# proxima-one/kzg

Measured on AMD Instinct MI355X. Metric: commitments/sec + MSM G1-adds/sec at degree 2^20, 1/2/4/8 MI355X, higher is better.
Workload: dtype u32 limbs (Fq 381-bit / Fr 255-bit Montgomery integer arithmetic); 1 GPU; degree-2^20 coeff_form commit (G1 Pippenger MSM) on 1xMI355X, batch of 64 per step; mode=single, polynomial_coefficients=1048576, scalars=uniform full-width Fr (SplitMix64 counter stream), terms_per_rank=1048576, window_bits=17, windows=15, srs=setup(tau, n) generated on the GPU, table=15 window rows 2^(17 w) P per point, inputs_resident_in_hbm=True

## Files before the change

### kzg_amd/csrc/capi.hip

```cpp
#include <algorithm>

#include "common.h"
#include "emit.h"
#include "multiopen_plan.h"

namespace kzg {

static int host_scalar(kzg_ctx *ctx, const void *s, int sfmt, Fr *mont) {
    Fr v;
    memcpy(v.v, s, 32);
    if (sfmt == KZG_FR_CANONICAL_LE_32) {
        if (!is_canonical(v)) return fail(ctx, KZG_ERR_SHAPE, "scalar not canonical (>= r)");
        v = to_mont(v);
    } else if (sfmt != KZG_FR_MONT_LE_32) {
        return fail(ctx, KZG_ERR_SHAPE, "unknown scalar format");
    }
    *mont = v;
    return KZG_OK;
}

static void scalar_out(const Fr &mont, int sfmt, void *dst) {
    Fr v = sfmt == KZG_FR_CANONICAL_LE_32 ? from_mont(mont) : mont;
    memcpy(dst, v.v, 32);
}
// ... 39 lines not shown
            KZG_HIP_CHECK(ctx, hipMemcpyAsync(ctx->lanes[lane].pinned, d_pt, sizeof(MsmPoint), hipMemcpyDeviceToHost, st));
            KZG_TRY(heavy_pickup_enqueue(ctx, lane));
            KZG_HIP_CHECK(ctx, hipStreamSynchronize(st));
            MsmPoint pt;
            memcpy(&pt, ctx->lanes[lane].pinned, sizeof pt);
            alignas(16) uint8_t buf[144];
            emit_one(pt, buf, ofmt);
            memcpy(out, buf, psz);
        } else {
            KZG_TRY(emit_point(ctx, lane, d_pt, ctx->lanes[lane].pinned, ofmt));
            KZG_TRY(heavy_pickup_enqueue(ctx, lane));
            KZG_HIP_CHECK(ctx, hipStreamSynchronize(st));
            memcpy(out, ctx->lanes[lane].pinned, psz);
        }
    }
    heavy_pickup_read(ctx, lane);
    if (ctx->prof) prof_collect(ctx);
    return KZG_OK;
}

static int check_sfmt(kzg_ctx *ctx, int sfmt) {
    if (sfmt != KZG_FR_MONT_LE_32 && sfmt != KZG_FR_CANONICAL_LE_32) return fail(ctx, KZG_ERR_SHAPE, "unknown scalar format");
    return KZG_OK;
}

static bool is_pow2(size_t x) { return x && !(x & (x - 1)); }
static bool count_ok(size_t n) { return n <= ((size_t)1 << 40); }

#ifdef KZG_TEST_HOOKS
__global__ __launch_bounds__(256) void k_test_fr_mul(const Fr *a, const Fr *b, size_t n, Fr *o) {
    size_t i = (size_t)blockIdx.x * blockDim.x + threadIdx.x;
    if (i < n) o[i] = mul(a[i], b[i]);
}
__global__ __launch_bounds__(256) void k_test_fq_mul(const Fq *a, const Fq *b, size_t n, Fq *o) {
    size_t i = (size_t)blockIdx.x * blockDim.x + threadIdx.x;
    if (i < n) o[i] = mul(a[i], b[i]);
}
__global__ __launch_bounds__(256) void k_test_fr_inv(const Fr *a, size_t n, Fr *o) {
    size_t i = (size_t)blockIdx.x * blockDim.x + threadIdx.x;
    if (i < n) o[i] = a[i].is_zero() ? Fr::zero() : inv(a[i]);
}
__global__ __launch_bounds__(256) void k_test_g1_add(const G1Affine *a, const G1Affine *b, size_t n, G1Affine *o) {
    size_t i = (size_t)blockIdx.x * blockDim.x + threadIdx.x;
    if (i >= n) return;
    G1Xyzz p = g1_madd(G1Xyzz::from_affine(a[i]), b[i]);
    G1Xyzz pa = g1_madd(g1_dbl(G1Xyzz::from_affine(a[i])), g1_neg(a[i]));
    G1Xyzz pb = g1_madd(g1_dbl(G1Xyzz::from_affine(b[i])), g1_neg(b[i]));
    G1Xyzz q = g1_add(pa, pb);
    G1Affine r1 = g1_to_affine(p), r2 = g1_to_affine(q);
    bool same = (r1.x == r2.x) && (r1.y == r2.y);
    o[i] = same ? r1 : G1Affine{Fq::one(), Fq::one()};
}
__global__ __launch_bounds__(256) void k_test_g1_mul(const G1Affine *p, const Fr *k, size_t n, G1Affine *o) {
    size_t i = (size_t)blockIdx.x * blockDim.x + threadIdx.x;
    if (i >= n) return;
    Fr kk = k[i];
    o[i] = g1_to_affine(g1_scalar_mul(p[i], kk.v));
}

#endif

}

using namespace kzg;

extern "C" int kzg_msm_g1(kzg_ctx *ctx, const kzg_srs *srs, size_t offset, const void *scalars, size_t n, int sfmt,
                          int flags, void *out, int ofmt) {
    if (!ctx || !srs || !out || (!scalars && n)) return KZG_ERR_SHAPE;
    Lease ls;
    KZG_TRY(lease_lane(ctx, &ls));
    const int lane = ls.lane;
    KZG_HIP_CHECK(ctx, hipSetDevice(ctx->device));
    KZG_TRY(check_sfmt(ctx, sfmt));
    if (!point_format_bytes(ofmt)) return fail(ctx, KZG_ERR_SHAPE, "unknown G1 output format");
    if (n > srs->n || offset > srs->n - n) return fail(ctx, KZG_ERR_SHAPE, "MSM range exceeds the SRS (reference: slice index panic)");
    KZG_TRY(lane_reserve(ctx, lane, msm_workspace_bytes(srs, n) + stage_bytes(n * 32, flags) + 8192));
    const void *d_sc = nullptr;
    KZG_TRY(stage_in(ctx, lane, scalars, n * 32, flags, &d_sc));
    MsmPoint *res = nullptr;
    KZG_TRY(lease_msm(ctx, ls, srs, offset, d_sc, n, sfmt, &res));
    return finish_point(ctx, lane, res, out, ofmt, flags);
}

extern "C" int kzg_commit_coeff(kzg_ctx *ctx, const kzg_srs *srs, const void *coeffs, size_t n, int sfmt, int flags,
                                void *out, int ofmt) {
    return kzg_msm_g1(ctx, srs, 0, coeffs, n, sfmt, flags, out, ofmt);
}

extern "C" int kzg_commit_eval(kzg_ctx *ctx, const kzg_srs *lagrange, const void *evals, size_t d, int sfmt, int flags,
                               void *out, int ofmt) {
    if (!ctx || !lagrange) return KZG_ERR_SHAPE;
    if (d != lagrange->n) return fail(ctx, KZG_ERR_SHAPE, "assert!(self.d == evals.d) (src/eval_form.rs:115)");
    return kzg_msm_g1(ctx, lagrange, 0, evals, d, sfmt, flags, out, ofmt);
}

struct BatchPipe {
    int nl = 1, nas = 0;
    uint8_t *d_out = nullptr;
    bool out_dev = false;
};

static int batch_begin(kzg_ctx *ctx, size_t batch, size_t out_bytes, void *out, int flags, BatchPipe *bp) {
    bp->out_dev = (flags & KZG_OUT_DEVICE) != 0;
    if (bp->out_dev) {
        bp->d_out = (uint8_t *)out;
    } else {
        if (ctx->batch_out_bytes < out_bytes + 256) {
            if (ctx->batch_out) hipFree(ctx->batch_out);
            ctx->batch_out = nullptr;
            ctx->batch_out_bytes = 0;
            KZG_HIP_CHECK(ctx, hipMalloc((void **)&ctx->batch_out, out_bytes + 256));
            ctx->batch_out_bytes = out_bytes + 256;
        }
        bp->d_out = (uint8_t *)ctx->batch_out;
    }
    KZG_TRY(plan_pipeline(ctx, (int)std::min<size_t>(batch, (size_t)ctx->opt_streams), &bp->nl, &bp->nas));
    for (int l = 0; l < bp->nl; l++) set_lane_mode(ctx, l, bp->nl > 1, batch >= 2 * (size_t)bp->nl);
    return KZG_OK;
}

static int batch_msm(kzg_ctx *ctx, const BatchPipe &bp, size_t b, int lane, const kzg_srs *srs, size_t offset, const void *d_sc,
                     size_t n, int sfmt, MsmPoint **res, MsmPending *defer = nullptr) {
    if (bp.nas) {
        const int ev = defer ? lane + (int)((b / (size_t)bp.nl) & 1) * bp.nl : lane;
        return msm_run(ctx, lane, srs, offset, d_sc, n, sfmt, res, ctx->accum_streams[b % (size_t)accum_streams_for(ctx, bp.nas, srs, n)],
                       ctx->sorted_events[ev], ctx->accum_events[ev], defer);
    }
    return msm_run(ctx, lane, srs, offset, d_sc, n, sfmt, res);
}

static int batch_end(kzg_ctx *ctx, const BatchPipe &bp, int rc, void *out, size_t out_bytes) {
    for (int l = 0; l < bp.nl; l++) hipStreamSynchronize(ctx->lanes[l].stream);
    for (int l = 0; l < bp.nl; l++) set_lane_mode(ctx, l, false, false);
    if (rc == KZG_OK && !bp.out_dev) {
        hipError_t e = hipMemcpy(out, bp.d_out, out_bytes, hipMemcpyDeviceToHost);
        if (e != hipSuccess) rc = fail(ctx, KZG_ERR_HIP, hipGetErrorString(e));
    }
#if !defined(KZG_TIMING_NO_PICKUP)
    if (rc == KZG_OK) {
        uint32_t hv[KZG_MAX_LANES];
        if (hipMemcpy(hv, ctx->d_lane_heavy, sizeof hv, hipMemcpyDeviceToHost) == hipSuccess)
            for (int l = 0; l < bp.nl; l++) {
                Lane &ln = ctx->lanes[l];
                if (ln.heavy_seq == ln.heavy_seen) continue;
                ln.heavy_seen = ln.heavy_seq;
                if (hv[l] == ln.heavy_seq) ctx->heavy_last.store(ctx->msm_count.load(std::memory_order_relaxed), std::memory_order_relaxed);
            }
    }
#endif
    if (ctx->prof) prof_collect(ctx);
    return rc;
}

namespace kzg {
int msm_batch_strided(kzg_ctx *ctx, const kzg_srs *srs, size_t offset, const void *scalars, size_t n, size_t batch,
                      size_t stride_bytes, int sfmt, int flags, void *out, int ofmt) {
    Guard g(ctx);
    KZG_HIP_CHECK(ctx, hipSetDevice(ctx->device));
    KZG_TRY(check_sfmt(ctx, sfmt));
    size_t psz = point_format_bytes(ofmt);
    if (!psz) return fail(ctx, KZG_ERR_SHAPE, "unknown G1 output format");
    if (n > srs->n || offset > srs->n - n) return fail(ctx, KZG_ERR_SHAPE, "MSM range exceeds the SRS");
    if (batch == 0) return KZG_OK;
    BatchPipe bp;
    KZG_TRY(batch_begin(ctx, batch, batch * psz, out, flags, &bp));
    size_t per = align_up(msm_workspace_bytes(srs, n) + stage_bytes(n * 32, flags) + 8192, 4096);
    int rc = KZG_OK;
    const bool defer = bp.nas > 0 && batch > (size_t)bp.nl && !ctx->opt_no_defer_tail;
    std::vector<MsmPending> pend(defer ? 2 * (size_t)bp.nl : 0);
    for (int l = 0; l < bp.nl && rc == KZG_OK; l++) rc = lane_reserve(ctx, l, defer ? 2 * per : per);
    auto finish = [&](size_t b) {
        const int l = (int)(b % bp.nl);
        MsmPoint *res = nullptr;
        int r = msm_finish(ctx, pend[(size_t)l + ((b / (size_t)bp.nl) & 1) * (size_t)bp.nl], &res);
        if (r == KZG_OK) r = emit_point(ctx, l, res, bp.d_out + b * psz, ofmt);
        return r;
    };
    for (size_t b = 0; b < batch && rc == KZG_OK; b++) {
        int l = (int)(b % bp.nl);
        const size_t half = defer ? ((b / (size_t)bp.nl) & 1) : 0;
        ctx->lanes[l].arena_used = half * per;
        ctx->lanes[l].arena_limit = defer ? (half + 1) * per : 0;
        const void *d_sc = nullptr;
        rc = stage_in(ctx, l, (const uint8_t *)scalars + b * stride_bytes, n * 32, flags, &d_sc);
        MsmPoint *res = nullptr;
        if (defer) {
            MsmPending &pd = pend[(size_t)l + half * (size_t)bp.nl];
            if (rc == KZG_OK) rc = batch_msm(ctx, bp, b, l, srs, offset, d_sc, n, sfmt, &res, &pd);
            if (rc == KZG_OK && !pd.active) pd.result = res;
            if (rc == KZG_OK && b >= (size_t)bp.nl) rc = finish(b - bp.nl);
            continue;
        }
        if (rc == KZG_OK) rc = batch_msm(ctx, bp, b, l, srs, offset, d_sc, n, sfmt, &res);
        if (rc == KZG_OK) rc = emit_point(ctx, l, res, bp.d_out + b * psz, ofmt);
    }
    if (defer)
        for (size_t b = batch > (size_t)bp.nl ? batch - bp.nl : 0; b < batch && rc == KZG_OK; b++) rc = finish(b);
    for (int l = 0; l < bp.nl; l++) ctx->lanes[l].arena_limit = 0;
    return batch_end(ctx, bp, rc, out, batch * psz);
}
}

extern "C" int kzg_msm_g1_batch(kzg_ctx *ctx, const kzg_srs *srs, size_t offset, const void *scalars, size_t n,
                                size_t batch, int sfmt, int flags, void *out, int ofmt) {
    if (!ctx || !srs || !out || (!scalars && n && batch)) return KZG_ERR_SHAPE;
    if (n > SIZE_MAX / 32) return KZG_ERR_SHAPE;
    return msm_batch_strided(ctx, srs, offset, scalars, n, batch, n * 32, sfmt, flags, out, ofmt);
}

extern "C" int kzg_witness_coeff_many(kzg_ctx *ctx, const kzg_srs *srs, const void *coeffs, size_t n, const void *xs,
                                      const void *ys, size_t count, int sfmt, int flags, void *out, int ofmt, int *status) {
    if (!ctx || !srs || !coeffs || !out || n == 0 || ((!xs || !ys) && count)) return KZG_ERR_SHAPE;
    Guard g(ctx);
    KZG_HIP_CHECK(ctx, hipSetDevice(ctx->device));
    KZG_TRY(check_sfmt(ctx, sfmt));
    size_t psz = point_format_bytes(ofmt);
    if (!psz) return fail(ctx, KZG_ERR_SHAPE, "unknown G1 output format");
    if (n - 1 > srs->n) return fail(ctx, KZG_ERR_SHAPE, "quotient longer than the SRS (reference: slice index panic)");
    if (count == 0) return KZG_OK;
    std::vector<Fr> xm(count);
    for (size_t j = 0; j < count; j++) KZG_TRY(host_scalar(ctx, (const uint8_t *)xs + 32 * j, sfmt, &xm[j]));
    for (size_t j = 0; j < count; j++) {
        Fr ym;
        KZG_TRY(host_scalar(ctx, (const uint8_t *)ys + 32 * j, sfmt, &ym));
    }
    BatchPipe bp;
    KZG_TRY(batch_begin(ctx, count, count * psz, out, flags, &bp));
    int rc = KZG_OK;
    const int sl = bp.nl;
    rc = ensure_lanes(ctx, sl + 1);
    if (rc == KZG_OK) rc = lane_reserve(ctx, sl, stage_bytes(n * 32, flags) + count * 32 + 4096);
    const void *d_coeffs = nullptr;
    Fr *d_px = nullptr;
    if (rc == KZG_OK) rc = stage_in(ctx, sl, coeffs, n * 32, flags, &d_coeffs);
    if (rc == KZG_OK && !(d_px = (Fr *)lane_alloc(ctx, sl, count * 32))) rc = fail(ctx, KZG_ERR_ALLOC, "workspace");
    if (rc == KZG_OK && hipStreamSynchronize(ctx->lanes[sl].stream) != hipSuccess) rc = fail(ctx, KZG_ERR_HIP, "stage-in of the coefficients");
    size_t per = msm_workspace_bytes(srs, n - 1) + n * 32 + (n / 2048 + 4) * 64 + 65536;
    for (int l = 0; l < bp.nl && rc == KZG_OK; l++) rc = lane_reserve(ctx, l, per);
    for (size_t j = 0; j < count && rc == KZG_OK; j++) {
        int l = (int)(j % bp.nl);
        ctx->lanes[l].arena_used = 0;
        Fr *dq = (Fr *)lane_alloc(ctx, l, n * 32);
        if (!dq) rc = fail(ctx, KZG_ERR_ALLOC, "workspace");
        if (rc == KZG_OK) rc = quotient_linear_run(ctx, l, (const Fr *)d_coeffs, n, xm[j], dq, d_px + j);
        MsmPoint *res = nullptr;
        if (rc == KZG_OK) rc = batch_msm(ctx, bp, j, l, srs, 0, dq, n - 1, sfmt, &res);
        if (rc == KZG_OK) rc = emit_point(ctx, l, res, bp.d_out + j * psz, ofmt);
    }
    rc = batch_end(ctx, bp, rc, out, count * psz);
    if (rc != KZG_OK) return rc;
    std::vector<uint8_t> px(count * 32);
    KZG_HIP_CHECK(ctx, hipMemcpy(px.data(), d_px, count * 32, hipMemcpyDeviceToHost));
    int worst = KZG_OK;
    for (size_t j = 0; j < count; j++) {
        int sj = memcmp(px.data() + 32 * j, (const uint8_t *)ys + 32 * j, 32) != 0 ? KZG_ERR_POINT_NOT_ON_POLY : KZG_OK;
        if (status) status[j] = sj;
        if (sj) worst = sj;
    }
    if (worst && !status) return fail(ctx, KZG_ERR_POINT_NOT_ON_POLY, "point not on polynomial!");
    return KZG_OK;
}

extern "C" int kzg_witness_eval_many(kzg_ctx *ctx, const kzg_srs *lagrange, const void *evals, size_t d, const size_t *indices,
                                     size_t count, int sfmt, int flags, void *out, int ofmt) {
    if (!ctx || !lagrange || !evals || !out || (!indices && count)) return KZG_ERR_SHAPE;
    Guard g(ctx);
    KZG_HIP_CHECK(ctx, hipSetDevice(ctx->device));
    KZG_TRY(check_sfmt(ctx, sfmt));
    size_t psz = point_format_bytes(ofmt);
    if (!psz) return fail(ctx, KZG_ERR_SHAPE, "unknown G1 output format");
    if (!is_pow2(d)) return fail(ctx, KZG_ERR_SHAPE, "evaluation domain size must be a power of two");
    for (size_t j = 0; j < count; j++)
        if (indices[j] >= d) return fail(ctx, KZG_ERR_SHAPE, "evaluation index out of range (reference: index panic)");
    if (d > lagrange->n) return fail(ctx, KZG_ERR_SHAPE, "evaluations longer than the Lagrange SRS (reference: slice panic)");
    uint32_t log_d = (uint32_t)ilog2_ceil(d);
    if (log_d >= FR_TWO_ADICITY) return fail(ctx, KZG_ERR_DEGREE_TOO_LARGE, "domain too large");
    if (count == 0) return KZG_OK;
    BatchPipe bp;
    KZG_TRY(batch_begin(ctx, count, count * psz, out, flags, &bp));
    const int sl = bp.nl;
    int rc = ensure_lanes(ctx, sl + 1);
    if (rc == KZG_OK) rc = lane_reserve(ctx, sl, stage_bytes(d * 32, flags) + 4096);
    const void *de = nullptr;
    if (rc == KZG_OK) rc = stage_in(ctx, sl, evals, d * 32, flags, &de);
    if (rc == KZG_OK) rc = eval_tables_ready(ctx, sl, log_d);
    size_t per = msm_workspace_bytes(lagrange, d) + d * 32 + (d / 256 + 4) * 32 + 65536;
    for (int l = 0; l < bp.nl && rc == KZG_OK; l++) rc = lane_reserve(ctx, l, per);
    for (size_t j = 0; j < count && rc == KZG_OK; j++) {
        int l = (int)(j % bp.nl);
        ctx->lanes[l].arena_used = 0;
        Fr *dq = (Fr *)lane_alloc(ctx, l, d * 32);
        if (!dq) rc = fail(ctx, KZG_ERR_ALLOC, "workspace");
        if (rc == KZG_OK) rc = quotient_eval_run(ctx, l, (const Fr *)de, log_d, indices[j], sfmt, dq);
        MsmPoint *res = nullptr;
        if (rc == KZG_OK) rc = batch_msm(ctx, bp, j, l, lagrange, 0, dq, d, sfmt, &res);
        if (rc == KZG_OK) rc = emit_point(ctx, l, res, bp.d_out + j * psz, ofmt);
    }
    return batch_end(ctx, bp, rc, out, count * psz);
}

extern "C" int kzg_g1_sum(kzg_ctx *ctx, const void *points, size_t count, int pfmt, int flags, void *out, int ofmt) {
    if (!ctx || !out || (!points && count)) return KZG_ERR_SHAPE;
    Guard g(ctx);
    KZG_HIP_CHECK(ctx, hipSetDevice(ctx->device));
    size_t psz = point_format_bytes(pfmt);
    if (!psz || !point_format_bytes(ofmt)) return fail(ctx, KZG_ERR_SHAPE, "unknown G1 point format");
    size_t cnt = count ? count : 1;
    size_t need = stage_bytes(cnt * psz, flags) + cnt * sizeof(G1Xyzz) + (cnt + 2 * sum_points_scratch_count(cnt) + 4) * sizeof(MsmPoint) + 8192;
    KZG_TRY(lane_reserve(ctx, 0, need));
    hipStream_t st = ctx->lanes[0].stream;
    G1Xyzz *dec = (G1Xyzz *)lane_alloc(ctx, 0, cnt * sizeof(G1Xyzz));
    MsmPoint *pts = (MsmPoint *)lane_alloc(ctx, 0, cnt * sizeof(MsmPoint));
    MsmPoint *scratch = (MsmPoint *)lane_alloc(ctx, 0, 2 * sum_points_scratch_count(cnt) * sizeof(MsmPoint));
    int *bad = (int *)lane_alloc(ctx, 0, 256);
    if (!dec || !pts || !scratch || !bad) return fail(ctx, KZG_ERR_ALLOC, "sum workspace not reserved");
    KZG_HIP_CHECK(ctx, hipMemsetAsync(bad, 0, sizeof(int), st));
    MsmPoint *res = pts;
    if (count == 0) {
        KZG_TRY(point_set_infinity(ctx, st, pts));
    } else {
        const void *d_raw = nullptr;
        KZG_TRY(stage_in(ctx, 0, points, count * psz, flags, &d_raw));
        KZG_TRY(decode_points(ctx, st, d_raw, count, pfmt, dec, bad, POINTS_ON_CURVE));
        KZG_TRY(points_to30(ctx, st, dec, pts, count));
        KZG_TRY(sum_points_run(ctx, 0, pts, count, scratch, &res));
    }
    int hbad = 0;
    KZG_HIP_CHECK(ctx, hipMemcpyAsync(&hbad, bad, sizeof(int), hipMemcpyDeviceToHost, st));
    KZG_TRY(finish_point(ctx, 0, res, out, ofmt, flags));
    if (hbad) return fail(ctx, KZG_ERR_BAD_POINT, "a G1 point failed to decode or is not on the curve");
    return KZG_OK;
}

namespace kzg {
int g1_sum_batch_strided(kzg_ctx *ctx, const void *points, size_t count, size_t groups, size_t gstride, size_t istride, int pfmt,
                         int flags, void *out, int ofmt, int level) {
    Guard g(ctx);
    KZG_HIP_CHECK(ctx, hipSetDevice(ctx->device));
    size_t psz = point_format_bytes(pfmt), osz = point_format_bytes(ofmt);
    if (!psz || !osz) return fail(ctx, KZG_ERR_SHAPE, "unknown G1 point format");
    if (count > (1u << 20) || groups > (1u << 24)) return fail(ctx, KZG_ERR_SHAPE, "kzg_g1_sum_batch: count <= 2^20, groups <= 2^24");
    size_t total = count && groups ? (groups - 1) * gstride + (count - 1) * istride + 1 : 0;
    KZG_TRY(lane_reserve(ctx, 0, stage_bytes(total * psz, flags) + total * sizeof(G1Xyzz) + (total + groups + 4) * sizeof(MsmPoint) + groups * 144 + 65536));
    hipStream_t st = ctx->lanes[0].stream;
    G1Xyzz *dec = (G1Xyzz *)lane_alloc(ctx, 0, total * sizeof(G1Xyzz));
    MsmPoint *pts = (MsmPoint *)lane_alloc(ctx, 0, total * sizeof(MsmPoint));
    MsmPoint *tmp = (MsmPoint *)lane_alloc(ctx, 0, groups * sizeof(MsmPoint));
    int *bad = (int *)lane_alloc(ctx, 0, 256);
    void *d_out = (flags & KZG_OUT_DEVICE) ? out : lane_alloc(ctx, 0, groups * osz);
    if (!dec || !pts || !tmp || !bad || !d_out) return fail(ctx, KZG_ERR_ALLOC, "sum workspace not reserved");
    KZG_HIP_CHECK(ctx, hipMemsetAsync(bad, 0, sizeof(int), st));
    const void *d_raw = nullptr;
    KZG_TRY(stage_in(ctx, 0, points, total * psz, flags, &d_raw));
    KZG_TRY(decode_points(ctx, st, d_raw, total, pfmt, dec, bad, level));
    KZG_TRY(points_to30(ctx, st, dec, pts, total));
    const bool on_host = !(flags & KZG_OUT_DEVICE) && ctx->opt_host_affine && groups <= 4;
    KZG_TRY(sum_groups_emit(ctx, 0, pts, count, groups, gstride, istride, tmp, on_host ? nullptr : d_out, ofmt));
    int hbad = 0;
    KZG_HIP_CHECK(ctx, hipMemcpyAsync(&hbad, bad, sizeof(int), hipMemcpyDeviceToHost, st));
    MsmPoint hsum[4];
// ... 1198 lines not shown
```

### kzg_amd/csrc/common.h

```cpp
#pragma once
#ifndef KZG_NTT_KERNEL_DEFAULT
#define KZG_NTT_KERNEL_DEFAULT 1
#endif
#include <hip/hip_runtime.h>
#include <stdint.h>
#include <stdio.h>

#include <array>
#include <atomic>
#include <condition_variable>
#include <map>
#include <mutex>
#include <string>
#include <vector>

#include "../../include/kzg_mi355x.h"
#include "curve.h"
#include "curve30.h"

namespace kzg {

struct ProfEntry {
    uint64_t launches = 0;
    double total_ms = 0.0;
};

struct PendingEvent {
    std::string name;
    hipEvent_t start, stop;
};

#ifndef KZG_ACCUM_WAVES
#define KZG_ACCUM_WAVES 2
#endif

struct MsmMode {
    int accum_blocks = 256 * KZG_ACCUM_WAVES;
    int sort_threads = 1024;
    bool tail_quads = true;
    bool tail_wide = false;
};

struct Lane {
    MsmMode mode;
    hipStream_t stream = nullptr;
    char *arena = nullptr;
    size_t arena_bytes = 0;
    size_t arena_used = 0;
    size_t arena_limit = 0;
    uint32_t heavy_seq = 0, heavy_seen = 0;
    char *pinned = nullptr;
    size_t pinned_bytes = 0;
};

struct NttPlan;
struct FixedBaseTable;
struct EvalDomainTables;

struct CtxGate {
    std::mutex m;
    std::condition_variable cv;
    int shared_active = 0;
    int excl_waiting = 0;
    bool exclusive = false;
    uint32_t lane_busy = 0;
    void lock() {
        std::unique_lock<std::mutex> lk(m);
        excl_waiting++;
        cv.wait(lk, [&] { return !exclusive && shared_active == 0; });
        excl_waiting--;
        exclusive = true;
    }
    void unlock() {
        {
            std::lock_guard<std::mutex> lk(m);
            exclusive = false;
        }
        cv.notify_all();
    }
};
constexpr int KZG_HEAVY_WINDOW = 64;
constexpr int KZG_MAX_LANES = 24;

}

struct kzg_ctx;
namespace kzg {
struct StreamPool;
struct PointSetCache;
void point_sets_free(kzg_ctx *ctx);
void point_set_stats(kzg_ctx *ctx, uint64_t *hits, uint64_t *misses);
}
struct kzg_ctx {
    int device = 0;
    kzg::CtxGate mu;
    std::mutex err_mu;
    std::mutex prof_mu;
    std::mutex cache_mu;
    std::mutex accum_mu;
    std::atomic<uint32_t> accum_rr{0};
    int plan_want_lanes = 0, plan_want_accum = 0, plan_lanes = 0, plan_accum = 0, plan_queues = 0;
    bool plan_warned = false;
    bool pipe_planned = false;
    int pipe_lanes = 1, pipe_accum = 0;
    std::string err;
    std::vector<kzg::Lane> lanes;
    kzg::StreamPool *pool = nullptr;
    int opt_window_bits = 0;
    int opt_streams = 13;
    int opt_accum_blocks = 0;
    int opt_hw_queues = 0;
    int probed_queues = 0;
    int probed_lanes = 0, probed_accum = 0;
    std::vector<hipStream_t> probed_order;
    int opt_window_rows = 0;
    int opt_naf_window = 0;
    int opt_trusted_points = 0;
    int opt_ntt_vec_log = 2;
    int opt_verify_cosets_chunk = 0;
    int opt_verify_eval_batch_chunk = 0;
    int opt_multiopen_points_chunk = 0;
    int opt_multi_eval_segment = 0;
    int opt_multi_eval_points_chunk = 0;
    int opt_poly_divide_base = 0;
    int opt_point_tree_leaf = 0;
    int opt_host_pairing = 1;
    int opt_fk20_cosets_combine = 0;
    int opt_ntt_kernel = KZG_NTT_KERNEL_DEFAULT;
    int opt_ntt_three_from = 23;
    int opt_ntt_vec2_log = 1;
    int opt_ntt_xcd = 1;
    int opt_accum_blocks_batch = 0;
    int opt_tail_quads = 1;
    int opt_accum_streams = 2;
    int opt_accum_streams_small = 4;
    int opt_accum_blocks_small = 160;
    int64_t opt_small_entries = 2 << 20;
    int planned_accum = 0;
    bool msm_small(size_t entries) const { return opt_accum_blocks_small > 0 && planned_accum >= 3 && (int64_t)entries <= opt_small_entries; }
    hipStream_t accum_streams[4] = {nullptr, nullptr, nullptr, nullptr};
    std::vector<hipEvent_t> sorted_events, accum_events;
    int opt_sort_threads = 1024;
    int opt_sort_threads_batch = 1024;
    int opt_host_affine = 1;
    int opt_heavy_bins = 0;
    bool opt_no_defer_tail = false;
    int opt_sort_single = 0;
    int accum_blocks_single() const { return opt_accum_blocks ? opt_accum_blocks : 256 * KZG_ACCUM_WAVES; }
    int accum_blocks_batch() const { return opt_accum_blocks_batch ? opt_accum_blocks_batch : 240 * KZG_ACCUM_WAVES; }
    int num_cus = 256;
    std::atomic<bool> attr_msm_set{false}, attr_ntt_set{false}, attr_wide_set{false}, attr_sort20_set{false}, attr_horner_set{false};
    bool prof = false;
    bool prof_only_accum = false;
    std::map<std::string, kzg::ProfEntry> prof_map;
    std::vector<kzg::PendingEvent> prof_pending;
    std::vector<hipEvent_t> event_pool;
    std::map<uint32_t, kzg::NttPlan *> ntt_plans;
    std::map<uint32_t, kzg::EvalDomainTables *> eval_tabs;
    kzg::FixedBaseTable *fixed_base = nullptr;
    std::vector<std::pair<std::array<uint32_t, 8>, void *>> coset_tabs;
    kzg::PointSetCache *point_sets = nullptr;
    int opt_witness_cache_slots = 16;
    std::atomic<uint64_t> msm_count{0}, heavy_last{0};
    uint32_t *d_lane_heavy = nullptr;
    void *batch_out = nullptr;
    size_t batch_out_bytes = 0;
};

struct kzg_srs {
    size_t n = 0;
    size_t npad = 0;
    int c = 0;
    int W = 0;
    int rows = 0;
    bool narrow17 = false;
    bool sort20 = false;
    int naf = 0;
    int row_shift = 0;
    kzg::G1Affine *table = nullptr;
    void *table30 = nullptr;
    int device = 0;
};

namespace kzg {

struct Guard {
    std::lock_guard<CtxGate> lk;
    explicit Guard(kzg_ctx *c) : lk(c->mu) {}
};

struct Lease {
    kzg_ctx *ctx = nullptr;
    int lane = -1;
    bool pipelined = false;
    uint32_t slot = 0;
    ~Lease();
};
int lease_lane(kzg_ctx *ctx, Lease *ls);

enum { POINTS_TRUSTED = 0, POINTS_ON_CURVE = 1, POINTS_SUBGROUP = 2 };

#define KZG_HIP_CHECK(ctx, expr)                                                                   \
    do {                                                                                           \
        hipError_t _e = (expr);                                                                    \
        if (_e != hipSuccess) return kzg::fail((ctx), KZG_ERR_HIP, std::string(#expr) + ": " + hipGetErrorString(_e)); \
    } while (0)

#define KZG_TRY(expr)                                                                              \
    do {                                                                                           \
        int _s = (expr);                                                                           \
        if (_s != KZG_OK) return _s;                                                               \
    } while (0)

struct ThreadErr {
    const kzg_ctx *ctx = nullptr;
    std::string msg;
};
inline ThreadErr &thread_err() {
    static thread_local ThreadErr te;
    return te;
}
inline int fail(kzg_ctx *ctx, int code, const std::string &msg) {
    {
        std::lock_guard<std::mutex> lk(ctx->err_mu);
        ctx->err = msg;
    }
    ThreadErr &te = thread_err();
    te.ctx = ctx;
    te.msg = msg;
    return code;
}

int lane_reserve(kzg_ctx *ctx, int lane, size_t bytes);
void *lane_alloc(kzg_ctx *ctx, int lane, size_t bytes);
int lane_pinned(kzg_ctx *ctx, int lane, size_t bytes);
int ensure_lanes(kzg_ctx *ctx, int want);
int plan_pipeline(kzg_ctx *ctx, int want, int *nl_out, int *nas_out);
void set_lane_mode(kzg_ctx *ctx, int lane, bool pipelined, bool deep);
int accum_streams_for(kzg_ctx *ctx, int planned, const kzg_srs *srs, size_t n);

struct ProfScope {
    kzg_ctx *ctx;
    hipStream_t stream;
    hipEvent_t start = nullptr, stop = nullptr;
    const char *name;
    ProfScope(kzg_ctx *c, hipStream_t s, const char *n);
    ~ProfScope();
};
void prof_collect(kzg_ctx *ctx);

#define KZG_LAUNCH(ctx, stream, name, kern, grid, block, shmem, ...)                               \
    do {                                                                                           \
        kzg::ProfScope _ps((ctx), (stream), (name));                                               \
        hipLaunchKernelGGL(kern, dim3(grid), dim3(block), (shmem), (stream), __VA_ARGS__);         \
    } while (0)

inline int untrusted_level(const kzg_ctx *ctx) { return ctx->opt_trusted_points ? POINTS_ON_CURVE : POINTS_SUBGROUP; }
inline size_t align_up(size_t x, size_t a) { return (x + a - 1) / a * a; }
inline int ilog2_ceil(size_t x) {
    int l = 0;
    while (((size_t)1 << l) < x) l++;
    return l;
}

typedef G1Xyzz30 MsmPoint;

size_t msm_workspace_bytes(const kzg_srs *srs, size_t n);
int finish_point(kzg_ctx *ctx, int lane, const MsmPoint *d_pt, void *out, int ofmt, int flags);
struct MsmPending {
    bool active = false;
    hipStream_t st = nullptr;
    hipEvent_t accum_ev = nullptr;
    MsmMode mm;
    const MsmPoint *part = nullptr;
    MsmPoint *scratch = nullptr, *result = nullptr;
    const uint32_t *s1 = nullptr;
    int B = 0;
    size_t expected = 0;
    void *state = nullptr;
    char *tail_base = nullptr;
    size_t tail_off[8] = {0, 0, 0, 0, 0, 0, 0, 0};
    bool odd = false;
};
int msm_run(kzg_ctx *ctx, int lane, const kzg_srs *srs, size_t offset, const void *d_scalars, size_t n, int sfmt,
            MsmPoint **d_result, hipStream_t accum_stream = nullptr, hipEvent_t sorted_ev = nullptr, hipEvent_t accum_ev = nullptr,
            MsmPending *defer = nullptr);
int msm_finish(kzg_ctx *ctx, MsmPending &pd, MsmPoint **d_result);
int lease_msm(kzg_ctx *ctx, const Lease &ls, const kzg_srs *srs, size_t offset, const void *d_sc, size_t n, int sfmt, MsmPoint **res);
int sum_points_run(kzg_ctx *ctx, int lane, MsmPoint *d_points, size_t count, MsmPoint *d_scratch, MsmPoint **d_result);
int points_to30(kzg_ctx *ctx, hipStream_t st, const G1Xyzz *d_in, MsmPoint *d_out, size_t n);
int points_from30(kzg_ctx *ctx, hipStream_t st, const MsmPoint *d_in, G1Xyzz *d_out, size_t n);
int point_set_infinity(kzg_ctx *ctx, hipStream_t st, MsmPoint *d_pt);
size_t sum_points_scratch_count(size_t count);
int emit_point(kzg_ctx *ctx, int lane, const MsmPoint *d_point, void *d_out, int ofmt);
size_t point_format_bytes(int fmt);
int sum_groups_emit(kzg_ctx *ctx, int lane, const MsmPoint *d_pts, size_t count, size_t groups, size_t gstride, size_t istride,
                    MsmPoint *d_tmp, void *d_out, int ofmt);

int msm_batch_strided(kzg_ctx *ctx, const kzg_srs *srs, size_t offset, const void *scalars, size_t n, size_t batch,
                      size_t stride_bytes, int sfmt, int flags, void *out, int ofmt);
int g1_sum_batch_strided(kzg_ctx *ctx, const void *points, size_t count, size_t groups, size_t gstride, size_t istride, int pfmt,
                         int flags, void *out, int ofmt, int level = POINTS_ON_CURVE);

int srs_choose_window(int opt_window_bits, size_t n);
void srs_shape(int opt_window_bits, int opt_window_rows, size_t n, int *c, int *W, int *rows, bool *narrow17, int opt_naf = 0, int *naf = nullptr);
inline size_t srs_entries_per_scalar(const kzg_srs *s) { return s->naf ? (size_t)s->W : (size_t)s->rows; }
int srs_alloc(kzg_ctx *ctx, size_t n, kzg_srs **out);
int srs_finish_from_xyzz(kzg_ctx *ctx, kzg_srs *srs, G1Xyzz *d_row0_xyzz);
int srs_precompute(kzg_ctx *ctx, kzg_srs *srs);
int batch_to_affine(kzg_ctx *ctx, hipStream_t stream, const G1Xyzz *d_in, G1Affine *d_out, size_t n);
int decode_points(kzg_ctx *ctx, hipStream_t st, const void *d_raw, size_t n, int fmt, G1Xyzz *d_out, int *d_bad,
                  int level = POINTS_SUBGROUP);

int fixed_base_mul(kzg_ctx *ctx, hipStream_t stream, const Fr *d_scalars_mont, size_t n, G1Xyzz *d_out);
int powers_run(kzg_ctx *ctx, hipStream_t st, const Fr &base_mont, size_t first, size_t n, Fr *d_out);
int lagrange_scalars_run(kzg_ctx *ctx, hipStream_t st, const Fr &tau_mont, size_t d, Fr *d_out);

struct WitnessSink {
    const kzg_srs *srs;
    size_t first, len;
    size_t total;
    void *d_partial;
};
int witness_coeff_batched_run(kzg_ctx *ctx, const WitnessSink &sink, const void *coeffs, size_t n, const void *xs, const void *ys,
                              size_t k, int sfmt, int flags, void *out_w, int ofmt, void *out_r, size_t *out_r_len);
int vanishing_poly_run(kzg_ctx *ctx, hipStream_t st, const Fr *d_xs_mont, size_t k, Fr *d_z, Fr *d_tmp);
int coset_ntt_run(kzg_ctx *ctx, int lane, Fr *d, uint32_t log_n, int inverse, const Fr &g, size_t nnz = (size_t)-1);

void ntt_plans_free(kzg_ctx *ctx);
void eval_tabs_free(kzg_ctx *ctx);
void fixed_base_free(kzg_ctx *ctx);

int ntt_run(kzg_ctx *ctx, int lane, Fr *d_data, uint32_t log_n, int inverse, size_t nnz = (size_t)-1);
inline size_t ntt_workspace_bytes(uint32_t log_n) {
    const size_t n = (size_t)1 << log_n;
    return log_n > 24 ? n * 32 + ((size_t)1 << 24) * 32 + (2 << 20) : n * 32 + 4096;
}
bool ntt_short_input_ok(uint32_t log_n, size_t nnz);
int pow_table(kzg_ctx *ctx, hipStream_t stream, const Fr &base_mont, const Fr &scale_mont, size_t count, Fr *d_out);
Fr host_omega(uint32_t exp);

int fr_convert(kzg_ctx *ctx, hipStream_t stream, Fr *d_data, size_t n, int to_mont);
int batch_inverse(kzg_ctx *ctx, hipStream_t stream, const Fr *d_in, Fr *d_out, size_t n);
int batch_inverse_mul(kzg_ctx *ctx, hipStream_t stream, const Fr *d_c, Fr *d_a, Fr *d_tmp, size_t n, int *d_flag);
int poly_eval_run(kzg_ctx *ctx, int lane, const Fr *d_coeffs, size_t n, const Fr &x_mont, Fr *d_y_out);
int eval_tables_ready(kzg_ctx *ctx, int lane, uint32_t log_d);
int quotient_linear_run(kzg_ctx *ctx, int lane, const Fr *d_coeffs, size_t n, const Fr &x_mont, Fr *d_q_out,
                        Fr *d_px_out);
int quotient_eval_run(kzg_ctx *ctx, int lane, const Fr *d_evals, uint32_t log_d, size_t m, int sfmt, Fr *d_q_out);

constexpr int OE_MAX_CHUNK = 16;
struct OpenPoint {
    Fr z;
    Fr c;
    bool on_domain;
    size_t m;
};
int open_point_classify(uint32_t log_d, const Fr &z_mont, OpenPoint *pt);
size_t open_eval_fr_workspace_bytes(size_t d, size_t B);
size_t open_eval_fr_workspace_bytes(size_t d, size_t B, size_t nz);
int open_eval_fr_run(kzg_ctx *ctx, int lane, const Fr *d_evals, uint32_t log_d, size_t B, const OpenPoint *pts, int sfmt, Fr *d_y, Fr *d_q);

size_t open_powtab_bytes(size_t d);
int open_powtab_run(kzg_ctx *ctx, hipStream_t st, uint32_t log_d, Fr *d_tab);
int open_inverses_run(kzg_ctx *ctx, hipStream_t st, uint32_t log_d, const Fr *d_tab, const Fr *z_mont, int nz, Fr *d_den, Fr *d_inv);
int open_eval_values_idx_run(kzg_ctx *ctx, hipStream_t st, const Fr *d_evals, uint32_t log_d, const Fr *d_inv, const uint32_t *d_vidx,
                             const uint32_t *d_pu, const Fr *d_z, const Fr *d_c, size_t B, Fr *d_partial, Fr *d_y);

int fold_run(kzg_ctx *ctx, hipStream_t st, const Fr *d_v, size_t d, size_t t, size_t gstride, size_t groups, const Fr *d_gammas_mont,
             bool carry, Fr *d_out);

int lincomb_run(kzg_ctx *ctx, hipStream_t st, const Fr *d_v, size_t d, const uint32_t *d_idx, const Fr *d_weight, size_t count, bool carry,
                Fr *d_out);
int multiopen_gather_run(kzg_ctx *ctx, hipStream_t st, const Fr *d_v, size_t d, const uint32_t *d_idx, const uint32_t *d_at, size_t count, Fr *d_y);
int multiopen_accum_run(kzg_ctx *ctx, hipStream_t st, const Fr *d_v, size_t d, const uint32_t *d_idx, const Fr *d_w, const uint32_t *d_pstart,
                        int nz, const Fr *d_y, Fr *d_Y, const Fr *d_inv, Fr *d_g);

int series_inverse_run(kzg_ctx *ctx, int lane, const Fr *d_f, size_t fl_all, size_t m, size_t base, Fr *d_g, Fr *d_A, Fr *d_G);

int pt_ntt_run(kzg_ctx *ctx, hipStream_t st, Fr *d, size_t total, uint32_t log_t, int dit, const Fr *tw, uint32_t log_tw);


}
```

### kzg_amd/csrc/msm.hip

```cpp
#include "msm_internal.h"
#include "msm_sort.h"
#include "emit.h"
#include "naf.h"

namespace kzg {

template <class F>
__device__ __forceinline__ void digits_of(const uint32_t s[8], int c, int W, bool balanced, F f) {
    if (c == 17 && W == 15) for_each_digit_fixed<17, 15>(s, balanced, f);
    else for_each_digit(s, c, W, balanced, f);
}

extern __shared__ __attribute__((aligned(16))) uint32_t lds_u32[];

__global__ __launch_bounds__(1024) void k_hist(const Fr *scalars, size_t n, int sfmt, int c, int W, int B,
                                               size_t per_block, uint32_t *blk_hist, int mode, int w_lo, int w_hi) {
    const bool pk = mode == 2;
    const int BH = pk ? B / 2 : B;
    size_t i0 = (size_t)blockIdx.x * per_block;
    size_t i1 = i0 + per_block < n ? i0 + per_block : n;
    uint32_t *dst = blk_hist + (size_t)blockIdx.x * B;
    for (int half = 0; half < (pk ? 2 : 1); half++) {
        const uint32_t base = (uint32_t)half * (uint32_t)BH;
        if (half) __syncthreads();
        for (int b = threadIdx.x; b < BH; b += blockDim.x) lds_u32[b] = 0;
        __syncthreads();
        for (size_t i = i0 + threadIdx.x; i < i1; i += blockDim.x) {
            uint32_t s[8];
            load_scalar(scalars, i, sfmt, s);
            digits_of(s, c, W, pk, [&](int w, uint32_t mag, uint32_t) {
                if (w < w_lo || w >= w_hi) return;
                const uint32_t idx = (mag - 1) & (uint32_t)(B - 1);
                if (pk && (idx >> 15) != (uint32_t)half) return;
                atomicAdd(&lds_u32[idx - base], 1u);
            });
        }
        __syncthreads();
        for (int b = threadIdx.x; b < BH; b += blockDim.x) dst[base + b] = lds_u32[b];
    }
}

constexpr int SCAN_SEG = 256;
__global__ __launch_bounds__(SCAN_SEG) void k_scan_a(uint32_t *blk_hist, int G, int B, uint32_t *total, uint32_t *local, uint32_t *agg,
                                                     uint32_t *ready) {
    __shared__ uint32_t lds[4];
    if (threadIdx.x == 0) ready[blockIdx.x] = 0;
    const int b = blockIdx.x * SCAN_SEG + threadIdx.x;
    uint32_t run = 0;
    if (b < B) {
        for (int g = 0; g < G; g++) {
            uint32_t t = blk_hist[(size_t)g * B + b];
            blk_hist[(size_t)g * B + b] = run;
            run += t;
        }
        total[b] = run;
    }
    uint32_t tot;
    uint32_t ex = block_scan_256(run, lds, &tot);
    if (b < B) local[b] = ex;
    if (threadIdx.x == 0) agg[blockIdx.x] = tot;
}

__device__ __forceinline__ uint32_t mod_u32(uint32_t x, uint32_t e, double rcp_e) {
    uint32_t q = (uint32_t)((double)x * rcp_e);
    uint32_t r = x - q * e;
    if ((int32_t)r < 0) r += e;
    if (r >= e) r -= e;
    return r;
}

__global__ __launch_bounds__(SCAN_SEG) void k_scan_b(const uint32_t *total, const uint32_t *local, const uint32_t *agg, int B, int NB,
                                                     uint32_t *bucket_start, uint32_t *s1, MsmState *st, uint32_t slots, uint32_t *ready) {
    __shared__ uint32_t lds[4];
    __shared__ uint32_t my_prefix;
    uint32_t M;
    {
        uint32_t v = (int)threadIdx.x < NB ? agg[threadIdx.x] : 0u;
        uint32_t ex = block_scan_256(v, lds, &M);
        if (threadIdx.x == blockIdx.x) my_prefix = ex;
    }
    __syncthreads();
    uint32_t E = (M + slots - 1) / slots;
    if (E < KZG_ACCUM_MIN_CHUNK) E = KZG_ACCUM_MIN_CHUNK;
    const double rcp_e = 1.0 / (double)E;
    const int b = blockIdx.x * SCAN_SEG + threadIdx.x;
    uint32_t start = 0, f = 0;
    if (b < B) {
        start = my_prefix + local[b];
        f = (total[b] != 0 && mod_u32(start, E, rcp_e) != 0) ? 1u : 0u;
    }
    uint32_t ftot;
    const uint32_t fex = block_scan_256(f, lds, &ftot);
    if (threadIdx.x == 0) __hip_atomic_store(&ready[blockIdx.x], (ftot << 1) | 1u, __ATOMIC_RELAXED, __HIP_MEMORY_SCOPE_AGENT);
    uint32_t prev = 0;
    if (threadIdx.x < blockIdx.x) {
        uint32_t w;
        while (((w = __hip_atomic_load(&ready[threadIdx.x], __ATOMIC_RELAXED, __HIP_MEMORY_SCOPE_AGENT)) & 1u) == 0) __builtin_amdgcn_s_sleep(1);
        prev = w >> 1;
    }
    uint32_t before;
    block_scan_256(prev, lds, &before);
    if (b < B) {
        bucket_start[b] = start;
        s1[b] = before + fex + (start + E - 1) / E;
    }
    if (blockIdx.x == (unsigned)NB - 1 && threadIdx.x == 0) {
        bucket_start[B] = M;
        s1[B] = before + ftot + (M + E - 1) / E;
        st->M = M;
        st->E = E;
        st->ntasks = (M + E - 1) / E;
        st->ovf_tasks = 0;
    }
}

static int scan_run(kzg_ctx *ctx, hipStream_t st, uint32_t *blk_hist, int G, int B, uint32_t *total, uint32_t *local, uint32_t *agg,
                    uint32_t *bucket_start, uint32_t *s1, MsmState *state, uint32_t slots) {
    const int NB = (B + SCAN_SEG - 1) / SCAN_SEG;
    uint32_t *ready = agg + SCAN_SEG;
    KZG_LAUNCH(ctx, st, "k_scan_a", k_scan_a, NB, SCAN_SEG, 0, blk_hist, G, B, total, local, agg, ready);
    KZG_LAUNCH(ctx, st, "k_scan_b", k_scan_b, NB, SCAN_SEG, 0, total, local, agg, B, NB, bucket_start, s1, state, slots, ready);
    return KZG_OK;
}

__global__ __launch_bounds__(1024) void k_scatter(const Fr *scalars, size_t n, int sfmt, int c, int W, int B,
                                                  size_t per_block, const uint32_t *blk_off,
                                                  const uint32_t *bucket_start, uint32_t row_stride,
                                                  uint32_t idx_base, uint32_t *entries, int mode, int w_lo, int w_hi) {
    const uint32_t *off = blk_off + (size_t)blockIdx.x * B;
    const bool pk = mode == 2;
    const int BH = pk ? B / 2 : B;
    size_t i0 = (size_t)blockIdx.x * per_block;
    size_t i1 = i0 + per_block < n ? i0 + per_block : n;
    for (int half = 0; half < (pk ? 2 : 1); half++) {
        const uint32_t base = (uint32_t)half * (uint32_t)BH;
        if (half) __syncthreads();
        for (int b = threadIdx.x; b < BH; b += blockDim.x) lds_u32[b] = bucket_start[base + b] + off[base + b];
        __syncthreads();
        for (size_t i = i0 + threadIdx.x; i < i1; i += blockDim.x) {
            uint32_t s[8];
            load_scalar(scalars, i, sfmt, s);
            digits_of(s, c, W, pk, [&](int w, uint32_t mag, uint32_t neg) {
                if (w < w_lo || w >= w_hi) return;
                const uint32_t idx = (mag - 1) & (uint32_t)(B - 1);
                if (pk && (idx >> 15) != (uint32_t)half) return;
                const uint32_t pos = atomicAdd(&lds_u32[idx - base], 1u);
                const uint32_t hi = mode == 1 ? (((mag - 1) >> WIDE_LO_BITS) << WIDE_HI_SHIFT) : 0u;
                entries[pos] = ((uint32_t)(w - w_lo) * row_stride + idx_base + (uint32_t)i) | hi | (neg << 31);
            });
        }
    }
}

constexpr int BIN_SHIFT = 6, BIN_BUCKETS = 1 << BIN_SHIFT;

__global__ __launch_bounds__(1024) void k_bin_hist(const Fr *scalars, size_t n, int sfmt, size_t per_block, uint32_t *blk_bins,
                                                   int w_lo, int w_hi) {
    KZG_SIDE_PRIO_STMT;
    __shared__ uint32_t h[NBINS];
    for (int b = threadIdx.x; b < NBINS; b += blockDim.x) h[b] = 0;
    __syncthreads();
    size_t i0 = (size_t)blockIdx.x * per_block;
    size_t i1 = i0 + per_block < n ? i0 + per_block : n;
    for (size_t i = i0 + threadIdx.x; i < i1; i += blockDim.x) {
        uint32_t s[8];
        load_scalar(scalars, i, sfmt, s);
        for_each_digit_fixed<17, 15>(s, true, [&](int w, uint32_t mag, uint32_t) {
            if (w < w_lo || w >= w_hi) return;
            atomicAdd(&h[(mag - 1) >> BIN_SHIFT], 1u);
        });
    }
    __syncthreads();
    for (int b = threadIdx.x; b < NBINS; b += blockDim.x) blk_bins[(size_t)blockIdx.x * NBINS + b] = h[b];
}

constexpr int BIN_SCAN_SLICES = 16, BIN_SCAN_MAXG = 32;
constexpr int SORT2_MAX_BLOCKS = BIN_SCAN_SLICES * BIN_SCAN_MAXG;
__global__ __launch_bounds__(1024) void k_bin_scan(uint32_t *blk_bins, int G, uint32_t *bin_total, uint32_t *ready) {
    KZG_SIDE_PRIO_STMT;
    __shared__ uint32_t part[BIN_SCAN_SLICES][64];
    if (blockIdx.x == 0 && threadIdx.x < SCAN_SEG) ready[threadIdx.x] = 0;
    const int binl = threadIdx.x & 63, slice = threadIdx.x >> 6;
    const int bin = blockIdx.x * 64 + binl;
    const int gs = (G + BIN_SCAN_SLICES - 1) / BIN_SCAN_SLICES;
    const int g0 = slice * gs;
    uint32_t v[BIN_SCAN_MAXG];
#pragma unroll
    for (int k = 0; k < BIN_SCAN_MAXG; k++) v[k] = (k < gs && g0 + k < G) ? blk_bins[(size_t)(g0 + k) * NBINS + bin] : 0u;
    uint32_t sum = 0;
#pragma unroll
    for (int k = 0; k < BIN_SCAN_MAXG; k++) {
        const uint32_t t = v[k];
        v[k] = sum;
        sum += t;
    }
    part[slice][binl] = sum;
    __syncthreads();
    uint32_t pre = 0, tot = 0;
#pragma unroll
    for (int s2 = 0; s2 < BIN_SCAN_SLICES; s2++) {
        const uint32_t t = part[s2][binl];
        if (s2 < slice) pre += t;
        tot += t;
    }
#pragma unroll
    for (int k = 0; k < BIN_SCAN_MAXG; k++)
        if (k < gs && g0 + k < G) blk_bins[(size_t)(g0 + k) * NBINS + bin] = pre + v[k];
    if (slice == 0) bin_total[bin] = tot;
}


constexpr int BIN_SCATTER_LDS = (3 * NBINS + 16 + 15 * 1024) * 4;
template <class REC>
__global__ __launch_bounds__(1024) void k_bin_scatter(const Fr *scalars, size_t n, int sfmt, size_t per_block, const uint32_t *blk_off,
                                                      const uint32_t *bin_total, uint32_t *bin_base, uint32_t row_stride,
                                                      uint32_t idx_base, typename REC::T *rec, int w_lo, int w_hi) {
    KZG_SIDE_PRIO_STMT;
    uint32_t *cur = lds_u32, *cnt = cur + NBINS, *off = cnt + NBINS, *wsum = off + NBINS, *stage = wsum + 16;
    const uint32_t tid = threadIdx.x;
    {
        uint32_t tot;
        const uint32_t ex = block_scan_1024(bin_total[tid], wsum, &tot);
        cur[tid] = ex + blk_off[(size_t)blockIdx.x * NBINS + tid];
        if (blockIdx.x == 0) {
            bin_base[tid] = ex;
            if (tid == 0) bin_base[NBINS] = tot;
        }
    }
    const size_t i0 = (size_t)blockIdx.x * per_block;
    const size_t i1 = i0 + per_block < n ? i0 + per_block : n;
    for (size_t c0 = i0; c0 < i1; c0 += 1024) {
        cnt[tid] = 0;
        __syncthreads();
        uint32_t pk[15], rk[15];
#pragma unroll
        for (int w = 0; w < 15; w++) pk[w] = 0xffffffffu;
        if (c0 + tid < i1) {
            uint32_t s[8];
            load_scalar(scalars, c0 + tid, sfmt, s);
            for_each_digit_fixed<17, 15>(s, true, [&](int w, uint32_t mag, uint32_t neg) {
                if (w < w_lo || w >= w_hi) return;
                const uint32_t idx = mag - 1, bin = idx >> BIN_SHIFT;
                rk[w] = atomicAdd(&cnt[bin], 1u);
                pk[w] = bin | ((idx & (BIN_BUCKETS - 1)) << 10) | (neg << 16) | ((uint32_t)(w - w_lo) << 17) | (tid << 21);
            });
        }
        __syncthreads();
        uint32_t tot;
        off[tid] = block_scan_1024(cnt[tid], wsum, &tot);
        __syncthreads();
#pragma unroll
        for (int w = 0; w < 15; w++)
            if (pk[w] != 0xffffffffu) stage[off[pk[w] & (NBINS - 1)] + rk[w]] = pk[w];
        __syncthreads();
        const uint32_t ebase = idx_base + (uint32_t)c0;
        for (uint32_t p = tid; p < tot; p += 1024) {
            const uint32_t v = stage[p], bin = v & (NBINS - 1);
            const uint32_t index = ((v >> 17) & 15u) * row_stride + ebase + (v >> 21);
            rec[cur[bin] + p - off[bin]] = REC::pack(index, (v >> 16) & 1u, (v >> 10) & (BIN_BUCKETS - 1));
        }
        __syncthreads();
        cur[tid] += cnt[tid];
    }
}

__global__ __launch_bounds__(1024) void k_naf_recode(const Fr *scalars, size_t n, int sfmt, size_t per_block, uint32_t *recs, uint32_t *blk_bins) {
    __shared__ uint32_t h[NBINS];
    __shared__ uint32_t limbs[1024 * 12];
    for (int b = threadIdx.x; b < NBINS; b += blockDim.x) h[b] = 0;
    __syncthreads();
    uint32_t *L = limbs + threadIdx.x * 12;
    size_t i0 = (size_t)blockIdx.x * per_block;
    size_t i1 = i0 + per_block < n ? i0 + per_block : n;
    for (size_t i = i0 + threadIdx.x; i < i1; i += blockDim.x) {
        uint32_t s[8];
        load_scalar(scalars, i, sfmt, s);
        uint32_t flip = 0;
        if (s[7] & 0x40000000u) {
            uint64_t bw = 0;
#pragma unroll
            for (int k = 0; k < 8; k++) {
                uint64_t d = (uint64_t)FrParams::mod(k) - s[k] - bw;
                s[k] = (uint32_t)d;
                bw = (d >> 63) & 1u;
            }
            flip = 1;
        }
#pragma unroll
        for (int k = 0; k < 8; k++) L[k] = s[k];
        L[8] = L[9] = L[10] = L[11] = 0;
        uint32_t d[NAF_MAX_DIGITS];
        const int cnt = naf18_digits(L, flip, d);
#pragma unroll
        for (int k = 0; k < NAF_MAX_DIGITS; k++) {
            const uint32_t r = k < cnt ? d[k] : 0u;
            recs[(size_t)k * n + i] = r;
            if (r) atomicAdd(&h[(r & 0x1ffffu) >> BIN_SHIFT], 1u);
        }
    }
    __syncthreads();
    for (int b = threadIdx.x; b < NBINS; b += blockDim.x) blk_bins[(size_t)blockIdx.x * NBINS + b] = h[b];
}

template <class REC>
__global__ __launch_bounds__(1024) void k_bin_scatter_naf(const uint32_t *recs, size_t n, size_t per_block, const uint32_t *blk_off,
                                                          const uint32_t *bin_total, uint32_t *bin_base, uint32_t row_stride,
                                                          uint32_t idx_base, typename REC::T *rec) {
    uint32_t *cur = lds_u32, *cnt = cur + NBINS, *off = cnt + NBINS, *wsum = off + NBINS, *stage = wsum + 16;
    const uint32_t tid = threadIdx.x;
    {
        uint32_t tot;
        const uint32_t ex = block_scan_1024(bin_total[tid], wsum, &tot);
        cur[tid] = ex + blk_off[(size_t)blockIdx.x * NBINS + tid];
        if (blockIdx.x == 0) {
            bin_base[tid] = ex;
            if (tid == 0) bin_base[NBINS] = tot;
        }
    }
    const size_t i0 = (size_t)blockIdx.x * per_block;
    const size_t i1 = i0 + per_block < n ? i0 + per_block : n;
    for (size_t c0 = i0; c0 < i1; c0 += 1024) {
        cnt[tid] = 0;
        __syncthreads();
        uint32_t pk[NAF_MAX_DIGITS], rk[NAF_MAX_DIGITS];
#pragma unroll
        for (int k = 0; k < NAF_MAX_DIGITS; k++) {
            pk[k] = 0xffffffffu;
            if (c0 + tid < i1) {
                const uint32_t r = recs[(size_t)k * n + c0 + tid];
                if (r & NAF_REC_VALID) {
                    const uint32_t idx = r & 0x1ffffu, bin = idx >> BIN_SHIFT;
                    rk[k] = atomicAdd(&cnt[bin], 1u);
                    pk[k] = bin | ((idx & (BIN_BUCKETS - 1)) << 10) | (((r >> 17) & 1u) << 16) | ((uint32_t)k << 17) | (tid << 21);
                }
            }
        }
        __syncthreads();
        uint32_t tot;
        off[tid] = block_scan_1024(cnt[tid], wsum, &tot);
        __syncthreads();
#pragma unroll
        for (int k = 0; k < NAF_MAX_DIGITS; k++)
            if (pk[k] != 0xffffffffu) stage[off[pk[k] & (NBINS - 1)] + rk[k]] = pk[k];
        __syncthreads();
        const uint32_t ebase = idx_base + (uint32_t)c0;
        for (uint32_t p = tid; p < tot; p += 1024) {
            const uint32_t v = stage[p], bin = v & (NBINS - 1), t = v >> 21, k = (v >> 17) & 15u;
            const uint32_t row = (recs[(size_t)k * n + c0 + t] >> 18) & 0xffu;
            const uint32_t index = row * row_stride + ebase + t;
            rec[cur[bin] + p - off[bin]] = REC::pack(index, (v >> 16) & 1u, (v >> 10) & (BIN_BUCKETS - 1));
        }
        __syncthreads();
        cur[tid] += cnt[tid];
    }
}


__global__ __launch_bounds__(SCAN_SEG) void k_scan_b_bins(const uint32_t *total, const uint32_t *bin_base, int B, int NB,
                                                          uint32_t *bucket_start, uint32_t *s1, MsmState *st, uint32_t slots,
                                                          uint32_t *ready) {
    KZG_SIDE_PRIO_STMT;
    __shared__ uint32_t lds[4];
    const uint32_t M = bin_base[NBINS];
    const uint32_t my_prefix = bin_base[blockIdx.x * (SCAN_SEG / BIN_BUCKETS)];
    uint32_t E = (M + slots - 1) / slots;
    if (E < KZG_ACCUM_MIN_CHUNK) E = KZG_ACCUM_MIN_CHUNK;
    const double rcp_e = 1.0 / (double)E;
    const int b = blockIdx.x * SCAN_SEG + threadIdx.x;
    const uint32_t cnt = b < B ? total[b] : 0u;
    uint32_t btot;
    const uint32_t start = my_prefix + block_scan_256(cnt, lds, &btot);
    const uint32_t f = (cnt != 0 && mod_u32(start, E, rcp_e) != 0) ? 1u : 0u;
    uint32_t ftot;
    const uint32_t fex = block_scan_256(f, lds, &ftot);
    if (threadIdx.x == 0) __hip_atomic_store(&ready[blockIdx.x], (ftot << 1) | 1u, __ATOMIC_RELAXED, __HIP_MEMORY_SCOPE_AGENT);
    uint32_t prev = 0;
    if (threadIdx.x < blockIdx.x) {
        uint32_t w;
        while (((w = __hip_atomic_load(&ready[threadIdx.x], __ATOMIC_RELAXED, __HIP_MEMORY_SCOPE_AGENT)) & 1u) == 0) __builtin_amdgcn_s_sleep(1);
        prev = w >> 1;
    }
    uint32_t before;
    block_scan_256(prev, lds, &before);
    if (b < B) {
        bucket_start[b] = start;
        s1[b] = before + fex + (start + E - 1) / E;
    }
    if (blockIdx.x == (unsigned)NB - 1 && threadIdx.x == 0) {
        bucket_start[B] = M;
        s1[B] = before + ftot + (M + E - 1) / E;
        st->M = M;
        st->E = E;
        st->ntasks = (M + E - 1) / E;
        st->ovf_tasks = 0;
    }
}

__device__ __forceinline__ G1Affine30 load_entry_point30(const uint4 *table30, uint32_t ent) {
#if defined(KZG_TIMING_GATHER)
    const uint32_t e_ = ent & 0x7fffffffu;
    const size_t row_ = KZG_TIMING_GATHER == 1 ? (e_ & 0x3ffu) : KZG_TIMING_GATHER == 2 ? ((size_t)(e_ & 0x1ffu) << 14)
                        : KZG_TIMING_GATHER == 3 ? (e_ & 0x7ffffu) : (e_ & 0x3fffffu);
    const uint4 *src = table30 + row_ * (KZG_ROW_BYTES / 16);
#else
    const uint4 *src = table30 + (size_t)(ent & 0x7fffffffu) * (KZG_ROW_BYTES / 16);
#endif
    G1Affine30 p;
    uint4 *dst = reinterpret_cast<uint4 *>(&p);
#if defined(KZG_GATHER_NT)
    typedef unsigned int u32x4 __attribute__((ext_vector_type(4)));
#pragma unroll
    for (int k = 0; k < 7; k++) {
        const u32x4 v = __builtin_nontemporal_load(reinterpret_cast<const u32x4 *>(src) + k);
        dst[k] = make_uint4(v.x, v.y, v.z, v.w);
    }
#else
#pragma unroll
    for (int k = 0; k < 7; k++) dst[k] = src[k];
#endif
    return p;
}

__global__ __launch_bounds__(256) __attribute__((amdgpu_waves_per_eu(KZG_ACCUM_WAVES, KZG_ACCUM_WAVES))) void k_accum_affine(const uint32_t *entries, const uint32_t *bucket_start,
                                                      const uint32_t *s1, int B, const uint4 *table30,
                                                      MsmPoint *out, const MsmState *st) {
    const uint32_t E = st->E, M = st->M;
    const uint32_t s = blockIdx.x * blockDim.x + threadIdx.x;
    const uint64_t lo64 = (uint64_t)s * E;
    if (lo64 >= M) return;
    const uint32_t lo = (uint32_t)lo64;
    const uint32_t hi = (M - lo < E) ? M : lo + E;
    uint32_t bl = 0, bh = (uint32_t)B;
    while (bh - bl > 1) {
        uint32_t mid = (bl + bh) >> 1;
        if (bucket_start[mid] <= lo) bl = mid; else bh = mid;
    }
    uint32_t b = bl;
    uint32_t bend = bucket_start[b + 1];
    uint32_t bend_next = bucket_start[b + 2 < (uint32_t)B ? b + 2 : (uint32_t)B];
    uint32_t f_next = s1[b + 1] - (bucket_start[b + 1] + E - 1) / E;
    uint32_t pos = s + f_next;
    uint32_t ent = entries[lo];
    G1Affine30 cur = load_entry_point30(table30, ent);
    int32_t sigma;
    G1Xyzz30 acc = g1_from_table30s(cur, ent >> 31, sigma);
    uint32_t ent_next = 0;
    if (lo + 1 < hi) {
        ent = entries[lo + 1];
        cur = load_entry_point30(table30, ent);
    }
#ifndef KZG_NO_ENTRY_LOOKAHEAD
    if (lo + 2 < hi) ent_next = entries[lo + 2];
#endif
    for (uint32_t k = lo + 1; k < hi; k++) {
        const bool neg_k = (ent >> 31) != 0;
        int mode = 0;
        Madd30Mid mid;
        if (k == bend) {
            out[pos++] = g1_partial_store30(acc, sigma);
            for (;;) {
                b++;
                bend = bend_next;
                bend_next = bucket_start[b + 2 < (uint32_t)B ? b + 2 : (uint32_t)B];
                if (bend > k) break;
            }
            mode = 1;
        } else if (cur.is_inf_table()) {
            mode = 2;
        } else if (acc.inf) {
            mode = 1;
        }
        if (mode == 0) {
            sigma = g1_tau30(sigma, neg_k);
            mid = g1_madd30s_phase1(acc, cur, sigma);
        }
        if (mode == 1) acc = g1_from_table30s(cur, neg_k, sigma);
        if (k + 1 < hi) {
#ifndef KZG_NO_ENTRY_LOOKAHEAD
            ent = ent_next;
            if (k + 2 < hi) ent_next = entries[k + 2];
#else
            ent = entries[k + 1];
#endif
            cur = load_entry_point30(table30, ent);
        }
        if (mode == 0) acc = g1_madd30s_phase2(acc, mid, sigma, neg_k, sigma, [&]() { return load_entry_point30(table30, entries[k]); });
    }
    out[pos] = g1_partial_store30(acc, sigma);
}

__global__ __launch_bounds__(256) void k_sum_level(const MsmPoint *in, uint32_t count, int L, MsmPoint *out) {
    uint32_t t = blockIdx.x * blockDim.x + threadIdx.x;
    uint32_t nout = (count + L - 1) / L;
    if (t >= nout) return;
    uint32_t s = t * L, e = s + L < count ? s + L : count;
    MsmPoint acc = in[s];
    for (uint32_t k = s + 1; k < e; k++) acc = g1_add30(acc, in[k]);
    out[t] = acc;
}

__device__ __forceinline__ size_t format_bytes_dev(int fmt) {
    return fmt == KZG_G1_JACOBIAN_MONT_144 ? 144 : fmt == KZG_G1_ZCASH_COMPRESSED_48 ? 48 : 96;
}

__global__ __launch_bounds__(64) void k_emit_points(const MsmPoint *pts, size_t count, size_t stride_pts, uint8_t *out, int fmt) {
    KZG_SIDE_PRIO_STMT;
    size_t i = (size_t)blockIdx.x * blockDim.x + threadIdx.x;
    if (i >= count) return;
    emit_one(pts[i * stride_pts], out + i * format_bytes_dev(fmt), fmt);
}

__global__ __launch_bounds__(64) void k_sum_groups(const MsmPoint *pts, uint32_t count, uint32_t groups, size_t gstride,
                                                   size_t istride, MsmPoint *out) {
    uint32_t g = blockIdx.x * blockDim.x + threadIdx.x;
    if (g >= groups) return;
    MsmPoint acc = MsmPoint::infinity();
    for (uint32_t i = 0; i < count; i++) acc = g1_add30(acc, pts[(size_t)g * gstride + (size_t)i * istride]);
    out[g] = acc;
}

int sum_groups_emit(kzg_ctx *ctx, int lane, const MsmPoint *d_pts, size_t count, size_t groups, size_t gstride, size_t istride,
                    MsmPoint *d_tmp, void *d_out, int ofmt) {
    hipStream_t st = ctx->lanes[lane].stream;
    KZG_LAUNCH(ctx, st, "k_sum_groups", k_sum_groups, (unsigned)((groups + 63) / 64), 64, 0, d_pts, (uint32_t)count,
               (uint32_t)groups, gstride, istride, d_tmp);
    if (!d_out) return KZG_OK;
    KZG_LAUNCH(ctx, st, "k_emit_points", k_emit_points, (unsigned)((groups + 63) / 64), 64, 0, d_tmp, groups, (size_t)1,
               (uint8_t *)d_out, ofmt);
    return KZG_OK;
}

__global__ __launch_bounds__(256) void k_points_to30(const G1Xyzz *in, MsmPoint *out, size_t n) {
    size_t i = (size_t)blockIdx.x * blockDim.x + threadIdx.x;
    if (i < n) out[i] = g1_xyzz_to30(in[i]);
}
__global__ __launch_bounds__(256) void k_points_from30(const MsmPoint *in, G1Xyzz *out, size_t n) {
    size_t i = (size_t)blockIdx.x * blockDim.x + threadIdx.x;
    if (i < n) out[i] = g1_xyzz_from30(in[i]);
}
__global__ void k_point_set_infinity(MsmPoint *p) { *p = MsmPoint::infinity(); }

int points_to30(kzg_ctx *ctx, hipStream_t st, const G1Xyzz *d_in, MsmPoint *d_out, size_t n) {
    if (n) KZG_LAUNCH(ctx, st, "k_points_to30", k_points_to30, (unsigned)((n + 255) / 256), 256, 0, d_in, d_out, n);
    return KZG_OK;
}
int points_from30(kzg_ctx *ctx, hipStream_t st, const MsmPoint *d_in, G1Xyzz *d_out, size_t n) {
    if (n) KZG_LAUNCH(ctx, st, "k_points_from30", k_points_from30, (unsigned)((n + 255) / 256), 256, 0, d_in, d_out, n);
    return KZG_OK;
}
int point_set_infinity(kzg_ctx *ctx, hipStream_t st, MsmPoint *d_pt) {
    KZG_LAUNCH(ctx, st, "k_point_set_infinity", k_point_set_infinity, 1, 1, 0, d_pt);
    return KZG_OK;
}

size_t point_format_bytes(int fmt) {
    switch (fmt) {
        case KZG_G1_AFFINE_MONT_96: return 96;
        case KZG_G1_JACOBIAN_MONT_144: return 144;
        case KZG_G1_ZCASH_UNCOMPRESSED_96: return 96;
        case KZG_G1_ZCASH_COMPRESSED_48: return 48;
        default: return 0;
    }
}

int emit_point(kzg_ctx *ctx, int lane, const MsmPoint *d_point, void *d_out, int ofmt) {
    if (!point_format_bytes(ofmt)) return fail(ctx, KZG_ERR_SHAPE, "unknown G1 output format");
    hipStream_t st = ctx->lanes[lane].stream;
    KZG_LAUNCH(ctx, st, "k_emit_points", k_emit_points, 1, 64, 0, d_point, (size_t)1, (size_t)1, (uint8_t *)d_out,
               ofmt);
    return KZG_OK;
}

static int sort_blocks(size_t n) {
    size_t g = (n + 2047) / 2048;
    if (g < 1) g = 1;
    if (g > 256) g = 256;
    return (int)g;
}

static int sort2_blocks(size_t n) {
    size_t g = (n + 2047) / 2048;
    if (g < 1) g = 1;
    if (g > SORT2_MAX_BLOCKS) g = SORT2_MAX_BLOCKS;
    return (int)g;
}

size_t sum_points_scratch_count(size_t count) { return (count + SUM_L - 1) / SUM_L + 64; }

struct MsmLayout {
    int B, G, G2;
    size_t M_max, T1_max;
    size_t off_bins, off_bin_base, off_recs, off_seg, off_hv;
    size_t off_blk_hist, off_total, off_local, off_agg, off_bucket_start, off_s1, off_state, off_entries, off_bufA, off_bufB, off_tail,
        off_pass, bytes;
    TailLayout tail;
};

static MsmLayout msm_layout(const kzg_srs *srs, size_t n) {
    MsmLayout L;
    L.B = 1 << (srs->c - 1);
    L.G = sort_blocks(n);
    L.M_max = n * srs_entries_per_scalar(srs);
    L.T1_max = (size_t)ACC_SLOTS + L.B + 1;
    size_t o = 0;
    auto take = [&](size_t bytes) {
        size_t r = o;
        o = align_up(o + bytes, 256);
        return r;
    };
    L.G2 = sort2_blocks(n);
    size_t sort_bytes = (size_t)L.G * L.B * 4;
    if (srs->narrow17 && L.M_max * 8 > sort_bytes) sort_bytes = L.M_max * 8;
    if (srs->sort20) sort_bytes = L.M_max * 8;
    L.off_blk_hist = take(sort_bytes);
    L.off_bins = take((size_t)L.G2 * NBINS * 4);
    L.off_bin_base = take((2 * NBINS + 1) * 4);
    L.off_recs = take(srs->naf ? (size_t)NAF_MAX_DIGITS * n * 4 : 0);
    L.off_seg = take(srs->sort20 ? 3 * 256 * 4 : 0);
    L.off_hv = take(srs->sort20 ? sort2_hv_bytes(SORT20_BUCKETS) : (srs->narrow17 || srs->naf) ? sort2_hv_bytes(BIN_BUCKETS) : 0);
    L.off_total = take((size_t)L.B * 4);
    L.off_local = take((size_t)L.B * 4);
    L.off_agg = take(2 * SCAN_SEG * 4 + 64);
    L.off_bucket_start = take((size_t)(L.B + 1) * 4);
    L.off_s1 = take((size_t)(L.B + 1) * 4);
    L.off_state = take(sizeof(MsmState));
    L.off_entries = take(L.M_max * 4 + 16);
    L.off_bufA = take(L.T1_max * sizeof(MsmPoint));
    L.off_bufB = take(L.T1_max * sizeof(MsmPoint));
    L.tail = tail_layout(L.B, L.T1_max);
    L.off_tail = take(L.tail.bytes);
    L.off_pass = take(((size_t)(srs->W + srs->rows - 1) / srs->rows + 1) * sizeof(MsmPoint));
    L.bytes = o;
    return L;
}

struct WideLayout {
    int B_lo, nhi, Btot, G;
    size_t M_max, T1_max;
    size_t off_blk_hist, off_total, off_local, off_agg, off_lo_start, off_s1_lo, off_state, off_entries1, off_entries2, off_bucket_start, off_s1,
        off_blockcnt, off_binbase, off_segsums, off_segmaxs, off_segtotal, off_bufA, off_bufB, off_tail, bytes;
    TailLayout tail;
};

static WideLayout wide_layout(const kzg_srs *srs, size_t n) {
    WideLayout L;
    L.B_lo = 1 << WIDE_LO_BITS;
    L.nhi = 1 << (srs->c - 1 - WIDE_LO_BITS);
    L.Btot = L.nhi * L.B_lo;
    L.G = sort_blocks(n);
    L.M_max = n * (size_t)srs->W;
    L.T1_max = (size_t)ACC_SLOTS + L.Btot + 1;
    size_t o = 0;
    auto take = [&](size_t bytes) {
        size_t r = o;
        o = align_up(o + bytes, 256);
        return r;
    };
    L.off_blk_hist = take((size_t)L.G * L.B_lo * 4);
    L.off_total = take((size_t)L.B_lo * 4);
    L.off_local = take((size_t)L.B_lo * 4);
    L.off_agg = take(2 * SCAN_SEG * 4 + 64);
    L.off_lo_start = take((size_t)(L.B_lo + 1) * 4);
// ... 145 lines not shown
    size_t per_block = (n + G - 1) / G;
    const int mode = srs->narrow17 ? 2 : 0;
    size_t lds_bytes = srs->narrow17 ? (size_t)B * 2 : (size_t)B * 4;

    const int rows = srs->naf ? W : srs->rows, passes = (W + rows - 1) / rows;
    MsmPoint *pass_res = (MsmPoint *)(base + L.off_pass);
    const bool in_pipeline = accum_stream && accum_stream != st;
    const int acc_blocks = in_pipeline && ctx->msm_small(L.M_max) && ctx->opt_accum_blocks_small < mm.accum_blocks ? ctx->opt_accum_blocks_small
                                                                                                                   : mm.accum_blocks;
    const uint32_t slots = (uint32_t)acc_blocks * 256u;
    uint32_t *hvp = (uint32_t *)(base + L.off_hv);
    const uint32_t heavy_seq = ++ctx->lanes[lane].heavy_seq;
    uint32_t *lane_heavy = ctx->d_lane_heavy + lane;
    bool sliced = ctx->opt_heavy_bins == 1;
    {
        const uint64_t now = ctx->msm_count.fetch_add(1, std::memory_order_relaxed) + 1, last = ctx->heavy_last.load(std::memory_order_relaxed);
        if (ctx->opt_heavy_bins == 0 && last != 0 && now - last <= (uint64_t)KZG_HEAVY_WINDOW) sliced = true;
    }
    for (int p = 0; p < passes; p++) {
        const int w_lo = p * rows, w_hi = (p + 1) * rows < W ? (p + 1) * rows : W;
        if (srs->naf) {
            const int G2 = L.G2;
            const size_t per2 = (n + G2 - 1) / G2;
            uint32_t *bins = (uint32_t *)(base + L.off_bins), *bin_base = (uint32_t *)(base + L.off_bin_base);
            uint32_t *ready = (uint32_t *)(base + L.off_agg) + SCAN_SEG;
            uint32_t *recs = (uint32_t *)(base + L.off_recs);
            KZG_LAUNCH(ctx, st, "k_naf_recode", k_naf_recode, G2, 1024, 0, sc, n, sfmt, per2, recs, bins);
            uint32_t *bin_total = bin_base + NBINS + 1;
            KZG_LAUNCH(ctx, st, "k_bin_scan", k_bin_scan, NBINS / 64, 1024, 0, bins, G2, bin_total, ready);
            if ((uint64_t)srs->rows * srs->npad < REC4_MAX_INDEX) {
                uint32_t *rec = (uint32_t *)blk_hist;
                KZG_LAUNCH(ctx, st, "k_bin_scatter", k_bin_scatter_naf<Rec4>, G2, 1024, BIN_SCATTER_LDS, recs, n, per2, bins, bin_total, bin_base,
                           (uint32_t)srs->npad, (uint32_t)offset, rec);
                KZG_TRY(sort2_level2(ctx, st, 4, rec, bin_base, bin_total, hvp, entries, total, bucket_start, nullptr, slots, sliced, lane_heavy, heavy_seq));
            } else {
                uint2 *rec = (uint2 *)blk_hist;
                KZG_LAUNCH(ctx, st, "k_bin_scatter", k_bin_scatter_naf<Rec8>, G2, 1024, BIN_SCATTER_LDS, recs, n, per2, bins, bin_total, bin_base,
                           (uint32_t)srs->npad, (uint32_t)offset, rec);
                KZG_TRY(sort2_level2(ctx, st, 8, rec, bin_base, bin_total, hvp, entries, total, bucket_start, nullptr, slots, sliced, lane_heavy, heavy_seq));
            }
            KZG_LAUNCH(ctx, st, "k_scan_b_bins", k_scan_b_bins, B / SCAN_SEG, SCAN_SEG, 0, total, bin_base, B, B / SCAN_SEG, bucket_start, s1,
                       state, slots, ready);
        } else if (srs->sort20) {
            const int G2 = L.G2;
            uint32_t *bins = (uint32_t *)(base + L.off_bins), *bin_base = (uint32_t *)(base + L.off_bin_base);
            uint32_t *ready = (uint32_t *)(base + L.off_agg) + SCAN_SEG, *bin_total = bin_base + NBINS + 1;
            uint32_t *seg = (uint32_t *)(base + L.off_seg);
            KZG_TRY(sort20_hist(ctx, st, sc, n, sfmt, G2, bins));
            KZG_LAUNCH(ctx, st, "k_bin_scan", k_bin_scan, NBINS / 64, 1024, 0, bins, G2, bin_total, ready);
            KZG_TRY(sort20_place(ctx, st, sc, n, sfmt, G2, bins, bin_total, bin_base, (uint32_t)srs->npad, (uint32_t)offset, blk_hist, entries,
                                 bucket_start, s1, state, slots, seg, seg + 256, seg + 512, hvp, sliced, lane_heavy, heavy_seq));
        } else if (srs->narrow17 && !ctx->opt_sort_single) {
            const int G2 = L.G2;
            const size_t per2 = (n + G2 - 1) / G2;
            uint32_t *bins = (uint32_t *)(base + L.off_bins), *bin_base = (uint32_t *)(base + L.off_bin_base);
            uint32_t *ready = (uint32_t *)(base + L.off_agg) + SCAN_SEG;
            KZG_LAUNCH(ctx, st, "k_bin_hist", k_bin_hist, G2, 1024, 0, sc, n, sfmt, per2, bins, w_lo, w_hi);
            uint32_t *bin_total = bin_base + NBINS + 1;
            KZG_LAUNCH(ctx, st, "k_bin_scan", k_bin_scan, NBINS / 64, 1024, 0, bins, G2, bin_total, ready);
            if ((uint64_t)srs->rows * srs->npad < REC4_MAX_INDEX) {
                uint32_t *rec = (uint32_t *)blk_hist;
                KZG_LAUNCH(ctx, st, "k_bin_scatter", k_bin_scatter<Rec4>, G2, 1024, BIN_SCATTER_LDS, sc, n, sfmt, per2, bins, bin_total,
                           bin_base, (uint32_t)srs->npad, (uint32_t)offset, rec, w_lo, w_hi);
                KZG_TRY(sort2_level2(ctx, st, 4, rec, bin_base, bin_total, hvp, entries, total, bucket_start, nullptr, slots, sliced, lane_heavy, heavy_seq));
            } else {
                uint2 *rec = (uint2 *)blk_hist;
                KZG_LAUNCH(ctx, st, "k_bin_scatter", k_bin_scatter<Rec8>, G2, 1024, BIN_SCATTER_LDS, sc, n, sfmt, per2, bins, bin_total,
                           bin_base, (uint32_t)srs->npad, (uint32_t)offset, rec, w_lo, w_hi);
                KZG_TRY(sort2_level2(ctx, st, 8, rec, bin_base, bin_total, hvp, entries, total, bucket_start, nullptr, slots, sliced, lane_heavy, heavy_seq));
            }
            KZG_LAUNCH(ctx, st, "k_scan_b_bins", k_scan_b_bins, B / SCAN_SEG, SCAN_SEG, 0, total, bin_base, B, B / SCAN_SEG, bucket_start, s1,
                       state, slots, ready);
        } else {
            KZG_LAUNCH(ctx, st, "k_hist", k_hist, G, mm.sort_threads, lds_bytes, sc, n, sfmt, c, W, B, per_block, blk_hist, mode, w_lo,
                       w_hi);
            KZG_TRY(scan_run(ctx, st, blk_hist, G, B, total, (uint32_t *)(base + L.off_local), (uint32_t *)(base + L.off_agg), bucket_start,
                             s1, state, slots));
            KZG_LAUNCH(ctx, st, "k_scatter", k_scatter, G, mm.sort_threads, lds_bytes, sc, n, sfmt, c, W, B, per_block, blk_hist,
                       bucket_start, (uint32_t)srs->npad, (uint32_t)offset, entries, mode, w_lo, w_hi);
        }
        size_t thr1 = L.M_max / KZG_ACCUM_MIN_CHUNK + 1 < (size_t)slots ? L.M_max / KZG_ACCUM_MIN_CHUNK + 1 : (size_t)slots;
        unsigned grid1 = (unsigned)((thr1 + 255) / 256);
        if (accum_stream && accum_stream != st) {
            KZG_HIP_CHECK(ctx, hipEventRecord(sorted_ev, st));
            std::lock_guard<std::mutex> alk(ctx->accum_mu);
            KZG_HIP_CHECK(ctx, hipStreamWaitEvent(accum_stream, sorted_ev, 0));
            KZG_LAUNCH(ctx, accum_stream, "k_accum_affine", k_accum_affine, grid1, 256, 0, entries, bucket_start, s1, B,
                       (const uint4 *)srs->table30, bufA, state);
            KZG_HIP_CHECK(ctx, hipEventRecord(accum_ev, accum_stream));
            if (defer && passes == 1) {
                static_assert(sizeof(TailLayout) == sizeof(defer->tail_off), "MsmPending::tail_off mirrors TailLayout");
                defer->active = true;
                defer->st = st;
                defer->accum_ev = accum_ev;
                defer->mm = mm;
                defer->part = bufA;
                defer->scratch = bufB;
                defer->s1 = s1;
                defer->B = B;
                defer->expected = expected_partials(L.M_max, slots, B);
                defer->state = state;
                defer->tail_base = base + L.off_tail;
                memcpy(defer->tail_off, &L.tail, sizeof(TailLayout));
                defer->odd = srs->naf != 0;
                *d_result = nullptr;
                return KZG_OK;
            }
            KZG_HIP_CHECK(ctx, hipStreamWaitEvent(st, accum_ev, 0));
        } else {
            KZG_LAUNCH(ctx, st, "k_accum_affine", k_accum_affine, grid1, 256, 0, entries, bucket_start, s1, B,
                       (const uint4 *)srs->table30, bufA, state);
        }
        MsmPoint *res = nullptr;
        KZG_TRY(msm_tail_run(ctx, st, mm, bufA, bufB, s1, B, expected_partials(L.M_max, slots, B), state, base + L.off_tail, L.tail, &res,
                             srs->naf != 0));
        if (passes == 1) {
            *d_result = res;
            return KZG_OK;
        }
        KZG_HIP_CHECK(ctx, hipMemcpyAsync(pass_res + p, res, sizeof(MsmPoint), hipMemcpyDeviceToDevice, st));
    }
    KZG_LAUNCH(ctx, st, "k_combine_passes", k_combine_passes, 1, 64, 0, pass_res, passes, c * rows, pass_res + passes);
    *d_result = pass_res + passes;
    return KZG_OK;
}

int msm_finish(kzg_ctx *ctx, MsmPending &pd, MsmPoint **d_result) {
    if (!pd.active) {
        *d_result = pd.result;
        return KZG_OK;
    }
    pd.active = false;
    KZG_HIP_CHECK(ctx, hipStreamWaitEvent(pd.st, pd.accum_ev, 0));
    TailLayout tl;
    memcpy(&tl, pd.tail_off, sizeof tl);
    return msm_tail_run(ctx, pd.st, pd.mm, pd.part, pd.scratch, pd.s1, pd.B, pd.expected, (MsmState *)pd.state, pd.tail_base, tl, d_result, pd.odd);
}

int msm_run(kzg_ctx *ctx, int lane, const kzg_srs *srs, size_t offset, const void *d_scalars, size_t n, int sfmt,
            MsmPoint **d_result, hipStream_t accum_stream, hipEvent_t sorted_ev, hipEvent_t accum_ev, MsmPending *defer) {
    if (defer) defer->active = false;
    if (srs->device != ctx->device)
        return fail(ctx, KZG_ERR_SHAPE, "the SRS is resident on GPU " + std::to_string(srs->device) + ", this context runs on GPU " +
                                            std::to_string(ctx->device) + ": upload or generate it through this context");
    if (n > srs->n || offset > srs->n - n) return fail(ctx, KZG_ERR_SHAPE, "MSM range exceeds the SRS (reference: slice index panic)");
    if (srs->c > 16 && !srs->narrow17 && !(srs->sort20 && !ctx->opt_sort_single))
        return msm_run_wide(ctx, lane, srs, offset, d_scalars, n, sfmt, d_result);
    if ((uint64_t)srs->rows * srs->npad >= (1ull << 31))
        return fail(ctx, KZG_ERR_SHAPE, "SRS too large for the 31-bit entry index (table rows * points < 2^31)");
    if (srs->naf && offset + n > srs->npad) return fail(ctx, KZG_ERR_SHAPE, "MSM range exceeds the SRS");
    return msm_run_narrow(ctx, lane, srs, offset, d_scalars, n, sfmt, d_result, accum_stream, sorted_ev, accum_ev, defer);
}

}
```

### kzg_amd/csrc/msm_internal.h

```cpp
#pragma once
#include "common.h"

#ifndef KZG_SIDE_PRIO
#define KZG_SIDE_PRIO 0
#endif
#if KZG_SIDE_PRIO > 0
#define KZG_SIDE_PRIO_STMT __builtin_amdgcn_s_setprio(KZG_SIDE_PRIO)
#else
#define KZG_SIDE_PRIO_STMT ((void)0)
#endif

#ifndef KZG_ACCUM_MIN_CHUNK
#define KZG_ACCUM_MIN_CHUNK 8
#endif

namespace kzg {

constexpr uint32_t ACC_SLOTS = 256 * 4 * KZG_ACCUM_WAVES * 64;
constexpr int TAIL_THREADS = 256;
constexpr int SUM_L = 4;
constexpr int WIDE_LO_BITS = 15;
constexpr int WIDE_HI_SHIFT = 27;
constexpr uint32_t WIDE_HI_MASK = 0xfu << WIDE_HI_SHIFT;

struct MsmState {
    uint32_t M;
    uint32_t ntasks;
    uint32_t reserved[4];
    uint32_t E;
    uint32_t ovf_tasks;
};


int sum_level_run(kzg_ctx *ctx, hipStream_t st, const MsmPoint *in, uint32_t count, int L, MsmPoint *out);

constexpr int HI_BLOCKS = 256;
constexpr int HI_THREADS = 1024;
constexpr int SEG = 2048;
int wide_sort_pass2(kzg_ctx *ctx, hipStream_t st, const uint32_t *entries1, const MsmState *state, int nhi, uint32_t *blockcnt,
                    uint32_t *binbase, const uint32_t *lo_start, int B_lo, uint32_t *entries2, uint32_t *bucket_start);
int wide_s1_layout(kzg_ctx *ctx, hipStream_t st, const uint32_t *bucket_start, int Btot, MsmState *state, uint32_t *segsums,
                   uint32_t *segmaxs, uint32_t *segtotal, uint32_t *s1_out);
constexpr int NBINS = 1024;
constexpr int SORT20_C = 20, SORT20_W = 13, SORT20_SHIFT = 9, SORT20_BUCKETS = 1 << SORT20_SHIFT;
int sort20_hist(kzg_ctx *ctx, hipStream_t st, const void *d_scalars, size_t n, int sfmt, int G2, uint32_t *bins);
int sort20_place(kzg_ctx *ctx, hipStream_t st, const void *d_scalars, size_t n, int sfmt, int G2, const uint32_t *bins,
                 const uint32_t *bin_total, uint32_t *bin_base, uint32_t row_stride, uint32_t idx_base, void *rec, uint32_t *entries,
                 uint32_t *bucket_start, uint32_t *s1, MsmState *state, uint32_t slots, uint32_t *segsums, uint32_t *segmaxs,
                 uint32_t *segtotal, uint32_t *hv, bool sliced, uint32_t *lane_heavy, uint32_t heavy_seq);
constexpr size_t SORT2_HV_WORDS = 2112;
constexpr size_t sort2_hv_bytes(int buckets_per_bin) { return (SORT2_HV_WORDS + (size_t)2560 * buckets_per_bin) * 4; }
int sort2_level2(kzg_ctx *ctx, hipStream_t st, int kind, const void *rec, const uint32_t *bin_base, const uint32_t *bin_total, uint32_t *hv,
                 uint32_t *entries, uint32_t *total, uint32_t *bucket_start, MsmState *state, uint32_t slots, bool sliced, uint32_t *lane_heavy,
                 uint32_t heavy_seq);

struct TailLayout {
    size_t off_dense, off_rows, off_cols, off_Q, off_tasks, off_arrive, off_result, bytes;
};
TailLayout tail_layout(int B, size_t T1_max);
int msm_tail_run(kzg_ctx *ctx, hipStream_t st, const MsmMode &mode, const MsmPoint *part, MsmPoint *scratch, const uint32_t *s1, int B,
                 size_t expected_partials, MsmState *state, char *tail_base, const TailLayout &L, MsmPoint **d_result,
                 bool odd_weights = false);

}
```

### kzg_amd/csrc/msm_tail.hip

```cpp
#include "msm_internal.h"

#if defined(KZG_TAIL_WAVES)
#define KZG_TAIL_LB __launch_bounds__(256, KZG_TAIL_WAVES)
#else
#define KZG_TAIL_LB __launch_bounds__(256)
#endif

namespace kzg {

constexpr int FOLD_SEQ = 8;
constexpr int OVF_SLICE = 512;

__device__ __forceinline__ MsmPoint shfl_xor_point(const MsmPoint &p, int mask) {
    MsmPoint r;
#pragma unroll
    for (int i = 0; i < F30_N; i++) {
        r.x.v[i] = __shfl_xor(p.x.v[i], mask, 64);
        r.y.v[i] = __shfl_xor(p.y.v[i], mask, 64);
        r.zz.v[i] = __shfl_xor(p.zz.v[i], mask, 64);
        r.zzz.v[i] = __shfl_xor(p.zzz.v[i], mask, 64);
    }
    r.inf = (uint32_t)__shfl_xor((int)p.inf, mask, 64);
    r.pad[0] = r.pad[1] = r.pad[2] = 0;
    return r;
}

template <int WIDTH>
__device__ __forceinline__ MsmPoint butterfly_sum(MsmPoint acc) {
#pragma nounroll
    for (int off = WIDTH / 2; off >= 1; off >>= 1) acc = g1_add30(acc, shfl_xor_point(acc, off));
    return acc;
}

__device__ __forceinline__ MsmPoint load_partial(const MsmPoint *part, uint32_t k) { return g1_partial_load30(part[k]); }

template <bool RAW>
__device__ __forceinline__ MsmPoint wave_sum(const MsmPoint *p, uint32_t lo, uint32_t hi, int lane) {
    MsmPoint acc = MsmPoint::infinity();
    for (uint32_t k = lo + (uint32_t)lane; k < hi; k += 64) acc = g1_add30(acc, RAW ? load_partial(p, k) : p[k]);
    return butterfly_sum<64>(acc);
}

template <int G>
__global__ KZG_TAIL_LB void k_fold_dense(const MsmPoint *part, const uint32_t *s1, int B, MsmPoint *dense, MsmState *st,
                                                    uint32_t *tasks, uint32_t *arrive) {
    KZG_SIDE_PRIO_STMT;
    const uint32_t gid = blockIdx.x * blockDim.x + threadIdx.x;
    const uint32_t b = gid / G, g = gid % G;
    if (b >= (uint32_t)B) return;
    const uint32_t s = s1[b], cnt = s1[b + 1] - s;
    if (cnt > (uint32_t)(FOLD_SEQ * G)) {
        if (g == 0) {
            const uint32_t nsl = (cnt + OVF_SLICE - 1) / OVF_SLICE;
            const uint32_t base = atomicAdd(&st->ovf_tasks, nsl);
            for (uint32_t k = 0; k < nsl; k++) tasks[base + k] = (b << 12) | k;
            arrive[b] = 0;
        }
        return;
    }
    MsmPoint acc = MsmPoint::infinity();
    for (uint32_t k = g; k < cnt; k += G) acc = g1_add30(acc, load_partial(part, s + k));
    acc = butterfly_sum<G>(acc);
    if (g == 0) dense[b] = acc;
}

__global__ KZG_TAIL_LB void k_fold_overflow(const MsmPoint *part, MsmPoint *scratch, const uint32_t *s1, MsmPoint *dense,
                                                       const MsmState *st, const uint32_t *tasks, uint32_t *arrive) {
    KZG_SIDE_PRIO_STMT;
    const uint32_t T = st->ovf_tasks;
    if (T == 0) return;
    const int lane = threadIdx.x & 63;
    const uint32_t wave = (blockIdx.x * blockDim.x + threadIdx.x) >> 6, nwaves = (gridDim.x * blockDim.x) >> 6;
    for (uint32_t t = wave; t < T; t += nwaves) {
        const uint32_t e = tasks[t], b = e >> 12, sl = e & 0xfffu;
        const uint32_t s0 = s1[b], cnt = s1[b + 1] - s0, nsl = (cnt + OVF_SLICE - 1) / OVF_SLICE;
        const uint32_t lo = s0 + sl * OVF_SLICE, end = s0 + cnt, hi = lo + OVF_SLICE < end ? lo + OVF_SLICE : end;
        MsmPoint acc = wave_sum<true>(part, lo, hi, lane);
        if (nsl == 1) {
            if (lane == 0) dense[b] = acc;
            continue;
        }
        if (lane == 0) scratch[s0 + sl] = acc;
        __threadfence();
        uint32_t old = 0;
        if (lane == 0) old = atomicAdd(&arrive[b], 1u);
        old = (uint32_t)__shfl((int)old, 0, 64);
        if (old == nsl - 1) {
            __threadfence();
            acc = wave_sum<false>(scratch, s0, s0 + nsl, lane);
            if (lane == 0) dense[b] = acc;
        }
    }
}

__global__ KZG_TAIL_LB void k_rc_sums(const MsmPoint *dense, int Rn, int Cn, MsmPoint *rows, MsmPoint *cols) {
    KZG_SIDE_PRIO_STMT;
    const int lane = threadIdx.x & 63;
    const int wv = (int)((blockIdx.x * blockDim.x + threadIdx.x) >> 6);
    if (wv >= Rn + Cn) return;
    MsmPoint acc = MsmPoint::infinity();
    if (wv < Rn) {
        const MsmPoint *row = dense + (size_t)wv * Cn;
        for (int c = lane; c < Cn; c += 64) acc = g1_add30(acc, row[c]);
    } else {
        const MsmPoint *col = dense + (wv - Rn);
        for (int r = lane; r < Rn; r += 64) acc = g1_add30(acc, col[(size_t)r * Cn]);
    }
    acc = butterfly_sum<64>(acc);
    if (lane == 0) (wv < Rn ? rows[wv] : cols[wv - Rn]) = acc;
}

constexpr int RC_LANES = 8;
__global__ KZG_TAIL_LB void k_rc_sums_t(const MsmPoint *dense, int Rn, int Cn, MsmPoint *rows, MsmPoint *cols) {
    KZG_SIDE_PRIO_STMT;
    const int gid = blockIdx.x * blockDim.x + threadIdx.x;
    const int sum = gid / RC_LANES, l = gid % RC_LANES;
    if (sum >= Rn + Cn) return;
    MsmPoint acc = MsmPoint::infinity();
    if (sum < Rn) {
        const MsmPoint *row = dense + (size_t)sum * Cn;
#pragma nounroll
        for (int c = l; c < Cn; c += RC_LANES) acc = g1_add30(acc, row[c]);
    } else {
        const MsmPoint *col = dense + (sum - Rn);
#pragma nounroll
        for (int r = l; r < Rn; r += RC_LANES) acc = g1_add30(acc, col[(size_t)r * Cn]);
    }
    acc = butterfly_sum<RC_LANES>(acc);
    if (l == 0) (sum < Rn ? rows[sum] : cols[sum - Rn]) = acc;
}

__global__ KZG_TAIL_LB void k_weighted_bits(const MsmPoint *rows, const MsmPoint *cols, int lr, int lc, MsmPoint *Q) {
    KZG_SIDE_PRIO_STMT;
    const int lane = threadIdx.x & 63;
    const int wv = (int)((blockIdx.x * blockDim.x + threadIdx.x) >> 6);
    if (wv > lr + lc) return;
    const MsmPoint *X = wv < lr ? rows : cols;
    const int size = wv < lr ? (1 << lr) : (1 << lc);
    const int j = wv < lr ? wv : (wv < lr + lc ? wv - lr : -1);
    MsmPoint acc = MsmPoint::infinity();
    if (j >= 0) {
        for (int t = lane; t < size / 2; t += 64) {
            const int i = ((t >> j) << (j + 1)) | (1 << j) | (t & ((1 << j) - 1));
            acc = g1_add30(acc, X[i]);
        }
    } else {
        for (int i = lane; i < size; i += 64) acc = g1_add30(acc, X[i]);
    }
    acc = butterfly_sum<64>(acc);
    if (lane == 0) Q[wv] = acc;
}

__global__ __launch_bounds__(64) void k_reduce_final(const MsmPoint *Q, int lr, int lc, MsmPoint *result, int odd) {
    KZG_SIDE_PRIO_STMT;
    const int lane = threadIdx.x;
    const int cnt = lr + lc + 1;
    MsmPoint p = lane < cnt ? Q[lane] : MsmPoint::infinity();
    const int shift = lane < lr ? lane + lc + odd : (lane < lr + lc ? lane - lr + odd : 0);
    const int maxshift = (lr > 0 ? lr + lc - 1 : (lc > 0 ? lc - 1 : 0)) + odd;
    for (int k = 0; k < maxshift; k++)
        if (k < shift && lane < cnt) p = g1_dbl30(p);
    p = butterfly_sum<32>(p);
    if (lane == 0) *result = p;
}

template <int SRC>
__device__ __forceinline__ Fq30 quad_bcast(const Fq30 &v) {
    Fq30 r;
#pragma unroll
    for (int i = 0; i < F30_N; i++) r.v[i] = __builtin_amdgcn_update_dpp(0, v.v[i], SRC * 0x55, 0xf, 0xf, false);
    return r;
}

__device__ __forceinline__ Fq30 sel4(int role, const Fq30 &a0, const Fq30 &a1, const Fq30 &a2, const Fq30 &a3) {
    Fq30 r;
#pragma unroll
    for (int i = 0; i < F30_N; i++) {
        int32_t v = a0.v[i];
        v = role == 1 ? a1.v[i] : v;
        v = role == 2 ? a2.v[i] : v;
        v = role == 3 ? a3.v[i] : v;
        r.v[i] = v;
    }
    return r;
}

__device__ __forceinline__ void quad_round(int role, const Fq30 &a0, const Fq30 &b0, const Fq30 &a1, const Fq30 &b1, const Fq30 &a2,
                                           const Fq30 &b2, const Fq30 &a3, const Fq30 &b3, Fq30 &p0, Fq30 &p1, Fq30 &p2, Fq30 &p3) {
    const Fq30 t = mul30(sel4(role, a0, a1, a2, a3), sel4(role, b0, b1, b2, b3));
    p0 = quad_bcast<0>(t);
    p1 = quad_bcast<1>(t);
    p2 = quad_bcast<2>(t);
    p3 = quad_bcast<3>(t);
}

__device__ __noinline__ void add_same_x(const MsmPoint *p, const MsmPoint *q, MsmPoint *r) { *r = g1_add30(*p, *q); }

__device__ __forceinline__ MsmPoint qdbl(const MsmPoint &p, int role) {
    if (p.inf) return p;
    const Fq30 U = times2_30(p.y);
    Fq30 V, XX, d2, d3;
    quad_round(role, U, U, p.x, p.x, U, U, p.x, p.x, V, XX, d2, d3);
    if (is_zero30(V)) return MsmPoint::infinity();
    const Fq30 Mm = times3_30(XX);
    Fq30 W, S, MM, ZZ3;
    quad_round(role, U, V, p.x, V, Mm, Mm, V, p.zz, W, S, MM, ZZ3);
    MsmPoint r;
    r.inf = 0;
    r.pad[0] = r.pad[1] = r.pad[2] = 0;
    r.x = sub30(MM, times2_30(S));
    Fq30 MY, WY, ZZZ3;
    quad_round(role, Mm, sub30(S, r.x), W, p.y, W, p.zzz, W, p.zzz, MY, WY, ZZZ3, d3);
    r.y = sub30(MY, WY);
    r.zz = ZZ3;
    r.zzz = ZZZ3;
    return r;
}

__device__ __forceinline__ MsmPoint qadd(const MsmPoint &p, const MsmPoint &q, int role) {
    if (q.inf) return p;
    if (p.inf) return q;
    Fq30 U1, U2, S1, S2;
    quad_round(role, p.x, q.zz, q.x, p.zz, p.y, q.zzz, q.y, p.zzz, U1, U2, S1, S2);
    const Fq30 Pp = sub30(U2, U1), R = sub30(S2, S1);
    Fq30 PP, RR, ZZ12, ZZZ12;
    quad_round(role, Pp, Pp, R, R, p.zz, q.zz, p.zzz, q.zzz, PP, RR, ZZ12, ZZZ12);
    if (is_zero30(PP)) {
        MsmPoint pc = p, qc = q, r;
        add_same_x(&pc, &qc, &r);
        return r;
    }
    Fq30 PPP, Q, ZZ3, d3;
    quad_round(role, Pp, PP, U1, PP, ZZ12, PP, ZZ12, PP, PPP, Q, ZZ3, d3);
    MsmPoint r;
    r.inf = 0;
    r.pad[0] = r.pad[1] = r.pad[2] = 0;
    r.x = sub30(RR, add2x30(PPP, Q));
    Fq30 Bm, RY, ZZZ3;
    quad_round(role, S1, PPP, R, sub30(Q, r.x), ZZZ12, PPP, ZZZ12, PPP, Bm, RY, ZZZ3, d3);
    r.y = sub30(RY, Bm);
    r.zz = ZZ3;
    r.zzz = ZZZ3;
    return r;
}

template <int QUADS>
__device__ __forceinline__ MsmPoint quad_butterfly(MsmPoint acc, int role) {
#pragma nounroll
    for (int off = QUADS / 2; off >= 1; off >>= 1) acc = qadd(acc, shfl_xor_point(acc, 4 * off), role);
    return acc;
}

template <int WAVES>
__device__ __forceinline__ MsmPoint block_quad_sum(MsmPoint acc, MsmPoint *lds, int role) {
    acc = quad_butterfly<16>(acc, role);
    if (WAVES == 1) return acc;
    const int lane = threadIdx.x & 63, wave = threadIdx.x >> 6, ql = lane >> 2;
    if (lane == 0) lds[wave] = acc;
    __syncthreads();
    MsmPoint t = ql < WAVES ? lds[ql] : MsmPoint::infinity();
    return quad_butterfly<WAVES>(t, role);
}

__global__ KZG_TAIL_LB void k_weighted_bits_q(const MsmPoint *rows, const MsmPoint *cols, int lr, int lc, MsmPoint *Q) {
    KZG_SIDE_PRIO_STMT;
    __shared__ MsmPoint lds[4];
    const int role = threadIdx.x & 3, qd = threadIdx.x >> 2;
    const int wv = blockIdx.x;
    const MsmPoint *X = wv < lr ? rows : cols;
    const int size = wv < lr ? (1 << lr) : (1 << lc);
    const int j = wv < lr ? wv : (wv < lr + lc ? wv - lr : -1);
    MsmPoint acc = MsmPoint::infinity();
    if (j >= 0) {
        for (int t = qd; t < size / 2; t += 64) {
            const int i = ((t >> j) << (j + 1)) | (1 << j) | (t & ((1 << j) - 1));
            acc = qadd(acc, X[i], role);
        }
    } else {
        for (int i = qd; i < size; i += 64) acc = qadd(acc, X[i], role);
    }
    acc = block_quad_sum<4>(acc, lds, role);
    if (threadIdx.x == 0) Q[wv] = acc;
}

__global__ __launch_bounds__(128) void k_reduce_final_q(const MsmPoint *Q, int lr, int lc, MsmPoint *result, int odd) {
    KZG_SIDE_PRIO_STMT;
    __shared__ MsmPoint lds[2];
    const int role = threadIdx.x & 3, qd = threadIdx.x >> 2;
    const int cnt = lr + lc + 1;
    MsmPoint p = qd < cnt ? Q[qd] : MsmPoint::infinity();
    const int shift = qd < lr ? qd + lc + odd : (qd < lr + lc ? qd - lr + odd : 0);
    const int maxshift = (lr > 0 ? lr + lc - 1 : (lc > 0 ? lc - 1 : 0)) + odd;
#pragma nounroll
    for (int k = 0; k < maxshift; k++)
        if (k < shift && qd < cnt) p = qdbl(p, role);
    p = block_quad_sum<2>(p, lds, role);
    if (threadIdx.x == 0) *result = p;
}

void tail_shape(int B, int *Rn, int *Cn, int *lr, int *lc) {
    int lb = 0;
    while ((1 << lb) < B) lb++;
    *lc = (lb + 1) / 2;
    *lr = lb - *lc;
    *Cn = 1 << *lc;
    *Rn = 1 << *lr;
}

TailLayout tail_layout(int B, size_t T1_max) {
    TailLayout L;
    size_t o = 0;
    auto take = [&](size_t bytes) {
        size_t r = o;
        o = align_up(o + bytes, 256);
        return r;
    };
    int Rn, Cn, lr, lc;
    tail_shape(B, &Rn, &Cn, &lr, &lc);
    L.off_dense = take((size_t)B * sizeof(MsmPoint));
    L.off_rows = take((size_t)Rn * sizeof(MsmPoint));
    L.off_cols = take((size_t)Cn * sizeof(MsmPoint));
    L.off_Q = take(32 * sizeof(MsmPoint));
    L.off_tasks = take((T1_max / OVF_SLICE + (size_t)B + 64) * 4);
    L.off_arrive = take((size_t)B * 4);
    L.off_result = take(sizeof(MsmPoint));
    L.bytes = o;
    return L;
}

int msm_tail_run(kzg_ctx *ctx, hipStream_t st, const MsmMode &mode, const MsmPoint *part, MsmPoint *scratch, const uint32_t *s1, int B,
                 size_t expected_partials, MsmState *state, char *tail_base, const TailLayout &L, MsmPoint **d_result, bool odd_weights) {
    MsmPoint *dense = (MsmPoint *)(tail_base + L.off_dense), *rows = (MsmPoint *)(tail_base + L.off_rows);
    MsmPoint *cols = (MsmPoint *)(tail_base + L.off_cols), *Q = (MsmPoint *)(tail_base + L.off_Q);
    uint32_t *tasks = (uint32_t *)(tail_base + L.off_tasks), *arrive = (uint32_t *)(tail_base + L.off_arrive);
    MsmPoint *result = (MsmPoint *)(tail_base + L.off_result);
    int Rn, Cn, lr, lc;
    tail_shape(B, &Rn, &Cn, &lr, &lc);
    size_t avg = expected_partials / (size_t)B + 1;
    int G = 1;
    if (!mode.tail_wide) {
        while (G < 64 && (size_t)G * 2 < avg) G *= 2;
    } else {
        while (G < 64 && (size_t)G * (FOLD_SEQ / 2) < avg) G *= 2;
    }
    const int wpb = TAIL_THREADS / 64;
    const unsigned grid = (unsigned)(((size_t)B * G + TAIL_THREADS - 1) / TAIL_THREADS);
#define KZG_FOLD(GG)                                                                                                      \
    case GG:                                                                                                              \
        KZG_LAUNCH(ctx, st, "k_fold_dense", k_fold_dense<GG>, grid, TAIL_THREADS, 0, part, s1, B, dense, state, tasks, arrive); \
        break;
    switch (G) {
        KZG_FOLD(1) KZG_FOLD(2) KZG_FOLD(4) KZG_FOLD(8) KZG_FOLD(16) KZG_FOLD(32) KZG_FOLD(64)
    }
#undef KZG_FOLD
    KZG_LAUNCH(ctx, st, "k_fold_overflow", k_fold_overflow, 256, TAIL_THREADS, 0, part, scratch, s1, dense, state, tasks, arrive);
    if (mode.tail_wide && Rn >= RC_LANES && Cn >= RC_LANES) {
        KZG_LAUNCH(ctx, st, "k_rc_sums", k_rc_sums_t, ((Rn + Cn) * RC_LANES + 255) / 256, 256, 0, dense, Rn, Cn, rows, cols);
    } else {
        KZG_LAUNCH(ctx, st, "k_rc_sums", k_rc_sums, (Rn + Cn + wpb - 1) / wpb, TAIL_THREADS, 0, dense, Rn, Cn, rows, cols);
    }
    if (mode.tail_quads) {
        KZG_LAUNCH(ctx, st, "k_weighted_bits", k_weighted_bits_q, lr + lc + 1, 256, 0, rows, cols, lr, lc, Q);
        KZG_LAUNCH(ctx, st, "k_reduce_final", k_reduce_final_q, 1, 128, 0, Q, lr, lc, result, odd_weights ? 1 : 0);
    } else {
        KZG_LAUNCH(ctx, st, "k_weighted_bits", k_weighted_bits, (lr + lc + 1 + wpb - 1) / wpb, TAIL_THREADS, 0, rows, cols, lr, lc, Q);
        KZG_LAUNCH(ctx, st, "k_reduce_final", k_reduce_final, 1, 64, 0, Q, lr, lc, result, odd_weights ? 1 : 0);
    }
    *d_result = result;
    return KZG_OK;
}

}
```

### kzg_amd/csrc/msm_wide.hip

```cpp
#include "msm_internal.h"
#include "msm_sort.h"

namespace kzg {


__device__ __forceinline__ void hi_thread_range(uint32_t M, uint32_t &p0, uint32_t &p1) {
    const uint32_t chunk = (M + HI_BLOCKS - 1) / HI_BLOCKS;
    const uint32_t run = (chunk + HI_THREADS - 1) / HI_THREADS;
    uint64_t b0 = (uint64_t)blockIdx.x * chunk;
    uint64_t b1 = b0 + chunk < M ? b0 + chunk : M;
    uint64_t q0 = b0 + (uint64_t)threadIdx.x * run;
    uint64_t q1 = q0 + run < b1 ? q0 + run : b1;
    if (q0 > b1) q0 = b1;
    p0 = (uint32_t)q0;
    p1 = (uint32_t)(q1 < q0 ? q0 : q1);
}

__global__ __launch_bounds__(HI_THREADS) void k_hi_count(const uint32_t *entries, const MsmState *st, int nhi, uint32_t *blockcnt) {
    __shared__ uint32_t cnt[16];
    if (threadIdx.x < 16) cnt[threadIdx.x] = 0;
    __syncthreads();
    uint32_t p0, p1;
    hi_thread_range(st->M, p0, p1);
    uint32_t mine[16];
// ... 214 lines not shown
    for (size_t i = i0 + threadIdx.x; i < i1; i += blockDim.x) {
        uint32_t s[8];
        load_scalar(scalars, i, sfmt, s);
        for_each_digit_fixed<SORT20_C, SORT20_W>(s, false, [&](int, uint32_t mag, uint32_t) { atomicAdd(&h[(mag - 1) >> SORT20_SHIFT], 1u); });
    }
    __syncthreads();
    for (int b = threadIdx.x; b < NBINS; b += blockDim.x) blk_bins[(size_t)blockIdx.x * NBINS + b] = h[b];
}

constexpr int BIN_SCATTER20_LDS = (3 * NBINS + 16) * 4 + SORT20_W * 1024 * 8;
__global__ __launch_bounds__(1024) void k_bin_scatter20(const Fr *scalars, size_t n, int sfmt, size_t per_block, const uint32_t *blk_off,
                                                        const uint32_t *bin_total, uint32_t *bin_base, uint32_t row_stride,
                                                        uint32_t idx_base, uint2 *rec) {
    uint32_t *cur = lds_u32, *cnt = cur + NBINS, *off = cnt + NBINS, *wsum = off + NBINS;
    uint2 *stage = reinterpret_cast<uint2 *>(wsum + 16);
    const uint32_t tid = threadIdx.x;
    {
        uint32_t tot;
        const uint32_t ex = block_scan_1024(bin_total[tid], wsum, &tot);
        cur[tid] = ex + blk_off[(size_t)blockIdx.x * NBINS + tid];
        if (blockIdx.x == 0) {
            bin_base[tid] = ex;
            if (tid == 0) bin_base[NBINS] = tot;
        }
    }
    const size_t i0 = (size_t)blockIdx.x * per_block;
    const size_t i1 = i0 + per_block < n ? i0 + per_block : n;
    for (size_t c0 = i0; c0 < i1; c0 += 1024) {
        cnt[tid] = 0;
        __syncthreads();
        uint2 pk[SORT20_W];
        uint32_t rk[SORT20_W], have = 0;
        if (c0 + tid < i1) {
            uint32_t s[8];
            load_scalar(scalars, c0 + tid, sfmt, s);
            const uint32_t e0 = idx_base + (uint32_t)c0 + tid;
            for_each_digit_fixed<SORT20_C, SORT20_W>(s, false, [&](int w, uint32_t mag, uint32_t neg) {
                const uint32_t idx = mag - 1, bin = idx >> SORT20_SHIFT;
                rk[w] = atomicAdd(&cnt[bin], 1u);
                pk[w] = make_uint2(((uint32_t)w * row_stride + e0) | (neg << 31), (idx & (SORT20_BUCKETS - 1)) | (bin << 16));
                have |= 1u << w;
            });
        }
        __syncthreads();
        uint32_t tot;
        off[tid] = block_scan_1024(cnt[tid], wsum, &tot);
        __syncthreads();
#pragma unroll
        for (int w = 0; w < SORT20_W; w++)
            if ((have >> w) & 1u) stage[off[pk[w].y >> 16] + rk[w]] = pk[w];
        __syncthreads();
        for (uint32_t p = tid; p < tot; p += 1024) {
            const uint2 v = stage[p];
            const uint32_t bin = v.y >> 16;
            rec[cur[bin] + p - off[bin]] = v;
        }
        __syncthreads();
        cur[tid] += cnt[tid];
    }
}

constexpr int SORT2_THREADS = 256, SORT2_UNROLL = 8, SORT2_CHUNK = SORT2_THREADS * SORT2_UNROLL;
#ifndef KZG_HEAVY_GRID
#define KZG_HEAVY_GRID 256
#endif
constexpr int HEAVY_MAX_SLICES = 2560, HEAVY_GRID = KZG_HEAVY_GRID, HEAVY_SCAN_GRID = 64;
static_assert(SORT2_HV_WORDS >= 2 + 2 * NBINS, "hv layout");

template <int NB>
__device__ __forceinline__ void sort2_scan(const uint32_t *h, uint32_t *off, uint32_t *sc) {
    static_assert(NB == 64 || NB == 512, "buckets per bin");
    const uint32_t tid = threadIdx.x;
    if (NB == 512) {
        const uint32_t v0 = h[2 * tid], v1 = h[2 * tid + 1];
        uint32_t tot;
        const uint32_t ex = block_scan_256(v0 + v1, sc, &tot);
        off[2 * tid] = ex;
        off[2 * tid + 1] = ex + v0;
    } else if (tid < NB) {
        const uint32_t v = h[tid];
        uint32_t incl = v;
#pragma unroll
        for (int o = 1; o < 64; o <<= 1) {
            const uint32_t u = __shfl_up(incl, o, 64);
            if ((int)tid >= o) incl += u;
        }
        off[tid] = incl - v;
    }
}

template <class REC, int NB>
__device__ __forceinline__ void sort2_count_range(const typename REC::T *rec, uint32_t a, uint32_t b, uint32_t *h) {
    typedef typename REC::T RT;
    const uint32_t tid = threadIdx.x;
    for (uint32_t k = tid; k < NB; k += SORT2_THREADS) h[k] = 0;
    __syncthreads();
    for (uint32_t base = a + tid; base < b; base += SORT2_CHUNK) {
        RT e[SORT2_UNROLL];
#pragma unroll
        for (int k = 0; k < SORT2_UNROLL; k++) {
            const uint32_t r = base + (uint32_t)k * SORT2_THREADS;
            e[k] = r < b ? rec[r] : REC::invalid();
        }
#pragma unroll
        for (int k = 0; k < SORT2_UNROLL; k++)
            if (REC::valid(e[k])) atomicAdd(&h[REC::lo(e[k])], 1u);
    }
    __syncthreads();
}

template <class REC, int NB>
__device__ __forceinline__ void sort2_place_range(const typename REC::T *rec, uint32_t c_begin, uint32_t c_end, uint32_t *entries,
                                                  uint32_t *h, uint32_t *cur, uint32_t *off, uint32_t *sc, typename REC::T *stage) {
    typedef typename REC::T RT;
    const uint32_t tid = threadIdx.x;
    for (uint32_t c0 = c_begin; c0 < c_end; c0 += SORT2_CHUNK) {
        for (uint32_t k = tid; k < NB; k += SORT2_THREADS) h[k] = 0;
        __syncthreads();
        RT e[SORT2_UNROLL];
        uint32_t rk[SORT2_UNROLL];
#pragma unroll
        for (int k = 0; k < SORT2_UNROLL; k++) {
            const uint32_t r = c0 + tid + (uint32_t)k * SORT2_THREADS;
            e[k] = r < c_end ? rec[r] : REC::invalid();
        }
#pragma unroll
        for (int k = 0; k < SORT2_UNROLL; k++)
            if (REC::valid(e[k])) rk[k] = atomicAdd(&h[REC::lo(e[k])], 1u);
        __syncthreads();
        sort2_scan<NB>(h, off, sc);
        __syncthreads();
#pragma unroll
        for (int k = 0; k < SORT2_UNROLL; k++)
            if (REC::valid(e[k])) stage[off[REC::lo(e[k])] + rk[k]] = e[k];
        __syncthreads();
        const uint32_t m = c_end - c0 < (uint32_t)SORT2_CHUNK ? c_end - c0 : (uint32_t)SORT2_CHUNK;
        for (uint32_t p = tid; p < m; p += SORT2_THREADS) {
            const RT v = stage[p];
            const uint32_t b = REC::lo(v);
            entries[cur[b] + p - off[b]] = REC::entry(v);
        }
        __syncthreads();
        for (uint32_t k = tid; k < NB; k += SORT2_THREADS) cur[k] += h[k];
    }
}

__device__ __forceinline__ uint32_t heavy_slice_len(uint32_t M) {
    const uint32_t SL = (M + 2047) / 2048;
    return SL < 32768u ? 32768u : SL;
}
__device__ __forceinline__ uint32_t heavy_slices(uint32_t size, uint32_t SL) { return size > 4 * SL ? (size + SL - 1) / SL : 0u; }

template <class REC, int NB>
__global__ __launch_bounds__(SORT2_THREADS) void k_bin_sort2(const typename REC::T *rec, const uint32_t *bin_base, uint32_t *entries,
                                                             uint32_t *total, uint32_t *bucket_start, MsmState *st, uint32_t slots,
                                                             int sliced, uint32_t *lane_heavy, uint32_t heavy_seq) {
    typedef typename REC::T RT;
    __shared__ uint32_t h[NB], cur[NB], off[NB], sc[4];
    __shared__ RT stage[SORT2_CHUNK];
    const uint32_t tid = threadIdx.x;
    const uint32_t r0 = bin_base[blockIdx.x], r1 = bin_base[blockIdx.x + 1];
    if (st && blockIdx.x == 0 && tid == 0) {
        const uint32_t M = bin_base[NBINS];
        uint32_t E = (M + slots - 1) / slots;
        if (E < KZG_ACCUM_MIN_CHUNK) E = KZG_ACCUM_MIN_CHUNK;
        st->M = M;
        st->E = E;
        st->ntasks = (M + E - 1) / E;
        st->ovf_tasks = 0;
        bucket_start[(size_t)NBINS * NB] = M;
    }
    if (heavy_slices(r1 - r0, heavy_slice_len(bin_base[NBINS]))) {
        if (tid == 0) *lane_heavy = heavy_seq;
        if (sliced) return;
    }
    sort2_count_range<REC, NB>(rec, r0, r1, h);
    sort2_scan<NB>(h, off, sc);
    __syncthreads();
    for (uint32_t k = tid; k < NB; k += SORT2_THREADS) {
        const uint32_t start = r0 + off[k];
        cur[k] = start;
        if (total) total[(size_t)blockIdx.x * NB + k] = h[k];
        if (bucket_start) bucket_start[(size_t)blockIdx.x * NB + k] = start;
    }
    sort2_place_range<REC, NB>(rec, r0, r1, entries, h, cur, off, sc, stage);
}

__device__ __forceinline__ uint32_t heavy_bin_of(const uint32_t *hv, uint32_t id) {
    uint32_t lo = 0, hi = NBINS;
    while (hi - lo > 1) {
        const uint32_t mid = (lo + hi) >> 1;
        if (hv[2 + mid] <= id) lo = mid; else hi = mid;
    }
    return lo;
}

template <class REC, int NB>
__global__ __launch_bounds__(SORT2_THREADS) void k_heavy_count(const typename REC::T *rec, const uint32_t *bin_base, uint32_t *hv,
                                                               uint32_t *hcnt) {
    __shared__ uint32_t h[NB], plan[2 + 2 * NBINS], sc[4];
    const uint32_t tid = threadIdx.x;
    {
        const uint32_t SL = heavy_slice_len(bin_base[NBINS]);
        uint32_t ns[4], sum = 0;
#pragma unroll
        for (int k = 0; k < 4; k++) {
            const uint32_t bin = 4 * tid + k;
            ns[k] = heavy_slices(bin_base[bin + 1] - bin_base[bin], SL);
            sum += ns[k];
        }
        uint32_t tot;
        uint32_t run = block_scan_256(sum, sc, &tot);
#pragma unroll
        for (int k = 0; k < 4; k++) {
            plan[2 + 4 * tid + k] = run;
            plan[2 + NBINS + 4 * tid + k] = ns[k];
            run += ns[k];
        }
        if (tid == 0) {
            plan[0] = tot;
            plan[1] = SL;
        }
        __syncthreads();
        if (blockIdx.x == 0)
            for (uint32_t k = tid; k < 2 + 2 * NBINS; k += SORT2_THREADS) hv[k] = plan[k];
    }
    const uint32_t total = plan[0], SL = plan[1];
    for (uint32_t id = blockIdx.x; id < total; id += gridDim.x) {
        const uint32_t bin = heavy_bin_of(plan, id), j = id - plan[2 + bin];
        const uint32_t r0 = bin_base[bin], r1 = bin_base[bin + 1];
        const uint32_t a = r0 + j * SL, b = a + SL < r1 ? a + SL : r1;
        sort2_count_range<REC, NB>(rec, a, b, h);
        for (uint32_t k = tid; k < NB; k += SORT2_THREADS) hcnt[(size_t)id * NB + k] = h[k];
        __syncthreads();
    }
}

template <int NB>
__global__ __launch_bounds__(NB) void k_heavy_scan(const uint32_t *bin_base, const uint32_t *hv, uint32_t *hcnt, uint32_t *total,
                                                   uint32_t *bucket_start) {
    __shared__ uint32_t ws[8];
    if (hv[0] == 0) return;
    for (uint32_t bin = blockIdx.x; bin < NBINS; bin += gridDim.x) {
    const uint32_t ns = hv[2 + NBINS + bin];
    if (ns == 0) continue;
    const uint32_t s0 = hv[2 + bin], b = threadIdx.x;
    uint32_t run = 0, j = 0;
    for (; j + 8 <= ns; j += 8) {
        uint32_t t[8];
#pragma unroll
        for (int k = 0; k < 8; k++) t[k] = hcnt[(size_t)(s0 + j + k) * NB + b];
#pragma unroll
        for (int k = 0; k < 8; k++) {
            hcnt[(size_t)(s0 + j + k) * NB + b] = run;
            run += t[k];
        }
    }
    for (; j < ns; j++) {
        const uint32_t t = hcnt[(size_t)(s0 + j) * NB + b];
        hcnt[(size_t)(s0 + j) * NB + b] = run;
        run += t;
    }
    const int lane = threadIdx.x & 63, wave = threadIdx.x >> 6;
    uint32_t incl = run;
#pragma unroll
    for (int o = 1; o < 64; o <<= 1) {
        uint32_t u = __shfl_up(incl, o, 64);
        if (lane >= o) incl += u;
    }
    if (lane == 63) ws[wave] = incl;
    __syncthreads();
    uint32_t woff = 0;
#pragma unroll
    for (int w = 0; w < NB / 64; w++)
        if (w < wave) woff += ws[w];
    if (total) total[(size_t)bin * NB + b] = run;
    bucket_start[(size_t)bin * NB + b] = bin_base[bin] + woff + incl - run;
    __syncthreads();
    }
}

template <class REC, int NB>
__global__ __launch_bounds__(SORT2_THREADS) void k_heavy_place(const typename REC::T *rec, const uint32_t *bin_base, const uint32_t *hv,
                                                               const uint32_t *hcnt, const uint32_t *bucket_start, uint32_t *entries) {
    typedef typename REC::T RT;
    __shared__ uint32_t h[NB], cur[NB], off[NB], sc[4];
    __shared__ RT stage[SORT2_CHUNK];
    const uint32_t total = hv[0], SL = hv[1], tid = threadIdx.x;
    for (uint32_t id = blockIdx.x; id < total; id += gridDim.x) {
        const uint32_t bin = heavy_bin_of(hv, id), j = id - hv[2 + bin];
        const uint32_t r0 = bin_base[bin], r1 = bin_base[bin + 1];
        const uint32_t a = r0 + j * SL, b = a + SL < r1 ? a + SL : r1;
        for (uint32_t k = tid; k < NB; k += SORT2_THREADS) cur[k] = bucket_start[(size_t)bin * NB + k] + hcnt[(size_t)id * NB + k];
        sort2_place_range<REC, NB>(rec, a, b, entries, h, cur, off, sc, stage);
        __syncthreads();
    }
}

int wide_sort_pass2(kzg_ctx *ctx, hipStream_t st, const uint32_t *entries1, const MsmState *state, int nhi, uint32_t *blockcnt,
                    uint32_t *binbase, const uint32_t *lo_start, int B_lo, uint32_t *entries2, uint32_t *bucket_start) {
    if (!ctx->attr_wide_set) {
        KZG_HIP_CHECK(ctx, hipFuncSetAttribute((const void *)k_hi_scatter, hipFuncAttributeMaxDynamicSharedMemorySize, 16 * HI_THREADS * 4));
        ctx->attr_wide_set = true;
    }
    KZG_HIP_CHECK(ctx, hipMemsetAsync(bucket_start, 0, ((size_t)nhi * B_lo + 1) * 4, st));
    KZG_LAUNCH(ctx, st, "k_hi_count", k_hi_count, HI_BLOCKS, HI_THREADS, 0, entries1, state, nhi, blockcnt);
    KZG_LAUNCH(ctx, st, "k_hi_scan", k_hi_scan, 1, 1024, 0, blockcnt, nhi, binbase);
    KZG_LAUNCH(ctx, st, "k_hi_scatter", k_hi_scatter, HI_BLOCKS, HI_THREADS, 16 * HI_THREADS * 4, entries1, state, nhi, binbase,
               lo_start, B_lo, entries2, bucket_start);
    return KZG_OK;
}

int sort20_hist(kzg_ctx *ctx, hipStream_t st, const void *d_scalars, size_t n, int sfmt, int G2, uint32_t *bins) {
    const size_t per2 = (n + G2 - 1) / G2;
    KZG_LAUNCH(ctx, st, "k_bin_hist", k_bin_hist20, G2, 1024, 0, (const Fr *)d_scalars, n, sfmt, per2, bins);
    return KZG_OK;
}

template <class REC, int NB>
static int sort2_level2_t(kzg_ctx *ctx, hipStream_t st, const void *rec_v, const uint32_t *bin_base, uint32_t *hv, uint32_t *entries,
                          uint32_t *total, uint32_t *bucket_start, MsmState *state, uint32_t slots, bool sliced, uint32_t *lane_heavy,
                          uint32_t heavy_seq) {
    typedef typename REC::T RT;
    const RT *rec = (const RT *)rec_v;
    uint32_t *hcnt = hv + SORT2_HV_WORDS;
    KZG_LAUNCH(ctx, st, "k_bin_sort", (k_bin_sort2<REC, NB>), NBINS, SORT2_THREADS, 0, rec, bin_base, entries, total,
               state ? bucket_start : nullptr, state, slots, sliced ? 1 : 0, lane_heavy, heavy_seq);
    if (!sliced) return KZG_OK;
    KZG_LAUNCH(ctx, st, "k_heavy_count", (k_heavy_count<REC, NB>), HEAVY_GRID, SORT2_THREADS, 0, rec, bin_base, hv, hcnt);
    KZG_LAUNCH(ctx, st, "k_heavy_scan", k_heavy_scan<NB>, HEAVY_SCAN_GRID, NB, 0, bin_base, hv, hcnt, total, bucket_start);
    KZG_LAUNCH(ctx, st, "k_heavy_place", (k_heavy_place<REC, NB>), HEAVY_GRID, SORT2_THREADS, 0, rec, bin_base, hv, hcnt, bucket_start,
               entries);
    return KZG_OK;
}

int sort2_level2(kzg_ctx *ctx, hipStream_t st, int kind, const void *rec, const uint32_t *bin_base, const uint32_t *bin_total, uint32_t *hv,
                 uint32_t *entries, uint32_t *total, uint32_t *bucket_start, MsmState *state, uint32_t slots, bool sliced, uint32_t *lane_heavy,
                 uint32_t heavy_seq) {
    (void)bin_total;
    if (kind == 4) return sort2_level2_t<Rec4, 64>(ctx, st, rec, bin_base, hv, entries, total, bucket_start, nullptr, slots, sliced, lane_heavy, heavy_seq);
    if (kind == 8) return sort2_level2_t<Rec8, 64>(ctx, st, rec, bin_base, hv, entries, total, bucket_start, nullptr, slots, sliced, lane_heavy, heavy_seq);
    return sort2_level2_t<Rec20, SORT20_BUCKETS>(ctx, st, rec, bin_base, hv, entries, nullptr, bucket_start, state, slots, sliced, lane_heavy, heavy_seq);
}

int sort20_place(kzg_ctx *ctx, hipStream_t st, const void *d_scalars, size_t n, int sfmt, int G2, const uint32_t *bins,
                 const uint32_t *bin_total, uint32_t *bin_base, uint32_t row_stride, uint32_t idx_base, void *rec, uint32_t *entries,
                 uint32_t *bucket_start, uint32_t *s1, MsmState *state, uint32_t slots, uint32_t *segsums, uint32_t *segmaxs,
                 uint32_t *segtotal, uint32_t *hv, bool sliced, uint32_t *lane_heavy, uint32_t heavy_seq) {
    if (!ctx->attr_sort20_set) {
        KZG_HIP_CHECK(ctx, hipFuncSetAttribute((const void *)k_bin_scatter20, hipFuncAttributeMaxDynamicSharedMemorySize, BIN_SCATTER20_LDS));
        ctx->attr_sort20_set = true;
    }
    const size_t per2 = (n + G2 - 1) / G2;
    KZG_LAUNCH(ctx, st, "k_bin_scatter", k_bin_scatter20, G2, 1024, BIN_SCATTER20_LDS, (const Fr *)d_scalars, n, sfmt, per2, bins, bin_total,
               bin_base, row_stride, idx_base, (uint2 *)rec);
    KZG_TRY(sort2_level2(ctx, st, 20, rec, bin_base, bin_total, hv, entries, nullptr, bucket_start, state, slots, sliced, lane_heavy, heavy_seq));
    return wide_s1_layout(ctx, st, bucket_start, NBINS * SORT20_BUCKETS, state, segsums, segmaxs, segtotal, s1);
}

int wide_s1_layout(kzg_ctx *ctx, hipStream_t st, const uint32_t *bucket_start, int Btot, MsmState *state, uint32_t *segsums,
                   uint32_t *segmaxs, uint32_t *segtotal, uint32_t *s1_out) {
    const int nseg = (Btot + SEG - 1) / SEG;
    ScanS1 f{bucket_start, state};
    KZG_LAUNCH(ctx, st, "k_seg_sums", k_seg_sums<ScanS1>, nseg, 256, 0, f, Btot, state, 0, segsums, segmaxs);
    KZG_LAUNCH(ctx, st, "k_seg_top", k_seg_top, 1, 256, 0, segsums, segmaxs, nseg, 0, state, 0u, 0u, segtotal);
    KZG_LAUNCH(ctx, st, "k_seg_apply", k_seg_apply<ScanS1>, nseg, 256, 0, f, Btot, state, 0, segsums, segtotal, s1_out);
    KZG_LAUNCH(ctx, st, "k_s1_finish", k_s1_finish, (Btot + 1 + 255) / 256, 256, 0, bucket_start, Btot, state, s1_out);
    return KZG_OK;
}

}
```

### kzg_amd/csrc/runtime.hip

```cpp
#include <dlfcn.h>

#include <algorithm>

#include "common.h"

namespace kzg {

int lane_reserve(kzg_ctx *ctx, int lane, size_t bytes) {
    Lane &l = ctx->lanes[lane];
    bytes = align_up(bytes + 4096, 1 << 20);
    if (l.arena_bytes < bytes) {
        KZG_HIP_CHECK(ctx, hipStreamSynchronize(l.stream));
        if (l.arena) KZG_HIP_CHECK(ctx, hipFree(l.arena));
        l.arena = nullptr;
        l.arena_bytes = 0;
        hipError_t e = hipMalloc((void **)&l.arena, bytes);
        if (e != hipSuccess) return fail(ctx, KZG_ERR_ALLOC, std::string("hipMalloc(workspace): ") + hipGetErrorString(e));
        l.arena_bytes = bytes;
    }
    l.arena_used = 0;
    return KZG_OK;
}

void *lane_alloc(kzg_ctx *ctx, int lane, size_t bytes) {
    Lane &l = ctx->lanes[lane];
    size_t off = align_up(l.arena_used, 256);
    if (off + bytes > (l.arena_limit ? std::min(l.arena_limit, l.arena_bytes) : l.arena_bytes)) return nullptr;
    l.arena_used = off + bytes;
    return l.arena + off;
}

int lane_pinned(kzg_ctx *ctx, int lane, size_t bytes) {
    Lane &l = ctx->lanes[lane];
    if (l.pinned_bytes >= bytes) return KZG_OK;
    if (l.pinned) hipHostFree(l.pinned);
    l.pinned = nullptr;
    l.pinned_bytes = 0;
    bytes = align_up(bytes, 4096);
    KZG_HIP_CHECK(ctx, hipHostMalloc((void **)&l.pinned, bytes, hipHostMallocDefault));
    l.pinned_bytes = bytes;
    return KZG_OK;
}

static hipEvent_t get_event(kzg_ctx *ctx) {
    if (!ctx->event_pool.empty()) {
        hipEvent_t e = ctx->event_pool.back();
        ctx->event_pool.pop_back();
        return e;
    }
    hipEvent_t e = nullptr;
    hipEventCreate(&e);
    return e;
}

ProfScope::ProfScope(kzg_ctx *c, hipStream_t s, const char *n) : ctx(c), stream(s), name(n) {
    if (!ctx->prof) return;
    if (ctx->prof_only_accum && strcmp(n, "k_accum_affine") != 0) return;
    {
        std::lock_guard<std::mutex> lk(ctx->prof_mu);
        start = get_event(ctx);
        stop = get_event(ctx);
    }
    hipEventRecord(start, stream);
}

ProfScope::~ProfScope() {
    if (!start) return;
    hipEventRecord(stop, stream);
    std::lock_guard<std::mutex> lk(ctx->prof_mu);
    ctx->prof_pending.push_back(PendingEvent{name, start, stop});
}

void prof_collect(kzg_ctx *ctx) {
    std::vector<PendingEvent> pend;
    {
        std::lock_guard<std::mutex> lk(ctx->prof_mu);
        pend.swap(ctx->prof_pending);
    }
    std::vector<float> ms(pend.size(), -1.f);
    for (size_t i = 0; i < pend.size(); i++) {
        hipEventSynchronize(pend[i].stop);
        float t = 0.f;
        if (hipEventElapsedTime(&t, pend[i].start, pend[i].stop) == hipSuccess) ms[i] = t;
    }
    std::lock_guard<std::mutex> lk(ctx->prof_mu);
    for (size_t i = 0; i < pend.size(); i++) {
        if (ms[i] >= 0.f) {
            ProfEntry &e = ctx->prof_map[pend[i].name];
            e.launches++;
            e.total_ms += ms[i];
        }
        ctx->event_pool.push_back(pend[i].start);
        ctx->event_pool.push_back(pend[i].stop);
    }
}

}

using namespace kzg;

extern "C" const char *kzg_version(void) { return "kzg-mi355x 0.1.0 (gfx950)"; }

extern "C" int kzg_init_hw_queues(int queues) {
    if (queues < 0 || queues > 64) return KZG_ERR_SHAPE;
    char buf[16];
    snprintf(buf, sizeof buf, "%d", queues ? queues : 24);
    return setenv("GPU_MAX_HW_QUEUES", buf, 0) == 0 ? KZG_OK : KZG_ERR_INTERNAL;
}
__attribute__((constructor)) static void kzg_optional_hw_queues() {
    const char *e = getenv("KZG_SET_HW_QUEUES");
    if (e && atoi(e) > 0) kzg_init_hw_queues(atoi(e) == 1 ? 0 : atoi(e));
}

extern "C" int kzg_runtime_info(char *buf, size_t buflen) {
    if (!buf || !buflen) return KZG_ERR_SHAPE;
    Dl_info di;
    const char *file = "?";
    if (dladdr((const void *)&hipStreamSynchronize, &di) && di.dli_fname) file = di.dli_fname;
    int rt = 0, drv = 0;
    hipRuntimeGetVersion(&rt);
    hipDriverGetVersion(&drv);
    snprintf(buf, buflen, "hip=%s runtime_version=%d driver_version=%d", file, rt, drv);
    return KZG_OK;
}

extern "C" int kzg_ctx_info(kzg_ctx *ctx, char *buf, size_t buflen) {
    if (!ctx || !buf || !buflen) return KZG_ERR_SHAPE;
    Guard g(ctx);
    char nf[32] = "none";
    if (ctx->plan_lanes < ctx->plan_want_lanes || ctx->plan_accum < ctx->plan_want_accum)
        snprintf(nf, sizeof nf, "%d+%d", ctx->plan_want_lanes, ctx->plan_want_accum);
    snprintf(buf, buflen, "device=%d lanes=%d accum_streams=%d hw_queues_found=%d narrowed_from=%s witness_cache_slots=%d", ctx->device,
             ctx->plan_lanes, ctx->plan_accum, ctx->plan_queues, nf, ctx->opt_witness_cache_slots);
    return KZG_OK;
}

extern "C" int kzg_device_count(void) {
    int count = 0;
    if (hipGetDeviceCount(&count) != hipSuccess || count < 0) return 0;
    return count;
}

namespace kzg {
struct StreamPool {
    std::mutex mu;
    std::vector<hipStream_t> lanes;
    hipStream_t accum[4] = {nullptr, nullptr, nullptr, nullptr};
    std::map<hipStream_t, int> cls;
    int refs = 0;
};
static std::mutex g_pools_mu;
static std::map<int, StreamPool *> g_pools;
static StreamPool *pool_for(int device) {
    std::lock_guard<std::mutex> lk(g_pools_mu);
    auto it = g_pools.find(device);
    if (it != g_pools.end()) return it->second;
    StreamPool *p = new StreamPool();
    g_pools[device] = p;
    return p;
}
static void pool_ref(StreamPool *p) {
    std::lock_guard<std::mutex> lk(p->mu);
    p->refs++;
}
static void pool_unref(StreamPool *p) {
    std::lock_guard<std::mutex> lk(p->mu);
    if (--p->refs > 0) return;
    for (auto st : p->lanes) hipStreamDestroy(st);
    for (auto &st : p->accum)
        if (st) {
            hipStreamDestroy(st);
            st = nullptr;
        }
    p->lanes.clear();
    p->cls.clear();
}
static hipError_t pool_lane(StreamPool *p, int i, hipStream_t *out) {
    std::lock_guard<std::mutex> lk(p->mu);
    while ((int)p->lanes.size() <= i) {
        hipStream_t st = nullptr;
        hipError_t e = hipStreamCreateWithFlags(&st, hipStreamNonBlocking);
        if (e != hipSuccess) return e;
        p->lanes.push_back(st);
    }
    *out = p->lanes[i];
    return hipSuccess;
}
static hipError_t pool_accum(StreamPool *p, int i, hipStream_t *out) {
    std::lock_guard<std::mutex> lk(p->mu);
    if (!p->accum[i]) {
        hipError_t e = hipStreamCreateWithFlags(&p->accum[i], hipStreamNonBlocking);
        if (e != hipSuccess) return e;
    }
    *out = p->accum[i];
    return hipSuccess;
}
}

extern "C" int kzg_ctx_create(int device, kzg_ctx **out) {
    if (!out) return KZG_ERR_SHAPE;
    int count = 0;
    if (hipGetDeviceCount(&count) != hipSuccess || count <= 0 || device < 0 || device >= count) return KZG_ERR_NO_DEVICE;
    if (hipSetDevice(device) != hipSuccess) return KZG_ERR_NO_DEVICE;
    kzg_ctx *ctx = new kzg_ctx();
    ctx->device = device;
    hipDeviceProp_t prop;
    if (hipGetDeviceProperties(&prop, device) == hipSuccess) ctx->num_cus = prop.multiProcessorCount;
    ctx->lanes.reserve(KZG_MAX_LANES);
    ctx->lanes.resize(1);
    ctx->pool = pool_for(device);
    pool_ref(ctx->pool);
    if (pool_lane(ctx->pool, 0, &ctx->lanes[0].stream) != hipSuccess) {
        pool_unref(ctx->pool);
        delete ctx;
        return KZG_ERR_HIP;
    }
    if (hipMalloc((void **)&ctx->d_lane_heavy, KZG_MAX_LANES * 4) != hipSuccess ||
        hipMemset(ctx->d_lane_heavy, 0, KZG_MAX_LANES * 4) != hipSuccess) {
        if (ctx->d_lane_heavy) hipFree(ctx->d_lane_heavy);
        pool_unref(ctx->pool);
        delete ctx;
        return KZG_ERR_ALLOC;
    }
    *out = ctx;
    return KZG_OK;
}

int kzg::ensure_lanes(kzg_ctx *ctx, int want) {
    if (want > KZG_MAX_LANES) return fail(ctx, KZG_ERR_INTERNAL, "lane count");
    while ((int)ctx->lanes.size() < want) {
        Lane l;
        KZG_HIP_CHECK(ctx, pool_lane(ctx->pool, (int)ctx->lanes.size(), &l.stream));
        ctx->lanes.push_back(l);
    }
    return KZG_OK;
}

extern "C" void kzg_ctx_destroy(kzg_ctx *ctx) {
    if (!ctx) return;
    hipSetDevice(ctx->device);
    for (auto &l : ctx->lanes) {
        if (l.stream) hipStreamSynchronize(l.stream);
        if (l.arena) hipFree(l.arena);
        if (l.pinned) hipHostFree(l.pinned);
    }
    for (auto e : ctx->event_pool) hipEventDestroy(e);
    for (auto e : ctx->sorted_events) hipEventDestroy(e);
    for (auto e : ctx->accum_events) hipEventDestroy(e);
    if (ctx->batch_out) hipFree(ctx->batch_out);
    if (ctx->d_lane_heavy) hipFree(ctx->d_lane_heavy);
    for (auto &ct : ctx->coset_tabs)
        if (ct.second) hipFree(ct.second);
    ntt_plans_free(ctx);
    eval_tabs_free(ctx);
    fixed_base_free(ctx);
    point_sets_free(ctx);
    for (auto st : ctx->accum_streams)
        if (st) hipStreamSynchronize(st);
    pool_unref(ctx->pool);
    delete ctx;
}

extern "C" const char *kzg_last_error(kzg_ctx *ctx) {
    if (!ctx) return "null context";
    static thread_local std::string tl_err;
    ThreadErr &te = thread_err();
    if (te.ctx == ctx) {
        tl_err = te.msg;
    } else {
        std::lock_guard<std::mutex> lk(ctx->err_mu);
        tl_err = ctx->err;
    }
    return tl_err.c_str();
}

extern "C" int kzg_sync(kzg_ctx *ctx) {
    if (!ctx) return KZG_ERR_SHAPE;
    Guard g(ctx);
    KZG_HIP_CHECK(ctx, hipSetDevice(ctx->device));
    for (auto &l : ctx->lanes) KZG_HIP_CHECK(ctx, hipStreamSynchronize(l.stream));
    return KZG_OK;
}

extern "C" int kzg_ctx_set_option(kzg_ctx *ctx, const char *key, int64_t value) {
    if (!ctx || !key) return KZG_ERR_SHAPE;
    Guard g(ctx);
    std::string k(key);
    if (k == "window_bits") {
        if (value != 0 && (value < 4 || value > 20)) return fail(ctx, KZG_ERR_SHAPE, "window_bits must be 0 or 4..20");
        ctx->opt_window_bits = (int)value;
    } else if (k == "streams") {
        if (value < 1 || value > 16) return fail(ctx, KZG_ERR_SHAPE, "streams must be 1..16");
        ctx->opt_streams = (int)value;
        ctx->pipe_planned = false;
    } else if (k == "accum_blocks" || k == "accum_blocks_batch") {
        if (value != 0 && (value < 64 || value > 256 * KZG_ACCUM_WAVES))
            return fail(ctx, KZG_ERR_SHAPE, "accum_blocks must be 0 (auto) or 64..256 x waves per SIMD");
        (k == "accum_blocks" ? ctx->opt_accum_blocks : ctx->opt_accum_blocks_batch) = (int)value;
    } else if (k == "scan_threads" || k == "scan_threads_batch") {
    } else if (k == "sort_threads" || k == "sort_threads_batch") {
        if (value != 256 && value != 512 && value != 1024) return fail(ctx, KZG_ERR_SHAPE, "sort_threads must be 256, 512 or 1024");
        (k == "sort_threads" ? ctx->opt_sort_threads : ctx->opt_sort_threads_batch) = (int)value;
    } else if (k == "accum_streams") {
        if (value < 0 || value > 4) return fail(ctx, KZG_ERR_SHAPE, "accum_streams must be 0..4");
        ctx->opt_accum_streams = (int)value;
        ctx->pipe_planned = false;
    } else if (k == "accum_streams_small") {
        if (value < 0 || value > 4) return fail(ctx, KZG_ERR_SHAPE, "accum_streams_small must be 0..4");
        ctx->opt_accum_streams_small = (int)value;
        ctx->pipe_planned = false;
    } else if (k == "accum_blocks_small") {
        if (value != 0 && (value < 64 || value > 256 * KZG_ACCUM_WAVES)) return fail(ctx, KZG_ERR_SHAPE, "accum_blocks_small must be 0 (off) or 64..256 x waves per SIMD");
        ctx->opt_accum_blocks_small = (int)value;
        ctx->pipe_planned = false;
    } else if (k == "small_entries") {
        if (value < 0) return fail(ctx, KZG_ERR_SHAPE, "small_entries must be >= 0");
        ctx->opt_small_entries = value;
    } else if (k == "host_affine") {
        ctx->opt_host_affine = value != 0;
    } else if (k == "host_pairing") {
        ctx->opt_host_pairing = value != 0;
    } else if (k == "heavy_bins") {
        if (value < 0 || value > 2) return fail(ctx, KZG_ERR_SHAPE, "heavy_bins: 0 (adaptive), 1 (always slice oversized sort bins), 2 (never)");
        ctx->opt_heavy_bins = (int)value;
        ctx->heavy_last.store(0, std::memory_order_relaxed);
    } else if (k == "sort_single_pass") {
        ctx->opt_sort_single = value != 0;
    } else if (k == "defer_tail") {
        ctx->opt_no_defer_tail = value == 0;
    } else if (k == "tail_quads") {
        ctx->opt_tail_quads = value != 0;
    } else if (k == "hw_queues") {
        if (value < 0 || value > 64) return fail(ctx, KZG_ERR_SHAPE, "hw_queues must be 0 (GPU_MAX_HW_QUEUES or the ROCm default of 4) or 1..64");
        ctx->opt_hw_queues = (int)value;
        ctx->pipe_planned = false;
    } else if (k == "window_rows") {
        if (value < 0 || value > 64) return fail(ctx, KZG_ERR_SHAPE, "window_rows must be 0 (one table row per window) or 1..64");
        ctx->opt_window_rows = (int)value;
    } else if (k == "naf_window") {
        if (value != 0 && value != 18) return fail(ctx, KZG_ERR_SHAPE, "naf_window must be 0 (window tables) or 18 (positional tables, width-18 NAF digits)");
        ctx->opt_naf_window = (int)value;
    } else if (k == "trusted_points") {
        ctx->opt_trusted_points = value != 0;
    } else if (k == "witness_cache_slots") {
        if (value < 0 || value > 256) return fail(ctx, KZG_ERR_SHAPE, "witness_cache_slots must be 0..256");
        if (ctx->point_sets) return fail(ctx, KZG_ERR_SHAPE, "witness_cache_slots: the cache already exists (set the option before the first create_witness_batched)");
        ctx->opt_witness_cache_slots = (int)value;
    } else if (k == "ntt_xcd") {
        if (value < 0 || value > 3) return fail(ctx, KZG_ERR_SHAPE, "ntt_xcd must be 0..3");
        ctx->opt_ntt_xcd = (int)value;
    } else if (k == "ntt_kernel") {
        if (value < 0 || value > 2) return fail(ctx, KZG_ERR_SHAPE, "ntt_kernel must be 0..2");
        ctx->opt_ntt_kernel = (int)value;
    } else if (k == "ntt_three_from") {
        if (value != 0 && (value < 20 || value > 24)) return fail(ctx, KZG_ERR_SHAPE, "ntt_three_from must be 0 (never) or 20..24");
        ctx->opt_ntt_three_from = (int)value;
    } else if (k == "ntt_vec2_log") {
        if (value < 0 || value > 2) return fail(ctx, KZG_ERR_SHAPE, "ntt_vec2_log must be 0..2");
        ctx->opt_ntt_vec2_log = (int)value;
    } else if (k == "fk20_cosets_combine") {
        if (value != 0 && value != 1) return fail(ctx, KZG_ERR_SHAPE, "fk20_cosets_combine must be 0 (Straus) or 1 (per term)");
        ctx->opt_fk20_cosets_combine = (int)value;
    } else if (k == "verify_cosets_chunk") {
        if (value < 0 || value > (1 << 20)) return fail(ctx, KZG_ERR_SHAPE, "verify_cosets_chunk must be 0 (the rule alone) or 1..2^20 cells");
        ctx->opt_verify_cosets_chunk = (int)value;
    } else if (k == "verify_eval_batch_chunk") {
        if (value < 0 || value > 16384) return fail(ctx, KZG_ERR_SHAPE, "verify_eval_batch_chunk must be 0 (16384 openings) or 1..16384 openings");
        ctx->opt_verify_eval_batch_chunk = (int)value;
    } else if (k == "multiopen_points_chunk") {
        if (value < 0 || value > 16) return fail(ctx, KZG_ERR_SHAPE, "multiopen_points_chunk must be 0 (min(16, 2^22 / d) points) or 1..16 points");
        ctx->opt_multiopen_points_chunk = (int)value;
    } else if (k == "multi_eval_segment") {
        if (value != 0 && (value < 8 || value > (1 << 28) || (value & (value - 1)))) return fail(ctx, KZG_ERR_SHAPE, "multi_eval_segment must be 0 (auto) or a power of two in 8..2^28");
        ctx->opt_multi_eval_segment = (int)value;
    } else if (k == "multi_eval_points_chunk") {
        if (value < 0 || value > (1 << 30)) return fail(ctx, KZG_ERR_SHAPE, "multi_eval_points_chunk must be 0 (auto) or 1..2^30 points");
        ctx->opt_multi_eval_points_chunk = (int)value;
    } else if (k == "poly_divide_base") {
        if (value != 0 && (value < 1 || value > 64 || (value & (value - 1)))) return fail(ctx, KZG_ERR_SHAPE, "poly_divide_base must be 0 (64) or a power of two in 1..64");
        ctx->opt_poly_divide_base = (int)value;
    } else if (k == "point_tree_leaf") {
        if (value != 0 && (value < 1 || value > 16 || (value & (value - 1)))) return fail(ctx, KZG_ERR_SHAPE, "point_tree_leaf must be 0 (16) or a power of two in 1..16");
        ctx->opt_point_tree_leaf = (int)value;
    } else if (k == "ntt_vec_log") {
        if (value < 0 || value > 2) return fail(ctx, KZG_ERR_SHAPE, "ntt_vec_log must be 0..2");
        ctx->opt_ntt_vec_log = (int)value;
    } else {
        return fail(ctx, KZG_ERR_SHAPE, "unknown option " + k);
    }
    return KZG_OK;
}

extern "C" int kzg_dev_alloc(kzg_ctx *ctx, size_t bytes, void **out) {
    if (!ctx || !out) return KZG_ERR_SHAPE;
    KZG_HIP_CHECK(ctx, hipSetDevice(ctx->device));
    hipError_t e = hipMalloc(out, bytes ? bytes : 16);
    if (e != hipSuccess) return fail(ctx, KZG_ERR_ALLOC, hipGetErrorString(e));
    return KZG_OK;
}
extern "C" int kzg_dev_free(kzg_ctx *ctx, void *p) {
    if (!ctx) return KZG_ERR_SHAPE;
    Guard g(ctx);
    KZG_HIP_CHECK(ctx, hipSetDevice(ctx->device));
    for (auto &l : ctx->lanes) hipStreamSynchronize(l.stream);
    if (p) KZG_HIP_CHECK(ctx, hipFree(p));
    return KZG_OK;
}
extern "C" int kzg_dev_upload(kzg_ctx *ctx, void *dst_dev, const void *src_host, size_t bytes) {
    if (!ctx) return KZG_ERR_SHAPE;
    KZG_HIP_CHECK(ctx, hipSetDevice(ctx->device));
    if (bytes) KZG_HIP_CHECK(ctx, hipMemcpy(dst_dev, src_host, bytes, hipMemcpyHostToDevice));
    return KZG_OK;
}
extern "C" int kzg_dev_download(kzg_ctx *ctx, void *dst_host, const void *src_dev, size_t bytes) {
    if (!ctx) return KZG_ERR_SHAPE;
    KZG_HIP_CHECK(ctx, hipSetDevice(ctx->device));
    if (bytes) KZG_HIP_CHECK(ctx, hipMemcpy(dst_host, src_dev, bytes, hipMemcpyDeviceToHost));
    return KZG_OK;
}

extern "C" int kzg_prof_enable(kzg_ctx *ctx, int on) {
    if (!ctx) return KZG_ERR_SHAPE;
    Guard g(ctx);
    ctx->prof = on != 0;
    ctx->prof_only_accum = on == 2;
    return KZG_OK;
}
extern "C" int kzg_prof_reset(kzg_ctx *ctx) {
    if (!ctx) return KZG_ERR_SHAPE;
    Guard g(ctx);
    prof_collect(ctx);
    ctx->prof_map.clear();
    return KZG_OK;
}
extern "C" int kzg_prof_get(kzg_ctx *ctx, const char *kernel, uint64_t *launches, double *total_ms) {
    if (!ctx || !kernel) return KZG_ERR_SHAPE;
    if (!strcmp(kernel, "point_set_cache")) {
        uint64_t h = 0, m = 0;
        point_set_stats(ctx, &h, &m);
        if (launches) *launches = h;
        if (total_ms) *total_ms = (double)m;
        return KZG_OK;
    }
    Guard g(ctx);
    prof_collect(ctx);
    auto it = ctx->prof_map.find(kernel);
    if (launches) *launches = it == ctx->prof_map.end() ? 0 : it->second.launches;
    if (total_ms) *total_ms = it == ctx->prof_map.end() ? 0.0 : it->second.total_ms;
    return KZG_OK;
}
extern "C" int kzg_prof_names(kzg_ctx *ctx, char *buf, size_t buflen) {
    if (!ctx || !buf || !buflen) return KZG_ERR_SHAPE;
    Guard g(ctx);
    prof_collect(ctx);
    std::string s;
    for (auto &kv : ctx->prof_map) {
        if (!s.empty()) s += ",";
        s += kv.first;
    }
    snprintf(buf, buflen, "%s", s.c_str());
    return KZG_OK;
}

__global__ __launch_bounds__(256) void k_mad_issue_rate(uint32_t *out, int iters, uint32_t seed) {
    int32_t a = (int32_t)(seed + threadIdx.x), b = (int32_t)(seed * 3 + blockIdx.x);
    uint64_t c0 = a, c1 = b, c2 = a ^ b, c3 = a + b, c4 = a * 3, c5 = b * 5, c6 = a * 7, c7 = b * 9;
    for (int i = 0; i < iters; i++) {
#define KZG_M(c) asm volatile("v_mad_i64_i32 %0, vcc, %1, %2, %0" : "+v"(c) : "v"(a), "v"(b) : "vcc");
        KZG_M(c0) KZG_M(c1) KZG_M(c2) KZG_M(c3) KZG_M(c4) KZG_M(c5) KZG_M(c6) KZG_M(c7)
#undef KZG_M
    }
    uint64_t s = c0 ^ c1 ^ c2 ^ c3 ^ c4 ^ c5 ^ c6 ^ c7;
    out[blockIdx.x * blockDim.x + threadIdx.x] = (uint32_t)s ^ (uint32_t)(s >> 32);
}

extern "C" int kzg_measure_mad_issue_rate(kzg_ctx *ctx, int waves_per_simd, double *tera_lane_mads_per_s) {
    if (!ctx || !tera_lane_mads_per_s || waves_per_simd < 1 || waves_per_simd > 8) return KZG_ERR_SHAPE;
    Guard g(ctx);
    KZG_HIP_CHECK(ctx, hipSetDevice(ctx->device));
    const int blocks = ctx->num_cus * waves_per_simd, iters = 25000 * waves_per_simd;
    KZG_TRY(lane_reserve(ctx, 0, (size_t)blocks * 256 * 4 + 4096));
    uint32_t *out = (uint32_t *)lane_alloc(ctx, 0, (size_t)blocks * 256 * 4);
    if (!out) return fail(ctx, KZG_ERR_ALLOC, "workspace");
    hipStream_t st = ctx->lanes[0].stream;
    hipEvent_t e0, e1;
    KZG_HIP_CHECK(ctx, hipEventCreate(&e0));
    KZG_HIP_CHECK(ctx, hipEventCreate(&e1));
    hipLaunchKernelGGL(k_mad_issue_rate, dim3(blocks), dim3(256), 0, st, out, iters / 4, 7u);
// ... 46 lines not shown
        {
            Guard ex(ctx);
            rc = hipSetDevice(ctx->device) == hipSuccess ? KZG_OK : fail(ctx, KZG_ERR_HIP, "hipSetDevice");
            if (rc == KZG_OK && !ctx->pipe_planned) rc = plan_for_callers(ctx);
        }
        if (rc != KZG_OK) return rc;
        lk.lock();
    }
    const int others = g.shared_active;
    int lane = 0;
    if (ctx->pipe_planned)
        while (lane < ctx->pipe_lanes && (g.lane_busy >> lane & 1u)) lane++;
    g.lane_busy |= 1u << lane;
    g.shared_active++;
    ls->ctx = ctx;
    ls->lane = lane;
    const bool pipelined = others > 0 && ctx->pipe_planned;
    set_lane_mode(ctx, lane, pipelined, others >= 3);
    if (pipelined && ctx->pipe_accum > 0) {
        ls->pipelined = true;
        ls->slot = ctx->accum_rr.fetch_add(1);
    }
    return KZG_OK;
}

int kzg::accum_streams_for(kzg_ctx *ctx, int planned, const kzg_srs *srs, size_t n) {
    if (planned <= 0) return 1;
    if (ctx->msm_small((size_t)srs->W * n)) return planned;
    return planned < ctx->opt_accum_streams ? planned : (ctx->opt_accum_streams > 0 ? ctx->opt_accum_streams : 1);
}

int kzg::lease_msm(kzg_ctx *ctx, const Lease &ls, const kzg_srs *srs, size_t offset, const void *d_sc, size_t n, int sfmt, MsmPoint **res) {
    if (ls.pipelined) {
        hipStream_t accum = ctx->accum_streams[ls.slot % (uint32_t)accum_streams_for(ctx, ctx->pipe_accum, srs, n)];
        return msm_run(ctx, ls.lane, srs, offset, d_sc, n, sfmt, res, accum, ctx->sorted_events[ls.lane], ctx->accum_events[ls.lane]);
    }
    return msm_run(ctx, ls.lane, srs, offset, d_sc, n, sfmt, res);
}

__global__ void k_probe_spin(unsigned long long ticks, unsigned long long *out) {
    const unsigned long long t0 = wall_clock64();
    while (wall_clock64() - t0 < ticks) {
    }
    *out = wall_clock64();
}
__global__ void k_probe_mark(unsigned long long *out) { *out = wall_clock64(); }

static int probe_queues(kzg_ctx *ctx, int nl, int nas) {
    std::vector<hipStream_t *> ss;
    for (int l = 0; l < nl; l++) ss.push_back(&ctx->lanes[l].stream);
    for (int i = 0; i < nas; i++) ss.push_back(&ctx->accum_streams[i]);
    const size_t K = ss.size();
    std::vector<int> cls(K, -1);
    int ncls = 0;
    std::unique_lock<std::mutex> plk(ctx->pool->mu);
    bool known = !ctx->pool->cls.empty();
    for (size_t t = 0; t < K && known; t++)
        if (!ctx->pool->cls.count(*ss[t])) known = false;
    if (known) {
        std::map<int, int> remap;
        for (size_t t = 0; t < K; t++) {
            const int c = ctx->pool->cls[*ss[t]];
            if (!remap.count(c)) remap[c] = ncls++;
            cls[t] = remap[c];
        }
    }
    unsigned long long *d = nullptr;
    if (!known) KZG_HIP_CHECK(ctx, hipMalloc((void **)&d, K * sizeof(unsigned long long)));
    std::vector<unsigned long long> h(K);
    for (size_t s0 = 0; s0 < K && !known; s0++) {
        if (cls[s0] != -1) continue;
        cls[s0] = ncls;
        hipLaunchKernelGGL(k_probe_spin, dim3(1), dim3(1), 0, *ss[s0], 30000ull, d + s0);
        for (size_t t = s0 + 1; t < K; t++)
            if (cls[t] == -1) hipLaunchKernelGGL(k_probe_mark, dim3(1), dim3(1), 0, *ss[t], d + t);
        for (size_t t = s0; t < K; t++) KZG_HIP_CHECK(ctx, hipStreamSynchronize(*ss[t]));
        KZG_HIP_CHECK(ctx, hipMemcpy(h.data(), d, K * sizeof(unsigned long long), hipMemcpyDeviceToHost));
        for (size_t t = s0 + 1; t < K; t++)
            if (cls[t] == -1 && h[t] >= h[s0]) cls[t] = ncls;
        ncls++;
    }
    if (!known) {
        hipFree(d);
        ctx->pool->cls.clear();
        for (size_t t = 0; t < K; t++) ctx->pool->cls[*ss[t]] = cls[t];
    }
    plk.unlock();
    std::vector<hipStream_t> order;
    std::vector<bool> seen(ncls, false);
    for (size_t t = 0; t < K; t++)
        if (!seen[cls[t]]) {
            seen[cls[t]] = true;
            order.push_back(*ss[t]);
        }
    std::vector<bool> seen2(ncls, false);
    for (size_t t = 0; t < K; t++) {
        if (seen2[cls[t]]) order.push_back(*ss[t]);
        seen2[cls[t]] = true;
    }
    ctx->probed_queues = ncls;
    ctx->probed_order = order;
    if (getenv("KZG_DEBUG")) fprintf(stderr, "kzg: probe_queues: %zu streams on %d hardware queues\n", K, ncls);
    return KZG_OK;
}

void kzg::set_lane_mode(kzg_ctx *ctx, int lane, bool pipelined, bool deep) {
    MsmMode &m = ctx->lanes[lane].mode;
    m.accum_blocks = pipelined ? ctx->accum_blocks_batch() : ctx->accum_blocks_single();
    m.sort_threads = pipelined ? ctx->opt_sort_threads_batch : ctx->opt_sort_threads;
    m.tail_quads = pipelined ? false : ctx->opt_tail_quads != 0;
    m.tail_wide = pipelined && deep;
}

int kzg::plan_pipeline(kzg_ctx *ctx, int want, int *nl_out, int *nas_out) {
    int nl = want, nas = want > 1 ? ctx->opt_accum_streams : 0;
    if (nas > 0 && ctx->opt_accum_blocks_small > 0 && ctx->opt_accum_streams_small > nas) nas = ctx->opt_accum_streams_small;
    const int want_nl = nl, want_nas = nas;
    int found_queues = 0;
    if (want > 1) {
        KZG_TRY(ensure_lanes(ctx, want));
        for (int i = 0; i < nas; i++)
            if (!ctx->accum_streams[i]) KZG_HIP_CHECK(ctx, pool_accum(ctx->pool, i, &ctx->accum_streams[i]));
        int queues = ctx->opt_hw_queues;
        if (queues <= 0) {
            if (ctx->probed_queues == 0 || ctx->probed_lanes < want || ctx->probed_accum < nas) {
                KZG_TRY(probe_queues(ctx, want, nas));
                ctx->probed_lanes = want;
                ctx->probed_accum = nas;
            }
            queues = ctx->probed_queues;
        }
        found_queues = queues;
        if (nl + nas > queues) {
            if (queues >= 4) {
                nas = nas ? (queues >= 6 && nas >= 2 ? 2 : 1) : 0;
                nl = queues - nas;
            } else {
                nas = 0;
                nl = queues > 0 ? queues : 1;
            }
            if (nl > want) nl = want;
        }
        if (ctx->opt_hw_queues <= 0 && (int)ctx->probed_order.size() == ctx->probed_lanes + ctx->probed_accum &&
            nl <= ctx->probed_lanes && nas <= ctx->probed_accum) {
            for (auto &l : ctx->lanes) KZG_HIP_CHECK(ctx, hipStreamSynchronize(l.stream));
            size_t r = 0;
            for (int l = 0; l < nl; l++) ctx->lanes[l].stream = ctx->probed_order[r++];
            for (int i = 0; i < nas; i++) ctx->accum_streams[i] = ctx->probed_order[r++];
            for (int l = nl; l < ctx->probed_lanes; l++) ctx->lanes[l].stream = ctx->probed_order[r++];
            for (int i = nas; i < ctx->probed_accum; i++) ctx->accum_streams[i] = ctx->probed_order[r++];
            ctx->pipe_planned = false;
        }
    }
    if (getenv("KZG_DEBUG")) fprintf(stderr, "kzg: pipeline plan: %d lanes + %d accumulation streams\n", nl, nas);
    if (want > 1) {
        ctx->plan_want_lanes = want_nl, ctx->plan_want_accum = want_nas, ctx->plan_lanes = nl, ctx->plan_accum = nas, ctx->plan_queues = found_queues;
        if ((nl < want_nl || nas < want_nas) && !ctx->plan_warned) {
            ctx->plan_warned = true;
            fprintf(stderr, "kzg: device %d: this context's %d + %d streams found only %d hardware queues of their own (other streams of the "
                            "process hold the rest: another context, an RCCL communicator, the host's); the batched pipeline is narrowed to %d "
                            "lanes + %d accumulation streams -- expect 10-25 %% less batched throughput from THIS context.  Create contexts before "
                            "communicators, give the process more queues (kzg_init_hw_queues / GPU_MAX_HW_QUEUES before the first HIP call) or set "
                            "option \"streams\" explicitly; kzg_ctx_info reports the plan.\n",
                    ctx->device, want_nl, want_nas, found_queues, nl, nas);
        }
    }
    KZG_TRY(ensure_lanes(ctx, nl));
    while (nas && (int)ctx->sorted_events.size() < 2 * nl) {
        hipEvent_t e1 = nullptr, e2 = nullptr;
        KZG_HIP_CHECK(ctx, hipEventCreateWithFlags(&e1, hipEventDisableTiming));
        KZG_HIP_CHECK(ctx, hipEventCreateWithFlags(&e2, hipEventDisableTiming));
        ctx->sorted_events.push_back(e1);
        ctx->accum_events.push_back(e2);
    }
    ctx->planned_accum = nas;
    *nl_out = nl;
    *nas_out = nas;
    return KZG_OK;
}
```

Baseline: 466.5 commitments/s.

## Group batched MSMs into shared sort/tail launches across four streams

Adds a grouped path for kzg_msm_g1_batch. Up to 16 MSMs share a single launch of each sort and tail kernel, using a device table of per-MSM slots indexed by blockIdx.y. The work is pipelined on four fixed streams (sort, two accumulation, tail) with event dependencies and double-buffered slot arenas. The goal is to cut per-MSM launch and host scheduling overhead and the dependence on many hardware queues, at the cost of a larger arena, extra code paths, and one heavy-bucket readback per batch.

New measurement: 486.2 commitments/s, median of 6. +4.2%, better.

```diff
diff --git a/kzg_amd/csrc/capi.hip b/kzg_amd/csrc/capi.hip
--- a/kzg_amd/csrc/capi.hip
+++ b/kzg_amd/csrc/capi.hip
@@ -215,9 +215,91 @@
     return rc;
 }
 
+static bool batch_wants_group(kzg_ctx *ctx, const kzg_srs *srs, size_t n, size_t batch) {
+    if (ctx->plan_group <= 0 || batch < 2 || !msm_group_covers(ctx, srs, n)) return false;
+    if (ctx->opt_heavy_bins == 1) return false;
+    const uint64_t now = ctx->msm_count.load(std::memory_order_relaxed) + 1, last = ctx->heavy_last.load(std::memory_order_relaxed);
+    return !(ctx->opt_heavy_bins == 0 && last != 0 && now - last <= (uint64_t)KZG_HEAVY_WINDOW);
+}
+
+static int msm_batch_grouped(kzg_ctx *ctx, const BatchPipe &bp, const kzg_srs *srs, size_t offset, const void *scalars, size_t n,
+                             size_t batch, size_t stride_bytes, int sfmt, int flags, size_t psz, int ofmt) {
+    const size_t G = (size_t)ctx->plan_group, ngroups = (batch + G - 1) / G;
+    const size_t ws = align_up(msm_workspace_bytes(srs, n), 256);
+    const size_t per = align_up(ws + stage_bytes(n * 32, flags) + 8192, 4096);
+    const size_t D = KZG_GROUP_DEPTH, nslots = std::min(batch, D * G);
+    hipStream_t s_sort = ctx->lanes[0].stream, s_tail = ctx->lanes[1].stream;
+    hipStream_t s_acc[2] = {ctx->accum_streams[0], bp.nas >= 2 ? ctx->accum_streams[1] : ctx->lanes[2].stream};
+    while (ctx->group_events.size() < 4 * D) {
+        hipEvent_t e = nullptr;
+        KZG_HIP_CHECK(ctx, hipEventCreateWithFlags(&e, hipEventDisableTiming));
+        ctx->group_events.push_back(e);
+    }
+    hipEvent_t *ev = ctx->group_events.data();
+    if (ctx->group_tab_count < batch) {
+        if (ctx->group_tab) hipFree(ctx->group_tab);
+        ctx->group_tab = nullptr;
+        ctx->group_tab_count = 0;
+        KZG_HIP_CHECK(ctx, hipMalloc((void **)&ctx->group_tab, batch * sizeof(GroupSlot)));
+        ctx->group_tab_count = batch;
+    }
+    KZG_TRY(lane_reserve(ctx, 0, nslots * per + 4096));
+    ctx->lanes[0].arena_limit = 0;
+    char *arena = (char *)lane_alloc(ctx, 0, nslots * per);
+    if (!arena) return fail(ctx, KZG_ERR_ALLOC, "group arena not reserved");
+    std::vector<GroupSlot> tab(batch);
+    for (size_t b = 0; b < batch; b++) {
+        const size_t slot = ((b / G) % D) * G + b % G;
+        GroupSlot &t = tab[b];
+        t.base = arena + slot * per;
+        t.scalars = (flags & KZG_IN_DEVICE) ? (const void *)((const uint8_t *)scalars + b * stride_bytes) : (const void *)(t.base + ws);
+        t.out = bp.d_out + b * psz;
+        t.heavy = ctx->d_lane_heavy + KZG_MAX_LANES + slot;
+    }
+    KZG_HIP_CHECK(ctx, hipMemcpy(ctx->group_tab, tab.data(), batch * sizeof(GroupSlot), hipMemcpyHostToDevice));
+    const uint32_t seq = ++ctx->group_heavy_seq;
+    ctx->msm_count.fetch_add(batch, std::memory_order_relaxed);
+    auto enqueue = [&]() -> int {
+    for (size_t g = 0; g < ngroups; g++) {
+        const size_t b0 = g * G, cnt = std::min(G, batch - b0), h = g % D;
+        const GroupSlot *d_tab = ctx->group_tab + b0;
+        if (g >= D) KZG_HIP_CHECK(ctx, hipStreamWaitEvent(s_sort, ev[4 * h + 3], 0));
+        if (!(flags & KZG_IN_DEVICE))
+            for (size_t i = 0; i < cnt; i++)
+                KZG_HIP_CHECK(ctx, hipMemcpyAsync(tab[b0 + i].base + ws, (const uint8_t *)scalars + (b0 + i) * stride_bytes, n * 32,
+                                                  hipMemcpyHostToDevice, s_sort));
+        KZG_TRY(msm_group_sort(ctx, s_sort, srs, offset, n, sfmt, d_tab, (int)cnt, seq));
+        KZG_HIP_CHECK(ctx, hipEventRecord(ev[4 * h], s_sort));
+        const int na = cnt > 1 ? 2 : 1;
+        for (int a = 0; a < na; a++) KZG_HIP_CHECK(ctx, hipStreamWaitEvent(s_acc[a], ev[4 * h], 0));
+        for (size_t i = 0; i < cnt; i++) KZG_TRY(msm_group_accum(ctx, s_acc[i & 1], srs, n, tab[b0 + i].base));
+        for (int a = 0; a < na; a++) {
+            KZG_HIP_CHECK(ctx, hipEventRecord(ev[4 * h + 1 + a], s_acc[a]));
+            KZG_HIP_CHECK(ctx, hipStreamWaitEvent(s_tail, ev[4 * h + 1 + a], 0));
+        }
+        KZG_TRY(msm_group_tail(ctx, s_tail, srs, n, d_tab, (int)cnt, ofmt));
+        KZG_HIP_CHECK(ctx, hipEventRecord(ev[4 * h + 3], s_tail));
+    }
+    return KZG_OK;
+    };
+    const int rc = enqueue();
+    if (rc != KZG_OK) {
+        for (hipStream_t st : {s_sort, s_acc[0], s_acc[1], s_tail}) hipStreamSynchronize(st);
+        return rc;
+    }
+#if !defined(KZG_TIMING_NO_PICKUP)
+    KZG_HIP_CHECK(ctx, hipStreamSynchronize(s_tail));
+    uint32_t hv[KZG_GROUP_DEPTH * KZG_MAX_GROUP];
+    KZG_HIP_CHECK(ctx, hipMemcpy(hv, ctx->d_lane_heavy + KZG_MAX_LANES, sizeof hv, hipMemcpyDeviceToHost));
+    for (size_t k = 0; k < nslots; k++)
+        if (hv[k] == seq) ctx->heavy_last.store(ctx->msm_count.load(std::memory_order_relaxed), std::memory_order_relaxed);
+#endif
+    return KZG_OK;
+}
+
 namespace kzg {
 int msm_batch_strided(kzg_ctx *ctx, const kzg_srs *srs, size_t offset, const void *scalars, size_t n, size_t batch,
-                      size_t stride_bytes, int sfmt, int flags, void *out, int ofmt) {
+                      size_t stride_bytes, int sfmt, int flags, void *out, int ofmt, bool may_group) {
     Guard g(ctx);
     KZG_HIP_CHECK(ctx, hipSetDevice(ctx->device));
     KZG_TRY(check_sfmt(ctx, sfmt));
@@ -227,6 +309,8 @@
     if (batch == 0) return KZG_OK;
     BatchPipe bp;
     KZG_TRY(batch_begin(ctx, batch, batch * psz, out, flags, &bp));
+    if (may_group && batch_wants_group(ctx, srs, n, batch))
+        return batch_end(ctx, bp, msm_batch_grouped(ctx, bp, srs, offset, scalars, n, batch, stride_bytes, sfmt, flags, psz, ofmt), out, batch * psz);
     size_t per = align_up(msm_workspace_bytes(srs, n) + stage_bytes(n * 32, flags) + 8192, 4096);
     int rc = KZG_OK;
     const bool defer = bp.nas > 0 && batch > (size_t)bp.nl && !ctx->opt_no_defer_tail;
@@ -268,7 +352,7 @@
                                 size_t batch, int sfmt, int flags, void *out, int ofmt) {
     if (!ctx || !srs || !out || (!scalars && n && batch)) return KZG_ERR_SHAPE;
     if (n > SIZE_MAX / 32) return KZG_ERR_SHAPE;
-    return msm_batch_strided(ctx, srs, offset, scalars, n, batch, n * 32, sfmt, flags, out, ofmt);
+    return msm_batch_strided(ctx, srs, offset, scalars, n, batch, n * 32, sfmt, flags, out, ofmt, true);
 }
 
 extern "C" int kzg_witness_coeff_many(kzg_ctx *ctx, const kzg_srs *srs, const void *coeffs, size_t n, const void *xs,
diff --git a/kzg_amd/csrc/common.h b/kzg_amd/csrc/common.h
--- a/kzg_amd/csrc/common.h
+++ b/kzg_amd/csrc/common.h
@@ -81,6 +81,9 @@
 };
 constexpr int KZG_HEAVY_WINDOW = 64;
 constexpr int KZG_MAX_LANES = 24;
+constexpr int KZG_MAX_GROUP = 16;
+constexpr int KZG_GROUP_DEPTH = 2;
+struct GroupSlot;
 
 }
 
@@ -149,7 +152,7 @@
     int accum_blocks_single() const { return opt_accum_blocks ? opt_accum_blocks : 256 * KZG_ACCUM_WAVES; }
     int accum_blocks_batch() const { return opt_accum_blocks_batch ? opt_accum_blocks_batch : 240 * KZG_ACCUM_WAVES; }
     int num_cus = 256;
-    std::atomic<bool> attr_msm_set{false}, attr_ntt_set{false}, attr_wide_set{false}, attr_sort20_set{false}, attr_horner_set{false};
+    std::atomic<bool> attr_msm_set{false}, attr_ntt_set{false}, attr_wide_set{false}, attr_sort20_set{false}, attr_horner_set{false}, attr_group_set{false};
     bool prof = false;
     bool prof_only_accum = false;
     std::map<std::string, kzg::ProfEntry> prof_map;
@@ -163,6 +166,12 @@
     int opt_witness_cache_slots = 16;
     std::atomic<uint64_t> msm_count{0}, heavy_last{0};
     uint32_t *d_lane_heavy = nullptr;
+    int opt_group_msms = 16;
+    int plan_group = 0;
+    kzg::GroupSlot *group_tab = nullptr;
+    size_t group_tab_count = 0;
+    std::vector<hipEvent_t> group_events;
+    uint32_t group_heavy_seq = 0;
     void *batch_out = nullptr;
     size_t batch_out_bytes = 0;
 };
@@ -286,6 +295,17 @@
             MsmPoint **d_result, hipStream_t accum_stream = nullptr, hipEvent_t sorted_ev = nullptr, hipEvent_t accum_ev = nullptr,
             MsmPending *defer = nullptr);
 int msm_finish(kzg_ctx *ctx, MsmPending &pd, MsmPoint **d_result);
+struct GroupSlot {
+    const void *scalars;
+    char *base;
+    void *out;
+    uint32_t *heavy;
+};
+bool msm_group_covers(const kzg_ctx *ctx, const kzg_srs *srs, size_t n);
+int msm_group_sort(kzg_ctx *ctx, hipStream_t st, const kzg_srs *srs, size_t offset, size_t n, int sfmt, const GroupSlot *d_tab, int cnt,
+                   uint32_t heavy_seq);
+int msm_group_accum(kzg_ctx *ctx, hipStream_t st, const kzg_srs *srs, size_t n, char *base);
+int msm_group_tail(kzg_ctx *ctx, hipStream_t st, const kzg_srs *srs, size_t n, const GroupSlot *d_tab, int cnt, int ofmt);
 int lease_msm(kzg_ctx *ctx, const Lease &ls, const kzg_srs *srs, size_t offset, const void *d_sc, size_t n, int sfmt, MsmPoint **res);
 int sum_points_run(kzg_ctx *ctx, int lane, MsmPoint *d_points, size_t count, MsmPoint *d_scratch, MsmPoint **d_result);
 int points_to30(kzg_ctx *ctx, hipStream_t st, const G1Xyzz *d_in, MsmPoint *d_out, size_t n);
@@ -298,7 +318,7 @@
                     MsmPoint *d_tmp, void *d_out, int ofmt);
 
 int msm_batch_strided(kzg_ctx *ctx, const kzg_srs *srs, size_t offset, const void *scalars, size_t n, size_t batch,
-                      size_t stride_bytes, int sfmt, int flags, void *out, int ofmt);
+                      size_t stride_bytes, int sfmt, int flags, void *out, int ofmt, bool may_group = false);
 int g1_sum_batch_strided(kzg_ctx *ctx, const void *points, size_t count, size_t groups, size_t gstride, size_t istride, int pfmt,
                          int flags, void *out, int ofmt, int level = POINTS_ON_CURVE);
 
diff --git a/kzg_amd/csrc/msm.hip b/kzg_amd/csrc/msm.hip
--- a/kzg_amd/csrc/msm.hip
+++ b/kzg_amd/csrc/msm.hip
@@ -154,8 +154,8 @@
 
 constexpr int BIN_SHIFT = 6, BIN_BUCKETS = 1 << BIN_SHIFT;
 
-__global__ __launch_bounds__(1024) void k_bin_hist(const Fr *scalars, size_t n, int sfmt, size_t per_block, uint32_t *blk_bins,
-                                                   int w_lo, int w_hi) {
+__device__ __forceinline__ void bin_hist_body(const Fr *scalars, size_t n, int sfmt, size_t per_block, uint32_t *blk_bins, int w_lo,
+                                              int w_hi) {
     KZG_SIDE_PRIO_STMT;
     __shared__ uint32_t h[NBINS];
     for (int b = threadIdx.x; b < NBINS; b += blockDim.x) h[b] = 0;
@@ -173,10 +173,19 @@
     __syncthreads();
     for (int b = threadIdx.x; b < NBINS; b += blockDim.x) blk_bins[(size_t)blockIdx.x * NBINS + b] = h[b];
 }
+__global__ __launch_bounds__(1024) void k_bin_hist(const Fr *scalars, size_t n, int sfmt, size_t per_block, uint32_t *blk_bins,
+                                                   int w_lo, int w_hi) {
+    bin_hist_body(scalars, n, sfmt, per_block, blk_bins, w_lo, w_hi);
+}
+__global__ __launch_bounds__(1024) void k_bin_hist_g(const GroupSlot *tab, GroupSortOff o, size_t n, int sfmt, size_t per_block, int w_lo,
+                                                     int w_hi) {
+    const GroupSlot s = tab[blockIdx.y];
+    bin_hist_body((const Fr *)s.scalars, n, sfmt, per_block, (uint32_t *)(s.base + o.bins), w_lo, w_hi);
+}
 
 constexpr int BIN_SCAN_SLICES = 16, BIN_SCAN_MAXG = 32;
 constexpr int SORT2_MAX_BLOCKS = BIN_SCAN_SLICES * BIN_SCAN_MAXG;
-__global__ __launch_bounds__(1024) void k_bin_scan(uint32_t *blk_bins, int G, uint32_t *bin_total, uint32_t *ready) {
+__device__ __forceinline__ void bin_scan_body(uint32_t *blk_bins, int G, uint32_t *bin_total, uint32_t *ready) {
     KZG_SIDE_PRIO_STMT;
     __shared__ uint32_t part[BIN_SCAN_SLICES][64];
     if (blockIdx.x == 0 && threadIdx.x < SCAN_SEG) ready[threadIdx.x] = 0;
@@ -208,13 +217,20 @@
         if (k < gs && g0 + k < G) blk_bins[(size_t)(g0 + k) * NBINS + bin] = pre + v[k];
     if (slice == 0) bin_total[bin] = tot;
 }
+__global__ __launch_bounds__(1024) void k_bin_scan(uint32_t *blk_bins, int G, uint32_t *bin_total, uint32_t *ready) {
+    bin_scan_body(blk_bins, G, bin_total, ready);
+}
+__global__ __launch_bounds__(1024) void k_bin_scan_g(const GroupSlot *tab, GroupSortOff o, int G) {
+    char *base = tab[blockIdx.y].base;
+    bin_scan_body((uint32_t *)(base + o.bins), G, (uint32_t *)(base + o.bin_base) + NBINS + 1, (uint32_t *)(base + o.agg) + SCAN_SEG);
+}
 
 
 constexpr int BIN_SCATTER_LDS = (3 * NBINS + 16 + 15 * 1024) * 4;
 template <class REC>
-__global__ __launch_bounds__(1024) void k_bin_scatter(const Fr *scalars, size_t n, int sfmt, size_t per_block, const uint32_t *blk_off,
-                                                      const uint32_t *bin_total, uint32_t *bin_base, uint32_t row_stride,
-                                                      uint32_t idx_base, typename REC::T *rec, int w_lo, int w_hi) {
+__device__ __forceinline__ void bin_scatter_body(const Fr *scalars, size_t n, int sfmt, size_t per_block, const uint32_t *blk_off,
+                                                 const uint32_t *bin_total, uint32_t *bin_base, uint32_t row_stride, uint32_t idx_base,
+                                                 typename REC::T *rec, int w_lo, int w_hi) {
     KZG_SIDE_PRIO_STMT;
     uint32_t *cur = lds_u32, *cnt = cur + NBINS, *off = cnt + NBINS, *wsum = off + NBINS, *stage = wsum + 16;
     const uint32_t tid = threadIdx.x;
@@ -262,6 +278,20 @@
         __syncthreads();
         cur[tid] += cnt[tid];
     }
+}
+template <class REC>
+__global__ __launch_bounds__(1024) void k_bin_scatter(const Fr *scalars, size_t n, int sfmt, size_t per_block, const uint32_t *blk_off,
+                                                      const uint32_t *bin_total, uint32_t *bin_base, uint32_t row_stride,
+                                                      uint32_t idx_base, typename REC::T *rec, int w_lo, int w_hi) {
+    bin_scatter_body<REC>(scalars, n, sfmt, per_block, blk_off, bin_total, bin_base, row_stride, idx_base, rec, w_lo, w_hi);
+}
+template <class REC>
+__global__ __launch_bounds__(1024) void k_bin_scatter_g(const GroupSlot *tab, GroupSortOff o, size_t n, int sfmt, size_t per_block,
+                                                        uint32_t row_stride, uint32_t idx_base, int w_lo, int w_hi) {
+    const GroupSlot s = tab[blockIdx.y];
+    uint32_t *bin_base = (uint32_t *)(s.base + o.bin_base);
+    bin_scatter_body<REC>((const Fr *)s.scalars, n, sfmt, per_block, (const uint32_t *)(s.base + o.bins), bin_base + NBINS + 1, bin_base,
+                          row_stride, idx_base, (typename REC::T *)(s.base + o.rec), w_lo, w_hi);
 }
 
 __global__ __launch_bounds__(1024) void k_naf_recode(const Fr *scalars, size_t n, int sfmt, size_t per_block, uint32_t *recs, uint32_t *blk_bins) {
@@ -356,9 +386,8 @@
 }
 
 
-__global__ __launch_bounds__(SCAN_SEG) void k_scan_b_bins(const uint32_t *total, const uint32_t *bin_base, int B, int NB,
-                                                          uint32_t *bucket_start, uint32_t *s1, MsmState *st, uint32_t slots,
-                                                          uint32_t *ready) {
+__device__ __forceinline__ void scan_b_bins_body(const uint32_t *total, const uint32_t *bin_base, int B, int NB, uint32_t *bucket_start,
+                                                 uint32_t *s1, MsmState *st, uint32_t slots, uint32_t *ready) {
     KZG_SIDE_PRIO_STMT;
     __shared__ uint32_t lds[4];
     const uint32_t M = bin_base[NBINS];
@@ -395,6 +424,16 @@
         st->ovf_tasks = 0;
     }
 }
+__global__ __launch_bounds__(SCAN_SEG) void k_scan_b_bins(const uint32_t *total, const uint32_t *bin_base, int B, int NB,
+                                                          uint32_t *bucket_start, uint32_t *s1, MsmState *st, uint32_t slots,
+                                                          uint32_t *ready) {
+    scan_b_bins_body(total, bin_base, B, NB, bucket_start, s1, st, slots, ready);
+}
+__global__ __launch_bounds__(SCAN_SEG) void k_scan_b_bins_g(const GroupSlot *tab, GroupSortOff o, int B, int NB, uint32_t slots) {
+    char *base = tab[blockIdx.y].base;
+    scan_b_bins_body((const uint32_t *)(base + o.total), (const uint32_t *)(base + o.bin_base), B, NB, (uint32_t *)(base + o.bucket_start),
+                     (uint32_t *)(base + o.s1), (MsmState *)(base + o.state), slots, (uint32_t *)(base + o.agg) + SCAN_SEG);
+}
 
 __device__ __forceinline__ G1Affine30 load_entry_point30(const uint4 *table30, uint32_t ent) {
 #if defined(KZG_TIMING_GATHER)
@@ -508,6 +547,13 @@
     size_t i = (size_t)blockIdx.x * blockDim.x + threadIdx.x;
     if (i >= count) return;
     emit_one(pts[i * stride_pts], out + i * format_bytes_dev(fmt), fmt);
+}
+
+__global__ __launch_bounds__(64) void k_emit_points_g(const GroupSlot *tab, int cnt, size_t off_result, int fmt) {
+    KZG_SIDE_PRIO_STMT;
+    const int i = blockIdx.x * blockDim.x + threadIdx.x;
+    if (i >= cnt) return;
+    emit_one(*(const MsmPoint *)(tab[i].base + off_result), (uint8_t *)tab[i].out, fmt);
 }
 
 __global__ __launch_bounds__(64) void k_sum_groups(const MsmPoint *pts, uint32_t count, uint32_t groups, size_t gstride,
@@ -959,4 +1005,55 @@
     return msm_run_narrow(ctx, lane, srs, offset, d_scalars, n, sfmt, d_result, accum_stream, sorted_ev, accum_ev, defer);
 }
 
-}
+bool msm_group_covers(const kzg_ctx *ctx, const kzg_srs *srs, size_t n) {
+    return srs->device == ctx->device && srs->narrow17 && !srs->naf && !srs->sort20 && !ctx->opt_sort_single && srs->rows == srs->W &&
+           (uint64_t)srs->rows * srs->npad < REC4_MAX_INDEX && n >= ((size_t)1 << 17) && n <= srs->n;
+}
+
+static uint32_t group_slots(const kzg_ctx *ctx) { return (uint32_t)ctx->accum_blocks_batch() * 256u; }
+
+int msm_group_sort(kzg_ctx *ctx, hipStream_t st, const kzg_srs *srs, size_t offset, size_t n, int sfmt, const GroupSlot *d_tab, int cnt,
+                   uint32_t heavy_seq) {
+    if (cnt < 1 || cnt > KZG_MAX_GROUP || !msm_group_covers(ctx, srs, n) || offset > srs->n - n)
+        return fail(ctx, KZG_ERR_INTERNAL, "grouped MSM outside its scope");
+    if (!ctx->attr_group_set) {
+        KZG_HIP_CHECK(ctx, hipFuncSetAttribute((const void *)k_bin_scatter_g<Rec4>, hipFuncAttributeMaxDynamicSharedMemorySize, BIN_SCATTER_LDS));
+        ctx->attr_group_set = true;
+    }
+    const MsmLayout L = msm_layout(srs, n);
+    const GroupSortOff o = {L.off_bins, L.off_bin_base, L.off_blk_hist, L.off_agg, L.off_total, L.off_bucket_start, L.off_s1, L.off_state,
+                            L.off_entries};
+    const int G2 = L.G2, W = srs->W;
+    const size_t per2 = (n + G2 - 1) / G2;
+    const uint32_t slots = group_slots(ctx);
+    KZG_LAUNCH(ctx, st, "k_bin_hist", k_bin_hist_g, dim3(G2, cnt), 1024, 0, d_tab, o, n, sfmt, per2, 0, W);
+    KZG_LAUNCH(ctx, st, "k_bin_scan", k_bin_scan_g, dim3(NBINS / 64, cnt), 1024, 0, d_tab, o, G2);
+    KZG_LAUNCH(ctx, st, "k_bin_scatter", k_bin_scatter_g<Rec4>, dim3(G2, cnt), 1024, BIN_SCATTER_LDS, d_tab, o, n, sfmt, per2,
+               (uint32_t)srs->npad, (uint32_t)offset, 0, W);
+    KZG_TRY(sort2_level2_group(ctx, st, d_tab, cnt, o, slots, heavy_seq));
+    KZG_LAUNCH(ctx, st, "k_scan_b_bins", k_scan_b_bins_g, dim3(L.B / SCAN_SEG, cnt), SCAN_SEG, 0, d_tab, o, L.B, L.B / SCAN_SEG, slots);
+    return KZG_OK;
+}
+
+int msm_group_accum(kzg_ctx *ctx, hipStream_t st, const kzg_srs *srs, size_t n, char *base) {
+    const MsmLayout L = msm_layout(srs, n);
+    const uint32_t slots = group_slots(ctx);
+    const size_t thr1 = L.M_max / KZG_ACCUM_MIN_CHUNK + 1 < (size_t)slots ? L.M_max / KZG_ACCUM_MIN_CHUNK + 1 : (size_t)slots;
+    KZG_LAUNCH(ctx, st, "k_accum_affine", k_accum_affine, (unsigned)((thr1 + 255) / 256), 256, 0, (const uint32_t *)(base + L.off_entries),
+               (const uint32_t *)(base + L.off_bucket_start), (const uint32_t *)(base + L.off_s1), L.B, (const uint4 *)srs->table30,
+               (MsmPoint *)(base + L.off_bufA), (MsmState *)(base + L.off_state));
+    return KZG_OK;
+}
+
+int msm_group_tail(kzg_ctx *ctx, hipStream_t st, const kzg_srs *srs, size_t n, const GroupSlot *d_tab, int cnt, int ofmt) {
+    if (!point_format_bytes(ofmt)) return fail(ctx, KZG_ERR_SHAPE, "unknown G1 output format");
+    const MsmLayout L = msm_layout(srs, n);
+    const GroupTailOff o = {L.off_bufA, L.off_bufB, L.off_s1, L.off_state, L.off_tail + L.tail.off_dense, L.off_tail + L.tail.off_rows,
+                            L.off_tail + L.tail.off_cols, L.off_tail + L.tail.off_Q, L.off_tail + L.tail.off_tasks,
+                            L.off_tail + L.tail.off_arrive, L.off_tail + L.tail.off_result};
+    KZG_TRY(msm_tail_run_group(ctx, st, d_tab, cnt, o, L.B, expected_partials(L.M_max, group_slots(ctx), L.B)));
+    KZG_LAUNCH(ctx, st, "k_emit_points", k_emit_points_g, (cnt + 63) / 64, 64, 0, d_tab, cnt, o.result, ofmt);
+    return KZG_OK;
+}
+
+}
diff --git a/kzg_amd/csrc/msm_internal.h b/kzg_amd/csrc/msm_internal.h
--- a/kzg_amd/csrc/msm_internal.h
+++ b/kzg_amd/csrc/msm_internal.h
@@ -58,6 +58,17 @@
     size_t off_dense, off_rows, off_cols, off_Q, off_tasks, off_arrive, off_result, bytes;
 };
 TailLayout tail_layout(int B, size_t T1_max);
+
+struct GroupSortOff {
+    size_t bins, bin_base, rec, agg, total, bucket_start, s1, state, entries;
+};
+struct GroupTailOff {
+    size_t part, scratch, s1, state, dense, rows, cols, Q, tasks, arrive, result;
+};
+int sort2_level2_group(kzg_ctx *ctx, hipStream_t st, const GroupSlot *d_tab, int cnt, const GroupSortOff &o, uint32_t slots,
+                       uint32_t heavy_seq);
+int msm_tail_run_group(kzg_ctx *ctx, hipStream_t st, const GroupSlot *d_tab, int cnt, const GroupTailOff &o, int B,
+                       size_t expected_partials);
 int msm_tail_run(kzg_ctx *ctx, hipStream_t st, const MsmMode &mode, const MsmPoint *part, MsmPoint *scratch, const uint32_t *s1, int B,
                  size_t expected_partials, MsmState *state, char *tail_base, const TailLayout &L, MsmPoint **d_result,
                  bool odd_weights = false);
diff --git a/kzg_amd/csrc/msm_tail.hip b/kzg_amd/csrc/msm_tail.hip
--- a/kzg_amd/csrc/msm_tail.hip
+++ b/kzg_amd/csrc/msm_tail.hip
@@ -42,8 +42,8 @@
 }
 
 template <int G>
-__global__ KZG_TAIL_LB void k_fold_dense(const MsmPoint *part, const uint32_t *s1, int B, MsmPoint *dense, MsmState *st,
-                                                    uint32_t *tasks, uint32_t *arrive) {
+__device__ __forceinline__ void fold_dense_body(const MsmPoint *part, const uint32_t *s1, int B, MsmPoint *dense, MsmState *st,
+                                                uint32_t *tasks, uint32_t *arrive) {
     KZG_SIDE_PRIO_STMT;
     const uint32_t gid = blockIdx.x * blockDim.x + threadIdx.x;
     const uint32_t b = gid / G, g = gid % G;
@@ -63,9 +63,20 @@
     acc = butterfly_sum<G>(acc);
     if (g == 0) dense[b] = acc;
 }
-
-__global__ KZG_TAIL_LB void k_fold_overflow(const MsmPoint *part, MsmPoint *scratch, const uint32_t *s1, MsmPoint *dense,
-                                                       const MsmState *st, const uint32_t *tasks, uint32_t *arrive) {
+template <int G>
+__global__ KZG_TAIL_LB void k_fold_dense(const MsmPoint *part, const uint32_t *s1, int B, MsmPoint *dense, MsmState *st,
+                                                    uint32_t *tasks, uint32_t *arrive) {
+    fold_dense_body<G>(part, s1, B, dense, st, tasks, arrive);
+}
+template <int G>
+__global__ KZG_TAIL_LB void k_fold_dense_g(const GroupSlot *tab, GroupTailOff o, int B) {
+    char *base = tab[blockIdx.y].base;
+    fold_dense_body<G>((const MsmPoint *)(base + o.part), (const uint32_t *)(base + o.s1), B, (MsmPoint *)(base + o.dense),
+                       (MsmState *)(base + o.state), (uint32_t *)(base + o.tasks), (uint32_t *)(base + o.arrive));
+}
+
+__device__ __forceinline__ void fold_overflow_body(const MsmPoint *part, MsmPoint *scratch, const uint32_t *s1, MsmPoint *dense,
+                                                   const MsmState *st, const uint32_t *tasks, uint32_t *arrive) {
     KZG_SIDE_PRIO_STMT;
     const uint32_t T = st->ovf_tasks;
     if (T == 0) return;
@@ -92,6 +103,16 @@
         }
     }
 }
+__global__ KZG_TAIL_LB void k_fold_overflow(const MsmPoint *part, MsmPoint *scratch, const uint32_t *s1, MsmPoint *dense,
+                                                       const MsmState *st, const uint32_t *tasks, uint32_t *arrive) {
+    fold_overflow_body(part, scratch, s1, dense, st, tasks, arrive);
+}
+__global__ KZG_TAIL_LB void k_fold_overflow_g(const GroupSlot *tab, GroupTailOff o) {
+    char *base = tab[blockIdx.y].base;
+    fold_overflow_body((const MsmPoint *)(base + o.part), (MsmPoint *)(base + o.scratch), (const uint32_t *)(base + o.s1),
+                       (MsmPoint *)(base + o.dense), (const MsmState *)(base + o.state), (const uint32_t *)(base + o.tasks),
+                       (uint32_t *)(base + o.arrive));
+}
 
 __global__ KZG_TAIL_LB void k_rc_sums(const MsmPoint *dense, int Rn, int Cn, MsmPoint *rows, MsmPoint *cols) {
     KZG_SIDE_PRIO_STMT;
@@ -111,7 +132,7 @@
 }
 
 constexpr int RC_LANES = 8;
-__global__ KZG_TAIL_LB void k_rc_sums_t(const MsmPoint *dense, int Rn, int Cn, MsmPoint *rows, MsmPoint *cols) {
+__device__ __forceinline__ void rc_sums_t_body(const MsmPoint *dense, int Rn, int Cn, MsmPoint *rows, MsmPoint *cols) {
     KZG_SIDE_PRIO_STMT;
     const int gid = blockIdx.x * blockDim.x + threadIdx.x;
     const int sum = gid / RC_LANES, l = gid % RC_LANES;
@@ -129,8 +150,15 @@
     acc = butterfly_sum<RC_LANES>(acc);
     if (l == 0) (sum < Rn ? rows[sum] : cols[sum - Rn]) = acc;
 }
-
-__global__ KZG_TAIL_LB void k_weighted_bits(const MsmPoint *rows, const MsmPoint *cols, int lr, int lc, MsmPoint *Q) {
+__global__ KZG_TAIL_LB void k_rc_sums_t(const MsmPoint *dense, int Rn, int Cn, MsmPoint *rows, MsmPoint *cols) {
+    rc_sums_t_body(dense, Rn, Cn, rows, cols);
+}
+__global__ KZG_TAIL_LB void k_rc_sums_t_g(const GroupSlot *tab, GroupTailOff o, int Rn, int Cn) {
+    char *base = tab[blockIdx.y].base;
+    rc_sums_t_body((const MsmPoint *)(base + o.dense), Rn, Cn, (MsmPoint *)(base + o.rows), (MsmPoint *)(base + o.cols));
+}
+
+__device__ __forceinline__ void weighted_bits_body(const MsmPoint *rows, const MsmPoint *cols, int lr, int lc, MsmPoint *Q) {
     KZG_SIDE_PRIO_STMT;
     const int lane = threadIdx.x & 63;
     const int wv = (int)((blockIdx.x * blockDim.x + threadIdx.x) >> 6);
@@ -150,8 +178,15 @@
     acc = butterfly_sum<64>(acc);
     if (lane == 0) Q[wv] = acc;
 }
-
-__global__ __launch_bounds__(64) void k_reduce_final(const MsmPoint *Q, int lr, int lc, MsmPoint *result, int odd) {
+__global__ KZG_TAIL_LB void k_weighted_bits(const MsmPoint *rows, const MsmPoint *cols, int lr, int lc, MsmPoint *Q) {
+    weighted_bits_body(rows, cols, lr, lc, Q);
+}
+__global__ KZG_TAIL_LB void k_weighted_bits_g(const GroupSlot *tab, GroupTailOff o, int lr, int lc) {
+    char *base = tab[blockIdx.y].base;
+    weighted_bits_body((const MsmPoint *)(base + o.rows), (const MsmPoint *)(base + o.cols), lr, lc, (MsmPoint *)(base + o.Q));
+}
+
+__device__ __forceinline__ void reduce_final_body(const MsmPoint *Q, int lr, int lc, MsmPoint *result, int odd) {
     KZG_SIDE_PRIO_STMT;
     const int lane = threadIdx.x;
     const int cnt = lr + lc + 1;
@@ -162,6 +197,13 @@
         if (k < shift && lane < cnt) p = g1_dbl30(p);
     p = butterfly_sum<32>(p);
     if (lane == 0) *result = p;
+}
+__global__ __launch_bounds__(64) void k_reduce_final(const MsmPoint *Q, int lr, int lc, MsmPoint *result, int odd) {
+    reduce_final_body(Q, lr, lc, result, odd);
+}
+__global__ __launch_bounds__(64) void k_reduce_final_g(const GroupSlot *tab, GroupTailOff o, int lr, int lc) {
+    char *base = tab[blockIdx.y].base;
+    reduce_final_body((const MsmPoint *)(base + o.Q), lr, lc, (MsmPoint *)(base + o.result), 0);
 }
 
 template <int SRC>
@@ -370,4 +412,29 @@
     return KZG_OK;
 }
 
-}
+int msm_tail_run_group(kzg_ctx *ctx, hipStream_t st, const GroupSlot *d_tab, int cnt, const GroupTailOff &o, int B,
+                       size_t expected_partials) {
+    int Rn, Cn, lr, lc;
+    tail_shape(B, &Rn, &Cn, &lr, &lc);
+    if (Rn < RC_LANES || Cn < RC_LANES) return fail(ctx, KZG_ERR_INTERNAL, "grouped tail: bucket count");
+    const size_t avg = expected_partials / (size_t)B + 1;
+    int G = 1;
+    while (G < 64 && (size_t)G * (FOLD_SEQ / 2) < avg) G *= 2;
+    const int wpb = TAIL_THREADS / 64;
+    const unsigned grid = (unsigned)(((size_t)B * G + TAIL_THREADS - 1) / TAIL_THREADS);
+#define KZG_FOLD(GG)                                                                                              \
+    case GG:                                                                                                      \
+        KZG_LAUNCH(ctx, st, "k_fold_dense", k_fold_dense_g<GG>, dim3(grid, cnt), TAIL_THREADS, 0, d_tab, o, B); \
+        break;
+    switch (G) {
+        KZG_FOLD(1) KZG_FOLD(2) KZG_FOLD(4) KZG_FOLD(8) KZG_FOLD(16) KZG_FOLD(32) KZG_FOLD(64)
+    }
+#undef KZG_FOLD
+    KZG_LAUNCH(ctx, st, "k_fold_overflow", k_fold_overflow_g, dim3(256, cnt), TAIL_THREADS, 0, d_tab, o);
+    KZG_LAUNCH(ctx, st, "k_rc_sums", k_rc_sums_t_g, dim3(((Rn + Cn) * RC_LANES + 255) / 256, cnt), 256, 0, d_tab, o, Rn, Cn);
+    KZG_LAUNCH(ctx, st, "k_weighted_bits", k_weighted_bits_g, dim3((lr + lc + 1 + wpb - 1) / wpb, cnt), TAIL_THREADS, 0, d_tab, o, lr, lc);
+    KZG_LAUNCH(ctx, st, "k_reduce_final", k_reduce_final_g, dim3(1, cnt), 64, 0, d_tab, o, lr, lc);
+    return KZG_OK;
+}
+
+}
diff --git a/kzg_amd/csrc/msm_wide.hip b/kzg_amd/csrc/msm_wide.hip
--- a/kzg_amd/csrc/msm_wide.hip
+++ b/kzg_amd/csrc/msm_wide.hip
@@ -390,9 +390,9 @@
 __device__ __forceinline__ uint32_t heavy_slices(uint32_t size, uint32_t SL) { return size > 4 * SL ? (size + SL - 1) / SL : 0u; }
 
 template <class REC, int NB>
-__global__ __launch_bounds__(SORT2_THREADS) void k_bin_sort2(const typename REC::T *rec, const uint32_t *bin_base, uint32_t *entries,
-                                                             uint32_t *total, uint32_t *bucket_start, MsmState *st, uint32_t slots,
-                                                             int sliced, uint32_t *lane_heavy, uint32_t heavy_seq) {
+__device__ __forceinline__ void bin_sort2_body(const typename REC::T *rec, const uint32_t *bin_base, uint32_t *entries, uint32_t *total,
+                                               uint32_t *bucket_start, MsmState *st, uint32_t slots, int sliced, uint32_t *lane_heavy,
+                                               uint32_t heavy_seq) {
     typedef typename REC::T RT;
     __shared__ uint32_t h[NB], cur[NB], off[NB], sc[4];
     __shared__ RT stage[SORT2_CHUNK];
@@ -423,6 +423,18 @@
     }
     sort2_place_range<REC, NB>(rec, r0, r1, entries, h, cur, off, sc, stage);
 }
+template <class REC, int NB>
+__global__ __launch_bounds__(SORT2_THREADS) void k_bin_sort2(const typename REC::T *rec, const uint32_t *bin_base, uint32_t *entries,
+                                                             uint32_t *total, uint32_t *bucket_start, MsmState *st, uint32_t slots,
+                                                             int sliced, uint32_t *lane_heavy, uint32_t heavy_seq) {
+    bin_sort2_body<REC, NB>(rec, bin_base, entries, total, bucket_start, st, slots, sliced, lane_heavy, heavy_seq);
+}
+template <class REC, int NB>
+__global__ __launch_bounds__(SORT2_THREADS) void k_bin_sort2_g(const GroupSlot *tab, GroupSortOff o, uint32_t slots, uint32_t heavy_seq) {
+    const GroupSlot s = tab[blockIdx.y];
+    bin_sort2_body<REC, NB>((const typename REC::T *)(s.base + o.rec), (const uint32_t *)(s.base + o.bin_base),
+                            (uint32_t *)(s.base + o.entries), (uint32_t *)(s.base + o.total), nullptr, nullptr, slots, 0, s.heavy, heavy_seq);
+}
 
 __device__ __forceinline__ uint32_t heavy_bin_of(const uint32_t *hv, uint32_t id) {
     uint32_t lo = 0, hi = NBINS;
@@ -581,6 +593,12 @@
     return sort2_level2_t<Rec20, SORT20_BUCKETS>(ctx, st, rec, bin_base, hv, entries, nullptr, bucket_start, state, slots, sliced, lane_heavy, heavy_seq);
 }
 
+int sort2_level2_group(kzg_ctx *ctx, hipStream_t st, const GroupSlot *d_tab, int cnt, const GroupSortOff &o, uint32_t slots,
+                       uint32_t heavy_seq) {
+    KZG_LAUNCH(ctx, st, "k_bin_sort", (k_bin_sort2_g<Rec4, 64>), dim3(NBINS, cnt), SORT2_THREADS, 0, d_tab, o, slots, heavy_seq);
+    return KZG_OK;
+}
+
 int sort20_place(kzg_ctx *ctx, hipStream_t st, const void *d_scalars, size_t n, int sfmt, int G2, const uint32_t *bins,
                  const uint32_t *bin_total, uint32_t *bin_base, uint32_t row_stride, uint32_t idx_base, void *rec, uint32_t *entries,
                  uint32_t *bucket_start, uint32_t *s1, MsmState *state, uint32_t slots, uint32_t *segsums, uint32_t *segmaxs,
diff --git a/kzg_amd/csrc/runtime.hip b/kzg_amd/csrc/runtime.hip
--- a/kzg_amd/csrc/runtime.hip
+++ b/kzg_amd/csrc/runtime.hip
@@ -130,8 +130,8 @@
     char nf[32] = "none";
     if (ctx->plan_lanes < ctx->plan_want_lanes || ctx->plan_accum < ctx->plan_want_accum)
         snprintf(nf, sizeof nf, "%d+%d", ctx->plan_want_lanes, ctx->plan_want_accum);
-    snprintf(buf, buflen, "device=%d lanes=%d accum_streams=%d hw_queues_found=%d narrowed_from=%s witness_cache_slots=%d", ctx->device,
-             ctx->plan_lanes, ctx->plan_accum, ctx->plan_queues, nf, ctx->opt_witness_cache_slots);
+    snprintf(buf, buflen, "device=%d lanes=%d accum_streams=%d hw_queues_found=%d narrowed_from=%s witness_cache_slots=%d group_msms=%d", ctx->device,
+             ctx->plan_lanes, ctx->plan_accum, ctx->plan_queues, nf, ctx->opt_witness_cache_slots, ctx->plan_group);
     return KZG_OK;
 }
 
@@ -215,8 +215,8 @@
         delete ctx;
         return KZG_ERR_HIP;
     }
-    if (hipMalloc((void **)&ctx->d_lane_heavy, KZG_MAX_LANES * 4) != hipSuccess ||
-        hipMemset(ctx->d_lane_heavy, 0, KZG_MAX_LANES * 4) != hipSuccess) {
+    const size_t heavy_bytes = (KZG_MAX_LANES + KZG_GROUP_DEPTH * KZG_MAX_GROUP) * 4;
+    if (hipMalloc((void **)&ctx->d_lane_heavy, heavy_bytes) != hipSuccess || hipMemset(ctx->d_lane_heavy, 0, heavy_bytes) != hipSuccess) {
         if (ctx->d_lane_heavy) hipFree(ctx->d_lane_heavy);
         pool_unref(ctx->pool);
         delete ctx;
@@ -247,6 +247,8 @@
     for (auto e : ctx->event_pool) hipEventDestroy(e);
     for (auto e : ctx->sorted_events) hipEventDestroy(e);
     for (auto e : ctx->accum_events) hipEventDestroy(e);
+    for (auto e : ctx->group_events) hipEventDestroy(e);
+    if (ctx->group_tab) hipFree(ctx->group_tab);
     if (ctx->batch_out) hipFree(ctx->batch_out);
     if (ctx->d_lane_heavy) hipFree(ctx->d_lane_heavy);
     for (auto &ct : ctx->coset_tabs)
@@ -334,6 +336,9 @@
         if (value < 0 || value > 64) return fail(ctx, KZG_ERR_SHAPE, "hw_queues must be 0 (GPU_MAX_HW_QUEUES or the ROCm default of 4) or 1..64");
         ctx->opt_hw_queues = (int)value;
         ctx->pipe_planned = false;
+    } else if (k == "group_msms") {
+        if (value < 0 || value > KZG_MAX_GROUP) return fail(ctx, KZG_ERR_SHAPE, "group_msms must be 0 (never grouped) or 1..16 MSMs per sort / tail launch");
+        ctx->opt_group_msms = (int)value;
     } else if (k == "window_rows") {
         if (value < 0 || value > 64) return fail(ctx, KZG_ERR_SHAPE, "window_rows must be 0 (one table row per window) or 1..64");
         ctx->opt_window_rows = (int)value;
@@ -686,17 +691,26 @@
             ctx->pipe_planned = false;
         }
     }
-    if (getenv("KZG_DEBUG")) fprintf(stderr, "kzg: pipeline plan: %d lanes + %d accumulation streams\n", nl, nas);
+    const int plan_group = nl >= 2 && (nas >= 2 || (nas == 1 && nl >= 3)) ? ctx->opt_group_msms : 0;
+    if (getenv("KZG_DEBUG")) {
+        if (plan_group)
+            fprintf(stderr, "kzg: pipeline plan: %d lanes + %d accumulation streams; batches the grouped shape covers: groups of %d on 4 streams\n", nl, nas, plan_group);
+        else
+            fprintf(stderr, "kzg: pipeline plan: %d lanes + %d accumulation streams\n", nl, nas);
+    }
     if (want > 1) {
         ctx->plan_want_lanes = want_nl, ctx->plan_want_accum = want_nas, ctx->plan_lanes = nl, ctx->plan_accum = nas, ctx->plan_queues = found_queues;
         if ((nl < want_nl || nas < want_nas) && !ctx->plan_warned) {
             ctx->plan_warned = true;
             fprintf(stderr, "kzg: device %d: this context's %d + %d streams found only %d hardware queues of their own (other streams of the "
                             "process hold the rest: another context, an RCCL communicator, the host's); the batched pipeline is narrowed to %d "
-                            "lanes + %d accumulation streams -- expect 10-25 %% less batched throughput from THIS context.  Create contexts before "
+                            "lanes + %d accumulation streams -- expect 10-25 %% less throughput from THIS context for concurrent blocking callers, "
+                            "the *_many calls and batches outside the grouped shape%s.  Create contexts before "
                             "communicators, give the process more queues (kzg_init_hw_queues / GPU_MAX_HW_QUEUES before the first HIP call) or set "
                             "option \"streams\" explicitly; kzg_ctx_info reports the plan.\n",
-                    ctx->device, want_nl, want_nas, found_queues, nl, nas);
+                    ctx->device, want_nl, want_nas, found_queues, nl, nas,
+                    plan_group ? " (kzg_msm_g1_batch with 17-bit windows from 2^17 points on runs grouped on four streams and does not need the queues)"
+                               : "");
         }
     }
     KZG_TRY(ensure_lanes(ctx, nl));
@@ -708,6 +722,7 @@
         ctx->accum_events.push_back(e2);
     }
     ctx->planned_accum = nas;
+    ctx->plan_group = plan_group;
     *nl_out = nl;
     *nas_out = nas;
     return KZG_OK;
```
